# LPD-EPFL-ML/X-MAP

Measured on AMD Instinct MI355X. Metric: item_sim_pairs_per_s, higher is better.
Workload: dtype f64

## Files before the change

### include/xmap_hip.h

```cpp
#ifndef XMAP_HIP_H
#define XMAP_HIP_H
#include <stdint.h>

#ifdef __cplusplus
extern "C" {
#endif

#define XMAP_OK 0
#define XMAP_ERR_HIP -1
#define XMAP_ERR_ARG -2
#define XMAP_ERR_OVERFLOW -3
#define XMAP_ERR_CAPACITY -4

#define XMAP_COSINE 0
#define XMAP_ADJUST_COSINE 1
#define XMAP_COSINE_EXACT 2

#define XMAP_TOPC 10

typedef struct xmap_ratings {
    int64_t n_users;
    int32_t n_items;
    int64_t nnz;
    const int64_t *user_ptr;
    const int32_t *user_item;
    const float *user_rating;
    const int64_t *user_time;
    const int64_t *item_ptr;
    const int32_t *item_user;
    const float *item_rating;
    const int32_t *prefix_cls;
    const int32_t *suffix_cls;
    const uint32_t *contains_mask;
    const uint8_t *flags;
} xmap_ratings;

const char *xmap_last_error(void);
int xmap_version(void);

int xmap_trim(void);
int xmap_debug_arena(void *stream, int64_t *live, int64_t *reserved);
int xmap_debug_arena_call(void *stream, int64_t bytes, int fail);

int xmap_exclusive_scan_i64(void *stream, const int64_t *in, int64_t *out, int64_t n, int64_t *h_total);
int xmap_exclusive_scan_i32_to_i64(void *stream, const int32_t *in, int64_t *out, int64_t n, int64_t *h_total);


int xmap_build_csc(void *stream, int64_t n_users, int32_t n_items, int64_t nnz, const int64_t *user_ptr,
                   const int32_t *user_item, const float *user_rating, int32_t *cnt ,
                   int64_t *item_ptr , int32_t *item_user , float *item_rating );

int xmap_user_stats(void *stream, const xmap_ratings *R, double *u_avg, double *u_norm2);

int xmap_item_stats(void *stream, const xmap_ratings *R, const double *u_avg, double *info ,
                    double *norms ,
                    int32_t *ua_item , int32_t *ia_user ,
                    int32_t item_lo, int32_t item_hi );

#ifdef XMAP_CROSSCHECK
int xmap_sim_plan(void *stream, const xmap_ratings *R, int32_t slot_target, int32_t *Q, int64_t *W, int64_t *unit_ptr,
                  int64_t *h_n_units, int64_t *h_contrib);
int xmap_sim_units(void *stream, int32_t n_items, const int32_t *Q, const int64_t *unit_ptr,
                   int32_t *unit_item , int32_t *unit_q );

int xmap_sim_count(void *stream, const xmap_ratings *R, int method, int cap, const double *u_avg,
                   const double *info, const int32_t *ua_item, const int32_t *ia_user, const int32_t *Q,
                   const int32_t *unit_item, const int32_t *unit_q, int64_t unit_lo, int64_t unit_hi,
                   int32_t *unit_cnt , int64_t *d_counters , int64_t *h_counters );
int xmap_sim_fill(void *stream, const xmap_ratings *R, int method, int cap, const double *u_avg,
                  const double *info, const int32_t *ua_item, const int32_t *ia_user, const int32_t *Q,
                  const int32_t *unit_item, const int32_t *unit_q, int64_t unit_lo, int64_t unit_hi,
                  const int64_t *unit_off , int32_t *col, double *sim, int32_t *mutu, int32_t *nij);

int xmap_sim_row_ptr(void *stream, int32_t n_items, const int64_t *unit_ptr, const int64_t *unit_off ,
                     int64_t *row_ptr );
#endif

#define XMAP_PAIRS_HEAVY 1
#define XMAP_PAIRS_LIGHT 2
#define XMAP_PAIRS_HEAVY_MERGE 4
#define XMAP_PAIRS_RESET 8
#define XMAP_PAIRS_MIRCOUNT 16
#define XMAP_PAIRS_RAW 32
#define XMAP_PAIRS_SHARD_SUMS 64
#define XMAP_PAIRS_NO_MARKS 128
#define XMAP_PAIRS_DEAL(m, r) ((((m) & 0xff) << 16) | (((r) & 0xff) << 8))
#define XMAP_PAIRS_DEAL_MOD(phases) (((phases) >> 16) & 0xff)
#define XMAP_PAIRS_DEAL_REM(phases) (((phases) >> 8) & 0xff)
int xmap_sim2_layout(void *stream, const xmap_ratings *R, const double *info, int32_t ch_min, int32_t *hist ,
                     int64_t *pre , int32_t *ctl , int32_t *hid , int32_t *hlist ,
                     uint64_t *ub_key , void *ub ,
                     void *rc ,
                     uint64_t *Wp ,
                     int32_t dups , int32_t *h_ctl );
int xmap_sim2_plan(void *stream, const xmap_ratings *R, int32_t slot_target, const void *rc, const int64_t *pre,
                   const int32_t *hid, const int32_t *ctl, int32_t *Q, int32_t *C, uint8_t *small ,
                   uint64_t *Wp , int32_t *Qcat , int64_t *uq_ptr ,
                   int64_t *uc_ptr , int32_t dups, int64_t *h_counts );
int xmap_sim2_units(void *stream, int32_t n_items, const int64_t *item_ptr, const int32_t *Qcat, const int64_t *uq_ptr,
                    int32_t *uq_item, int32_t *uq_q , const int32_t *C, const int64_t *uc_ptr, int32_t *uc_item,
                    int32_t *uc_c);
int xmap_sim2_pairs(void *stream, const xmap_ratings *R, int method, int cap, const double *u_avg, const double *norms,
                    const void *rc, const void *ub, const int32_t *Q,
                    const uint8_t *small, const int32_t *uq_item, const int32_t *uq_q, const int64_t *cls_ptr ,
                    int64_t unit_lo, int64_t unit_hi, const int32_t *hid,
                    const int32_t *hlist, const int32_t *ctl, const int32_t *C, const int64_t *uc_ptr,
                    const int32_t *uc_item, const int32_t *uc_c, int32_t n_heavy_units, int32_t n_heavy, int phases,
                    double *hp_hi, double *hp_lo, int32_t *hp_cnt, int32_t *hp_mut, int64_t coo_cap, int32_t *coo_i,
                    int32_t *coo_j, double *coo_sim, int32_t *coo_mutu, int32_t *coo_nij,
                    double *coo_ls , int32_t *rowcnt,
                    int64_t *d_shards ,
                    int64_t *d_counters ,
                    int32_t *mircnt );
int xmap_sim2_scatter(void *stream, int32_t n_items, int64_t n_coo, const int32_t *coo_i, const int32_t *coo_j,
                      const double *coo_sim, const int32_t *coo_mutu, const int32_t *coo_nij, const double *coo_ls ,
                      const int64_t *row_ptr, int32_t *fill , const int32_t *hid, const int32_t *hlist,
                      int32_t *col, double *sim, int32_t *mutu, int32_t *nij, double *ls );
#define XMAP_LAYOUT_RECORDS 1
#define XMAP_LAYOUT_STATS 2
#define XMAP_LAYOUT_UB_FLAGS 4
#define XMAP_LAYOUT_RC_FLAGS 8
#define XMAP_LAYOUT_ALL 15
int xmap_sim3_layout(void *stream, const xmap_ratings *R, int64_t *item_ptr ,
                     const double *rating64 , int32_t ch_min, int32_t phases, int32_t stats_lo, int32_t stats_hi,
                     int32_t *cnt ,
                     double *u_avg , double *u_norm , int32_t *hist ,
                     int64_t *pre , int32_t *ctl , int32_t *hid , int32_t *hlist ,
                     uint64_t *ub_key , void *ub , void *srec ,
                     void *bufA , void *bufB , void *rc ,
                     uint64_t *Wp , double *info , double *norms , int32_t *h_ctl );
int xmap_sim3_plan(void *stream, const xmap_ratings *R, int32_t slot_target, const int64_t *pre, const int32_t *hid,
                   const int32_t *ctl, int32_t *Q, int32_t *C, uint8_t *small, uint64_t *Wp, int32_t *Qcat ,
                   int64_t *uq_ptr , int64_t *uc_ptr , int32_t dups, int32_t *uq_item, int32_t *uq_q ,
                   int32_t *uc_item, int32_t *uc_c, int64_t cap_light, int64_t cap_heavy, int64_t *h_out );
int xmap_sim3_mircount(void *stream, int32_t n_items, int64_t coo_cap, const int32_t *coo_i, const int32_t *coo_j,
                       const int64_t *d_shards , int64_t n_pairs, int32_t skip_self, void *scratch, int32_t *mir );
int xmap_sim3_mirror(void *stream, int32_t n_items, int64_t coo_cap, const int32_t *coo_i, const int32_t *coo_j,
                     const double *coo_sim, const int32_t *coo_mutu, const int32_t *coo_nij,
                     const int64_t *d_shards ,
                     int64_t n_pairs, const int32_t *own , const int32_t *mir , int32_t *tot ,
                     int64_t *row_ptr , int64_t *mptr , int32_t *fill ,
                     void *bufA , void *bufB , int32_t *col,
                     double *sim, int32_t *mutu, int32_t *nij, const double *coo_aux , double *aux ,
                     int32_t row_lo, int32_t row_hi );

int xmap_sim2_pack_pairs(void *stream, int64_t n_coo, const int32_t *coo_i, const int32_t *coo_j, const double *coo_sim,
                         const int32_t *coo_mutu, const int32_t *coo_nij, int64_t *rec , int64_t *h_count);
int xmap_sim2_unpack_pairs(void *stream, int64_t n, const int64_t *rec , int32_t *coo_i, int32_t *coo_j, double *coo_sim,
                           int32_t *coo_mutu, int32_t *coo_nij);
int xmap_item_partials(void *stream, const xmap_ratings *R, const double *u_avg, double *partial );
int xmap_item_merge(void *stream, int32_t n_items, int32_t n_parts, const double *parts , double *info ,
                    double *norms );
int xmap_sim2_pack_partials(void *stream, int64_t n_coo, const int32_t *coo_i, const int32_t *coo_j, const double *coo_hi,
                            const double *coo_lo, const int32_t *coo_mutu, const int32_t *coo_nij, int64_t *rec ,
                            int64_t *h_count);
int xmap_sim2_sort_partials(void *stream, int64_t n, const int64_t *rec , int64_t *rec_sorted , int32_t n_items,
                            int32_t n_owners );
int xmap_sim2_merge_partials(void *stream, int method, int cap, int32_t n_items, int64_t n, const int64_t *rec_sorted,
                             const double *norms , int32_t *coo_i, int32_t *coo_j, double *coo_sim, int32_t *coo_mutu,
                             int32_t *coo_nij, int32_t *rowcnt , int64_t *h_counts );



typedef struct xmap_sim {
    int32_t n_items;
    const int64_t *row_ptr;
    const int32_t *col;
    const double *sim;
    const int32_t *mutu;
    const int32_t *nij;
    const double *info;
    const double *frac;
} xmap_sim;

int xmap_bridge_flags(void *stream, const xmap_sim *S, const int32_t *prefix_cls, uint8_t *bb);

int xmap_knn_classify(void *stream, const xmap_sim *S, int top_k, const uint8_t *bb, const int32_t *suffix_cls,
                      const uint32_t *contains_mask, uint8_t *cls, int32_t *kcnt ,
                      int32_t *kcol , double *kval ,
                      int32_t row_lo, int32_t row_hi );

int xmap_knn_thresholds(void *stream, int32_t n_items, int top_k, const int32_t *kcnt, const int32_t *kcol, const double *kval,
                        void *thr );
int xmap_reverse_count(void *stream, const xmap_sim *S, int mode, int top_k, const uint8_t *bb, const uint8_t *cls,
                       const int32_t *kcnt, const int32_t *kcol, const double *kval, const int32_t *suffix_cls,
                       const uint32_t *contains_mask, const uint8_t *flags, const int64_t *attach_ptr,
                       const void *thr ,
// ... 344 lines not shown
```

### x-map_amd/csrc/api.hip

```cpp
#include <math.h>
#include <stdlib.h>
#include <vector>

#include "common.h"

namespace xmap {

struct Pool {
    std::vector<void *> ptrs;
    void release() {
        for (void *p : ptrs) (void)hipFree(p);
        ptrs.clear();
    }
};
struct ScratchPool : Pool { ~ScratchPool() { release(); } };

}

using namespace xmap;

struct xmap_ctx {
    int device = 0;
    hipStream_t st = nullptr;
    Pool p_ratings, p_sim, p_ext, p_gen, p_rows;
// ... 168 lines not shown
    XM_HIP(hipMemsetAsync(c->top_end, 0xff, sizeof(int32_t) * (size_t)I * XMAP_TOPC, c->st));
    XM_HIP(hipMemsetAsync(c->top_val, 0, sizeof(double) * (size_t)I * XMAP_TOPC, c->st));
    int64_t *d_cnt;
    XM_ALLOCZ(c->p_ext, d_cnt, 8);
    int64_t h_cnt[8] = {0, 0, 0, 0, 0, 0, 0, 0};
    int rc;
    if (c->T.n_nb > 0) rc = xmap_extend_cols(c->st, &c->T, &c->Un, &Rw, &O, c->fast_div, d_cnt, h_cnt);
    else rc = xmap_extend_paths(c->st, &c->T, &c->Un, &Rw, &O, d_cnt, h_cnt);
    if (rc && rc != XMAP_ERR_CAPACITY) {
        c->p_rows.release();
        c->acc = nullptr;
    }
    c->n_out = h_cnt[0]; c->n_paths = h_cnt[1];
    return rc;
}

struct TriPass {
    const xmap_ratings *R;
    const double *rating64;
    int ch_min, dups, method, cap;
    bool heavy;
    bool aux, skip_self;
    int64_t half_contrib;
    Pool *stats_pool, *csr_pool, *mutu_pool;
    int64_t *row_ptr;
};
struct TriResult {
    double *u_avg, *u_norm , *info, *norms , *sim, *aux;
    int32_t *col, *mutu, *nij;
    int64_t n, n_unordered, kept;
};

static int tri_pass(hipStream_t st, const TriPass &J, Pool &tmp, TriResult &O) {
#define T_ALLOC(ptr, n) XM_TRY(dalloc(tmp, &(ptr), (size_t)(n), st))
#define T_ALLOCZ(ptr, n) XM_TRY(dalloc(tmp, &(ptr), (size_t)(n), st, true))
    const xmap_ratings &R = *J.R;
    const int I = R.n_items;
    const int64_t U = R.n_users, nnz = R.nnz;
    const bool wide = J.rating64 != nullptr;
    const size_t n1 = (size_t)(nnz ? nnz : 1), i1 = (size_t)(I ? I : 1);
    const size_t rw = wide ? 3 : 2;
    int32_t *cnt, *hist, *ctl, *hid, *hlist;
    int64_t *pre;
    uint64_t *ub_key, *ub, *rcrec, *Wp, *srec, *buf_a, *buf_b;
    O.u_norm = nullptr; O.aux = nullptr;
    XM_TRY(dalloc(*J.stats_pool, &O.u_avg, (size_t)U, st, wide));
    if (!wide) XM_TRY(dalloc(*J.stats_pool, &O.u_norm, (size_t)U, st));
    XM_TRY(dalloc(*J.stats_pool, &O.info, i1 * 4, st, true));
    T_ALLOCZ(O.norms, 2 * i1);
    T_ALLOC(cnt, i1);
    T_ALLOC(hist, U + 2); T_ALLOC(pre, U + 3); T_ALLOC(ctl, 4); T_ALLOC(hid, i1); T_ALLOCZ(hlist, 1024);
    T_ALLOC(ub_key, n1); T_ALLOC(ub, (wide ? 2 : 1) * n1); T_ALLOC(rcrec, 2 * n1); T_ALLOC(Wp, i1);
    T_ALLOC(srec, rw * n1); T_ALLOC(buf_a, rw * n1); T_ALLOC(buf_b, rw * n1);
    XM_TRY(xmap_sim3_layout(st, &R, (int64_t *)R.item_ptr, J.rating64, J.ch_min, XMAP_LAYOUT_RECORDS | XMAP_LAYOUT_STATS | XMAP_LAYOUT_UB_FLAGS,
                            0, I, cnt, O.u_avg, O.u_norm, hist, pre, ctl, hid, hlist, ub_key, ub, srec, buf_a, buf_b, rcrec, Wp, O.info,
                            O.norms, nullptr));
    int32_t *Q, *Cc, *Qcat, *uq_item = nullptr, *uq_q = nullptr, *uc_item = nullptr, *uc_c = nullptr;
    uint8_t *small;
    int64_t *uq_ptr, *uc_ptr;
    T_ALLOCZ(Q, i1); T_ALLOCZ(Cc, i1); T_ALLOCZ(small, i1); T_ALLOC(Qcat, 5 * i1); T_ALLOCZ(uq_ptr, (size_t)5 * I + 1);
    T_ALLOCZ(uc_ptr, I + 1);
    int slot_target = 768;
    double coo_slack = 1.0;
    int64_t hc[10];
    auto plan = [&](int target) -> int {
        const int64_t cap_light = J.half_contrib / target + I + 1, cap_heavy = nnz / J.ch_min + 1025;
        T_ALLOC(uq_item, cap_light); T_ALLOC(uq_q, 4 * cap_light); T_ALLOC(uc_item, cap_heavy); T_ALLOC(uc_c, cap_heavy);
        return xmap_sim3_plan(st, &R, target, pre, hid, ctl, Q, Cc, small, Wp, Qcat, uq_ptr, uc_ptr, J.dups, uq_item, uq_q, uc_item, uc_c,
                              cap_light, cap_heavy, hc);
    };
    XM_TRY(plan(slot_target));
    const int phases = XMAP_PAIRS_RESET | XMAP_PAIRS_LIGHT | XMAP_PAIRS_MIRCOUNT | XMAP_PAIRS_SHARD_SUMS | XMAP_PAIRS_NO_MARKS |
                       (J.heavy ? XMAP_PAIRS_HEAVY | XMAP_PAIRS_HEAVY_MERGE : 0);
    int32_t *coo_i = nullptr, *coo_j = nullptr, *coo_mutu = nullptr, *coo_nij = nullptr, *own = nullptr, *mir = nullptr;
    double *coo_sim = nullptr, *coo_aux = nullptr;
    int64_t *d_shards = nullptr;
    int64_t cap_coo = 0;
    for (;;) {
        const int64_t n_light = hc[0], n_hu = J.heavy ? hc[1] : 0, n_heavy = J.heavy ? hc[9] : 0;
        cap_coo = ((int64_t)((double)(J.half_contrib > 0 ? J.half_contrib : 1) * coo_slack) / 4096 + 1100) * 4096;
        double *hp_hi, *hp_lo;
        int32_t *hp_cnt, *hp_mut;
        int64_t *d_cnt;
        T_ALLOC(coo_i, cap_coo); T_ALLOC(coo_j, cap_coo); T_ALLOC(coo_sim, cap_coo); T_ALLOC(coo_mutu, cap_coo); T_ALLOC(coo_nij, cap_coo);
        if (J.aux) T_ALLOC(coo_aux, cap_coo);
        T_ALLOC(own, i1); T_ALLOC(mir, i1);
        const size_t hp = (size_t)(n_hu ? n_hu : 1) * 1024;
        T_ALLOC(hp_hi, hp); T_ALLOC(hp_lo, hp); T_ALLOC(hp_cnt, hp); T_ALLOC(hp_mut, hp);
        T_ALLOCZ(d_cnt, 6); T_ALLOC(d_shards, 2 * 4096);
        XM_TRY(xmap_sim2_pairs(st, &R, J.method, J.cap, O.u_avg, O.norms, rcrec, ub, Q, small, uq_item, uq_q, hc + 2, 0, n_light, hid, hlist,
                               ctl, Cc, uc_ptr, uc_item, uc_c, (int32_t)n_hu, (int32_t)n_heavy, phases, hp_hi, hp_lo, hp_cnt, hp_mut, cap_coo, coo_i,
                               coo_j, coo_sim, coo_mutu, coo_nij, coo_aux, own, d_shards, d_cnt, mir));
        int64_t h_cnt[6];
        XM_TRY(d2h(h_cnt, d_cnt, 6, st));
        XM_HIP(hipStreamSynchronize(st));
        if (h_cnt[2]) {
            if (slot_target <= 32) { set_error("pair-table overflow"); return XMAP_ERR_OVERFLOW; }
            slot_target /= 2;
            XM_TRY(plan(slot_target));
            continue;
        }
        if (h_cnt[3]) {
            if (coo_slack > 64) { set_error("half-COO overflow"); return XMAP_ERR_CAPACITY; }
            coo_slack *= 2;
            continue;
        }
        O.n = h_cnt[4]; O.n_unordered = h_cnt[5];
        break;
    }
    const int64_t n = O.n;
    const size_t nn = (size_t)(n ? n : 1);
    O.kept = 2 * n;
    int64_t *mptr;
    int32_t *fill, *tot;
    uint64_t *mir_a, *mir_b;
    T_ALLOCZ(mptr, I + 1);
    XM_TRY(dalloc(*J.csr_pool, &O.col, (size_t)O.kept, st)); XM_TRY(dalloc(*J.csr_pool, &O.sim, (size_t)O.kept, st));
    XM_TRY(dalloc(*J.mutu_pool, &O.mutu, (size_t)O.kept, st)); XM_TRY(dalloc(*J.csr_pool, &O.nij, (size_t)O.kept, st));
    if (J.aux) XM_TRY(dalloc(*J.csr_pool, &O.aux, (size_t)O.kept, st));
    T_ALLOC(fill, i1); T_ALLOC(tot, i1); T_ALLOC(mir_a, (J.aux ? 4 : 3) * nn); T_ALLOC(mir_b, (J.aux ? 4 : 3) * nn);
    XM_TRY(xmap_sim3_mircount(st, I, cap_coo, coo_i, coo_j, d_shards, n, J.skip_self ? 1 : 0, mir_a, mir));
    return xmap_sim3_mirror(st, I, cap_coo, coo_i, coo_j, coo_sim, coo_mutu, coo_nij, d_shards, n, own, mir, tot, J.row_ptr, mptr, fill, mir_a,
                            mir_b, O.col, O.sim, O.mutu, O.nij, coo_aux, O.aux, 0, I);
#undef T_ALLOC
#undef T_ALLOCZ
}

}

extern "C" {

int xmap_ctx_create(int device, xmap_ctx **out) {
    XM_ARG(out);
    *out = nullptr;
    XM_HIP(hipSetDevice(device));
    xmap_ctx *c = new xmap_ctx();
    c->device = device;
    memset(&c->R, 0, sizeof(c->R)); memset(&c->S, 0, sizeof(c->S)); memset(&c->T, 0, sizeof(c->T)); memset(&c->Un, 0, sizeof(c->Un));
    hipError_t e = hipStreamCreate(&c->st);
    if (e != hipSuccess) { delete c; set_error("hipStreamCreate -> %s", hipGetErrorString(e)); return XMAP_ERR_HIP; }
    *out = c;
    return XMAP_OK;
}

void xmap_ctx_destroy(xmap_ctx *c) {
    if (!c) return;
    (void)hipSetDevice(c->device);
    (void)hipStreamSynchronize(c->st);
    drop_tail(c);
    drop_fold(c);
    drop_union(c);
    c->p_gen.release(); c->p_ext.release(); c->p_sim.release(); c->p_rows.release(); c->p_ratings.release();
    if (c->st) (void)hipStreamDestroy(c->st);
    delete c;
}

static bool plain_sums_exact(int64_t U, int64_t nnz, const float *rating) {
    const char *force = getenv("XMAP_EXACT_COSINE");
    if (force && force[0] == '1') return false;
    double M = 0.0;
    int e = 0;
    for (int64_t k = 0; k < nnz; k++) {
        const double r = fabs((double)rating[k]);
        if (!(r <= 1e300)) return false;
        if (r > M) M = r;
        while (e <= 26 && ldexp(r, e) != floor(ldexp(r, e))) e++;
        if (e > 26) return false;
    }
    if (M == 0.0) return true;
    const double Mi = ldexp(M, e);
    if (Mi > 134217728.0) return false;
    const uint64_t m2 = (uint64_t)Mi * (uint64_t)Mi;
    return (uint64_t)U <= (1ull << 53) / m2;
}
// ... 1208 lines not shown
```

### x-map_amd/csrc/common.h

```cpp
#pragma once
#if defined(__HIP_DEVICE_COMPILE__) && !defined(__gfx950__)
#error "libxmap_hip is written for gfx950 (MI355X): build with --offload-arch=gfx950"
#endif
#include <hip/hip_runtime.h>
#include <stdint.h>
#include <stdio.h>
#include <string.h>

#include "../../include/xmap_hip.h"

namespace xmap {

void set_error(const char *fmt, ...);

#define XM_HIP(call)                                                                         \
    do {                                                                                     \
        hipError_t e_ = (call);                                                              \
        if (e_ != hipSuccess) {                                                              \
            xmap::set_error("%s:%d %s -> %s", __FILE__, __LINE__, #call, hipGetErrorString(e_)); \
            return XMAP_ERR_HIP;                                                             \
        }                                                                                    \
    } while (0)

#define XM_LAUNCH_CHECK() XM_HIP(hipGetLastError())

#define XM_ARG(cond)                                                        \
    do {                                                                    \
        if (!(cond)) {                                                      \
            xmap::set_error("%s:%d bad argument: %s", __FILE__, __LINE__, #cond); \
            return XMAP_ERR_ARG;                                            \
        }                                                                   \
    } while (0)

hipError_t xm_malloc_async(void **p, size_t bytes, hipStream_t st);
hipError_t xm_free_async(void *p, hipStream_t st);
struct XmScope {
    int dev; hipStream_t st; size_t live0; bool ok;
    explicit XmScope(hipStream_t st);
    ~XmScope();
    XmScope(const XmScope &) = delete;
    XmScope &operator=(const XmScope &) = delete;
};
#define XM_SCOPE(stream) xmap::XmScope xm_scope_((hipStream_t)(stream))
int radix_sort_pairs(hipStream_t st, unsigned long long *keys, int *vals, unsigned long long *keys_tmp, int *vals_tmp, long long n,
                     int bits);

constexpr int WAVE = 64;

__device__ __forceinline__ int lane_id() { return threadIdx.x & 63; }

__device__ __forceinline__ int rl32(int v, int l) { return __builtin_amdgcn_readlane(v, l); }
__device__ __forceinline__ float rlf(float v, int l) { return __int_as_float(rl32(__float_as_int(v), l)); }
__device__ __forceinline__ long long rl64(long long v, int l) {
    int lo = rl32((int)(v & 0xffffffffll), l), hi = rl32((int)(v >> 32), l);
    return ((long long)hi << 32) | (unsigned int)lo;
}
__device__ __forceinline__ double rld(double v, int l) {
    return __longlong_as_double(rl64(__double_as_longlong(v), l));
}
__device__ __forceinline__ int uniform(int v) { return __builtin_amdgcn_readfirstlane(v); }

__device__ __forceinline__ unsigned long long lanemask_lt() {
    return (1ull << lane_id()) - 1ull;
}

__device__ __forceinline__ double wave_sum(double v) {
#pragma unroll
    for (int m = 32; m >= 1; m >>= 1) v += __shfl_xor(v, m, 64);
    return v;
}
__device__ __forceinline__ long long wave_sum_ll(long long v) {
#pragma unroll
    for (int m = 32; m >= 1; m >>= 1) v += __shfl_xor(v, m, 64);
    return v;
}

__device__ __forceinline__ void dd_add(double &hi, double &lo, double x) {
    double s = hi + x;
    double bb = s - hi;
    double e = (hi - (s - bb)) + (x - bb);
    e += lo;
    double h2 = s + e;
    lo = e - (h2 - s);
    hi = h2;
}

template <int G>
__device__ __forceinline__ void dd_reduce(double &hi, double &lo) {
#pragma unroll
    for (int m = G / 2; m >= 1; m >>= 1) {
        double oh = __shfl_down(hi, m, G), ol = __shfl_down(lo, m, G);
        dd_add(hi, lo, oh);
        dd_add(hi, lo, ol);
    }
}

// ... 7 lines not shown
```

### x-map_amd/csrc/tri.h

```cpp
#pragma once
#include "common.h"
#include "tilesort.h"

namespace xmap {

constexpr int T_SLOTS = 1024;
constexpr int HMAX = 1024;
constexpr int SMALL_BOUND = 96;
constexpr int MID_BOUND = 384;

constexpr int N_CLASSES = 5;
constexpr int WIDE_MIN = 2048;
__host__ __device__ __forceinline__ int class_rank(int cls) {
    return cls == 4 ? 0 : (cls == 0 ? 1 : (cls == 2 ? 2 : (cls == 3 ? 3 : 4)));
}

__device__ __forceinline__ double weighted(double cs, int n, int cap) {
    const int mn = n < cap ? n : cap;
    return 1.0 * cs * (double)mn / (double)cap;
}
__device__ __forceinline__ unsigned long long ls_key(double d) {
    return (d != d) ? 0x7ff8000000000000ull : (unsigned long long)__double_as_longlong(d);
}

struct RaterRec { int e0; int pos_ge; float rating; int user; };
struct UbWide { int item_ge; int pad; double rating; };
struct RaterRecWide { int e0; int pos_ge; double rating; };

constexpr int COO_SHARDS = 4096;

int mirror_counts(hipStream_t st, int n_items, long long range_cap, int n_ranges, const unsigned long long *cur, const int *coo_i,
                  const int *coo_j, bool skip_self, int *part, int *counts);
void ts_geometry(int K, long long M, int ch, ts::Geo &G);
int ts_prepare(hipStream_t st, ts::Geo &G, const long long *ptr);
extern template __global__ void ts::k_ts_bin<3, true, ts::RecLoader<3>>(ts::Geo, ts::RecLoader<3>, long long, unsigned long long *__restrict__);

}
```

### x-map_amd/csrc/tri_layout.hip

```cpp
#include "tri.h"
#include "item_stats.h"

namespace xmap {

__device__ __forceinline__ unsigned long long wkey(int n, int item) {
    return ((unsigned long long)(unsigned)n << 32) | (unsigned)item;
}

constexpr int HIST_LDS = 2048;
constexpr int HIST_PER = 16;
__global__ __launch_bounds__(256) void k_hist(int I, const long long *iptr, int HB, int *hist) {
    __shared__ int loc[HIST_LDS];
    for (int t = threadIdx.x; t < HIST_LDS; t += 256) loc[t] = 0;
    __syncthreads();
    const long long base = (long long)blockIdx.x * 256 * HIST_PER;
    for (int q = 0; q < HIST_PER; q++) {
        const long long i = base + (long long)q * 256 + threadIdx.x;
        if (i < I) {
            long long n = iptr[i + 1] - iptr[i];
            int bin = n < HB - 1 ? (int)n : HB - 1;
            if (bin < HIST_LDS) atomicAdd(&loc[bin], 1); else atomicAdd(&hist[bin], 1);
        }
    }
    __syncthreads();
// ... 132 lines not shown
        i = lo;
        const int u = iuser[p];
        const long long a = uptr[u], b = uptr[u + 1];
        RaterRec r;
        r.e0 = (int)a; r.pos_ge = 0; r.rating = 0.f; r.user = u;
        for (long long e = a; e < b; e++) {
            int2 v = ub[e];
            if ((v.x & 0x7fffffff) == i) {
                if (taken && e + 1 < b && (ub[e + 1].x & 0x7fffffff) == i) {
                    e += atomicAdd(&taken[e], 1);
                    v = ub[e];
                }
                const int pos = (b - a >= 2) ? (int)(e - a) : 0;
                r.pos_ge = (int)((unsigned)pos | ((unsigned)v.x & 0x80000000u));
                r.rating = __int_as_float(v.y);
                pos_sum = pos;
                break;
            }
        }
        rc[p] = r;
    }
    const int lane = lane_id();
    const int i_prev = __shfl_up(i, 1, 64);
    const unsigned long long heads = __ballot(lane == 0 || i != i_prev);
    long long incl = pos_sum;
#pragma unroll
    for (int d = 1; d < 64; d <<= 1) { const long long t = __shfl_up(incl, d, 64); if (lane >= d) incl += t; }
    const bool seg_end = (lane == 63) || ((heads >> (lane + 1)) & 1ull);
    const int h = 63 - __clzll((long long)(heads & ((lane == 63) ? ~0ull : ((2ull << lane) - 1ull))));
    const long long before = __shfl(incl, h > 0 ? h - 1 : 0, 64);
    if (seg_end && i >= 0) {
        const long long seg = incl - (h > 0 ? before : 0);
        if (seg) atomicAdd(&Wp[i], (unsigned long long)seg);
    }
}
__device__ __forceinline__ void plan_item(int i, long long w, int I, const long long *iptr, const long long *pre, int HB,
                                          const int *hid, const int *CH, int target, int dups, int *Q, int *C,
                                          uint8_t *small, unsigned long long *Wp, int *Qcat) {
    const long long n = iptr[i + 1] - iptr[i];
    long long ge = I - pre[n < HB - 1 ? n : HB - 1];
    const long long others = ge - 1 + (dups ? 1 : 0);
    long long bound = w < others ? w : others;
    int q = 0, c = 0;
    if (w > 0) {
        if (hid[i] >= 0) c = (int)((n + *CH - 1) / *CH);
        else q = (int)((bound + target - 1) / target);
    }
    Q[i] = q;
    C[i] = c;
    const int cls = (q >= 1 && n >= WIDE_MIN) ? 4
                    : ((q != 1) ? 0 : (bound <= SMALL_BOUND ? 1 : (bound <= 2 * SMALL_BOUND ? 3 : (bound <= MID_BOUND ? 2 : 0))));
    small[i] = (uint8_t)cls;
    Wp[i] = (unsigned long long)w;
    Qcat[(size_t)class_rank(cls) * I + i] = q;
}

__global__ __launch_bounds__(256) void k_plan2(int I, const long long *iptr, const RaterRec *rc, const long long *pre,
                                               int HB, const int *hid, const int *CH, int target, int dups, int *Q, int *C,
                                               uint8_t *small, unsigned long long *Wp, int *Qcat) {
    const int i = blockIdx.x * blockDim.x + threadIdx.x;
    if (i >= I) return;
    plan_item(i, (long long)Wp[i], I, iptr, pre, HB, hid, CH, target, dups, Q, C, small, Wp, Qcat);
}

__global__ __launch_bounds__(256) void k_fill_units2(int I, const long long *iptr, const int *Qcat, const long long *uq_ptr,
                                                     int *uq_item, int *uq_q, const int *C, const long long *uc_ptr, int *uc_item,
                                                     int *uc_c, long long cap_light, long long cap_heavy) {
    const long long x = (long long)blockIdx.x * blockDim.x + threadIdx.x;
    if (x >= (long long)N_CLASSES * I) return;
    const int i = (int)(x % I);
    long long b = uq_ptr[x];
    const int nq = Qcat[x];
    if (nq > 0) {
        const int p0 = (int)iptr[i], p1 = (int)iptr[i + 1];
        for (int k = 0; k < nq && b + k < cap_light; k++) {
            uq_item[b + k] = i;
            ((int4 *)uq_q)[b + k] = make_int4(k, p0, p1, nq);
        }
    }
    if (x >= I) return;
    b = uc_ptr[i];
    for (int k = 0; k < C[i] && b + k < cap_heavy; k++) { uc_item[b + k] = i; uc_c[b + k] = k; }
}

constexpr int CNT_SLOTS = 4096;
constexpr int CNT_CHUNK = 8192;
__device__ __forceinline__ int cnt_slot(int it) { return (int)(mix32((uint32_t)it) & (CNT_SLOTS - 1)); }

__global__ __launch_bounds__(256) void k_count3(long long nnz, const int *uitem, int *cnt) {
    __shared__ int tag[CNT_SLOTS], loc[CNT_SLOTS];
    for (int t = threadIdx.x; t < CNT_SLOTS; t += 256) { tag[t] = -1; loc[t] = 0; }
    __syncthreads();
    const long long e0 = (long long)blockIdx.x * CNT_CHUNK;
    for (int q = threadIdx.x; q < CNT_CHUNK; q += 256) {
        const long long e = e0 + q;
        if (e >= nnz) break;
        const int it = uitem[e];
        const int sl = cnt_slot(it);
        const int old = atomicCAS(&tag[sl], -1, it);
        if (old == -1 || old == it) atomicAdd(&loc[sl], 1); else atomicAdd(&cnt[it], 1);
    }
    __syncthreads();
    for (int t = threadIdx.x; t < CNT_SLOTS; t += 256)
        if (loc[t]) atomicAdd(&cnt[tag[t]], loc[t]);
}


template <bool WIDE>
__device__ __forceinline__ void sort_entry3(const int *uitem, const float *ur32, const double *ur64, const int *cnt,
                                            long long e, unsigned long long &key, int &px, long long &py) {
    const int it = uitem[e];
    key = wkey(cnt[it], it);
    px = it;
    py = WIDE ? __double_as_longlong(ur64[e]) : (long long)(unsigned)__float_as_int(ur32[e]);
}

template <bool WIDE>
__device__ __forceinline__ void bitonic_desc3(int width, int pos, unsigned long long &key, int &px, long long &py) {
#pragma unroll
    for (int k2 = 2; k2 <= 64; k2 <<= 1) {
        if (k2 <= width)
// ... 269 lines not shown
        dd_add(s, slo, o[0]);
        dd_add(s, slo, o[1]);
        dd_add(q, qlo, o[2]);
        dd_add(q, qlo, o[3]);
        dd_add(a2, a2lo, o[4]);
        dd_add(a2, a2lo, o[5]);
        n += o[6];
    }
    const int i = d.x;
    info[(size_t)i * 4 + 0] = (n > 0.0) ? 1.0 * s / n : 0.0;
    info[(size_t)i * 4 + 1] = sqrt(q);
    info[(size_t)i * 4 + 2] = sqrt(a2);
    info[(size_t)i * 4 + 3] = 1.0 * n;
    norms[i] = sqrt(q);
    norms[(size_t)I + i] = sqrt(a2);
}

template <typename Src>
__global__ __launch_bounds__(256) void k_item_big_flags(const long long *iptr, const Src src, BigList B, const double *info) {
    const unsigned c = blockIdx.x * 4 + uniform((int)(threadIdx.x >> 6));
    if (c >= B.counters[0]) return;
    const int2 d = B.chunks[c];
    const double avg = info[(size_t)d.x * 4];
    const long long p0 = iptr[d.x] + (long long)d.y * STAT_CHK;
    const long long p1 = min(iptr[d.x + 1], p0 + STAT_CHK);
    for (long long p = p0 + lane_id(); p < p1; p += 64) {
        double r; int u;
        src.load(p, r, u);
        src.set_flag(p, r >= avg);
    }
}

__global__ __launch_bounds__(256) void k_rc_flags(long long nnz, RaterRec *rc, const int2 *ub, const double *info) {
    const long long p = (long long)blockIdx.x * blockDim.x + threadIdx.x;
    if (p >= nnz) return;
    const RaterRec r = rc[p];
    const int it = ub[(long long)r.e0 + (r.pos_ge & 0x7fffffff)].x & 0x7fffffff;
    if ((double)r.rating >= info[(size_t)it * 4]) rc[p].pos_ge = (int)((unsigned)r.pos_ge | 0x80000000u);
}

__global__ __launch_bounds__(256) void k_ub_flags(long long nnz, int2 *ub, const double *info) {
    const long long e = (long long)blockIdx.x * blockDim.x + threadIdx.x;
    if (e >= nnz) return;
    const int2 v = ub[e];
    if ((double)__int_as_float(v.y) >= info[(size_t)v.x * 4]) ub[e].x = (int)((unsigned)v.x | 0x80000000u);
}

}

using namespace xmap;

namespace {

int heavy_set(void *stream, int I, int64_t n_users, const int64_t *item_ptr, int32_t ch_min, int32_t *hist, int64_t *pre, int32_t *ctl,
              int32_t *hid, int32_t *hlist) {
    hipStream_t st = (hipStream_t)stream;
    const int HB = (int)n_users + 2;
    XM_HIP(hipMemsetAsync(hist, 0, sizeof(int32_t) * (size_t)HB, st));
    XM_HIP(hipMemsetAsync(ctl, 0x7f, sizeof(int32_t), st));
    XM_HIP(hipMemsetAsync(ctl + 1, 0, 3 * sizeof(int32_t), st));
    if (I > 0) {
        k_hist<<<dim3((unsigned)((I + 256 * HIST_PER - 1) / (256 * HIST_PER))), dim3(256), 0, st>>>(I, (const long long *)item_ptr, HB, hist);
        XM_LAUNCH_CHECK();
    }
    int rcode = xmap_exclusive_scan_i32_to_i64(stream, hist, pre, HB, nullptr);
    if (rcode) return rcode;
    if (HB - 1 > ch_min) {
        k_threshold<<<dim3((unsigned)((HB + 255) / 256)), dim3(256), 0, st>>>(I, HB, (const long long *)pre, ch_min, ctl);
        XM_LAUNCH_CHECK();
    }
    if (I > 0) {
        k_mark_heavy<<<dim3((unsigned)((I + 255) / 256)), dim3(256), 0, st>>>(I, (const long long *)item_ptr, ctl, hid, hlist, ctl + 1);
        XM_LAUNCH_CHECK();
    }
    return XMAP_OK;
}

int read_heavy_ctl(hipStream_t st, const int32_t *ctl, int32_t *h_ctl) {
    XM_HIP(hipMemcpyAsync(h_ctl, ctl, 2 * sizeof(int32_t), hipMemcpyDeviceToHost, st));
    XM_HIP(hipStreamSynchronize(st));
    if (h_ctl[1] > HMAX) {
        set_error("heavy set larger than %d", HMAX);
        return XMAP_ERR_OVERFLOW;
    }
    return XMAP_OK;
}

int plan_rows(void *stream, const xmap_ratings *R, int32_t slot_target, const void *rc, const int64_t *pre, const int32_t *hid,
              const int32_t *ctl, int32_t *Q, int32_t *C, uint8_t *small, uint64_t *Wp, int32_t *Qcat, int64_t *uq_ptr, int64_t *uc_ptr,
              int32_t dups, int64_t *h_light, int64_t *h_heavy) {
    XM_ARG(slot_target > 0 && slot_target <= T_SLOTS);
    hipStream_t st = (hipStream_t)stream;
    const int I = R->n_items;
    XM_HIP(hipMemsetAsync(Qcat, 0, sizeof(int32_t) * (size_t)N_CLASSES * (size_t)(I > 0 ? I : 1), st));
    if (I > 0) {
        k_plan2<<<dim3((unsigned)((I + 255) / 256)), dim3(256), 0, st>>>(
            I, (const long long *)R->item_ptr, (const RaterRec *)rc, (const long long *)pre, (int)R->n_users + 2, hid, ctl, slot_target, dups,
            Q, C, small, (unsigned long long *)Wp, Qcat);
        XM_LAUNCH_CHECK();
    }
    int rcode = xmap_exclusive_scan_i32_to_i64(stream, Qcat, uq_ptr, (int64_t)N_CLASSES * I, h_light);
    if (rcode) return rcode;
    return xmap_exclusive_scan_i32_to_i64(stream, C, uc_ptr, I, h_heavy);
}

template <int RW>
int sort_rater_records(hipStream_t st, const ts::Geo &G, long long nnz, const void *srec, void *bufA, void *bufB, const int64_t *user_ptr,
                       void *rc, uint64_t *Wp) {
    constexpr bool WIDE = RW == 3;
    const dim3 gridA((unsigned)((nnz + G.ch - 1) / G.ch)), gridB((unsigned)G.clist_cap), gridL((unsigned)G.slist_cap);
    ts::RecLoader<RW> LA{(const unsigned long long *)srec}, LB{(const unsigned long long *)bufA};
    ts::k_ts_bin<RW, false, ts::RecLoader<RW>><<<gridA, dim3(ts::BT), 0, st>>>(G, LA, nnz, (unsigned long long *)bufA);
    XM_LAUNCH_CHECK();
    ts::k_ts_bin<RW, true, ts::RecLoader<RW>><<<gridB, dim3(ts::BT), 0, st>>>(G, LB, nnz, (unsigned long long *)bufB);
    XM_LAUNCH_CHECK();
    k_rc_tiles<WIDE><<<dim3((unsigned)G.T), dim3(ts::CT), 0, st>>>(G, (const unsigned long long *)bufB, (const long long *)user_ptr,
                                                                  (ulonglong2 *)rc, (unsigned long long *)Wp);
    XM_LAUNCH_CHECK();
    k_rc_large<WIDE><<<gridL, dim3(ts::LT), 0, st>>>(G, (const unsigned long long *)bufB, (const long long *)user_ptr, (ulonglong2 *)rc,
                                                     (unsigned long long *)Wp);
    XM_LAUNCH_CHECK();
    return XMAP_OK;
}

template <typename Src>
int item_stats3(hipStream_t st, int I, int lo, int hi, const int64_t *item_ptr, const Src &src, double *info, double *norms,
                const BigList &B) {
    const long long *iptr = (const long long *)item_ptr;
    const dim3 grid((unsigned)((hi - lo + 15) / 16)), gridC((unsigned)((B.chunk_cap + 3) / 4)), gridI((unsigned)((B.item_cap + 63) / 64));
    k_item_stats3<Src><<<grid, dim3(256), 0, st>>>(I, lo, hi, iptr, src, info, norms, B);
    XM_LAUNCH_CHECK();
    k_item_chunks<Src><<<gridC, dim3(256), 0, st>>>(iptr, src, B);
    XM_LAUNCH_CHECK();
    k_item_big<<<gridI, dim3(64), 0, st>>>(I, B, info, norms);
    XM_LAUNCH_CHECK();
    if constexpr (Src::has_flags) {
        k_item_big_flags<Src><<<gridC, dim3(256), 0, st>>>(iptr, src, B, info);
        XM_LAUNCH_CHECK();
    }
    return XMAP_OK;
}

}

extern "C" {

int xmap_sim2_layout(void *stream, const xmap_ratings *R, const double *info, int32_t ch_min, int32_t *hist ,
                     int64_t *pre , int32_t *ctl , int32_t *hid, int32_t *hlist ,
                     uint64_t *ub_key , void *ub , void *rc ,
                     uint64_t *Wp , int32_t dups, int32_t *h_ctl ) {
    XM_ARG(R && info && hist && pre && ctl && hid && hlist && ub_key && ub && rc && Wp && ch_min >= 64);
    XM_ARG(R->nnz < 0x7fffffffLL && R->n_users < 0x7ffffff0LL);
    hipStream_t st = (hipStream_t)stream;
    const int I = R->n_items;
    int rcode = heavy_set(stream, I, R->n_users, R->item_ptr, ch_min, hist, pre, ctl, hid, hlist);
    if (rcode) return rcode;
    if (R->n_users > 0) {
        k_sort_profiles<<<dim3((unsigned)((R->n_users + 15) / 16)), dim3(256), 0, st>>>(
            R->n_users, (const long long *)R->user_ptr, R->user_item, R->user_rating, (const long long *)R->item_ptr, info,
            (unsigned long long *)ub_key, (int2 *)ub);
        XM_LAUNCH_CHECK();
    }
    XM_HIP(hipMemsetAsync(Wp, 0, sizeof(uint64_t) * (size_t)(I > 0 ? I : 1), st));
    if (R->nnz > 0) {
        if (dups) XM_HIP(hipMemsetAsync(ub_key, 0, sizeof(int32_t) * (size_t)R->nnz, st));
        k_rater_records<<<dim3((unsigned)((R->nnz + 255) / 256)), dim3(256), 0, st>>>(
            I, R->nnz, (const long long *)R->item_ptr, R->item_user, (const long long *)R->user_ptr, (const int2 *)ub,
            (RaterRec *)rc, dups ? (int *)ub_key : nullptr, (unsigned long long *)Wp);
        XM_LAUNCH_CHECK();
    }
    return h_ctl ? read_heavy_ctl(st, ctl, h_ctl) : XMAP_OK;
}

int xmap_sim2_plan(void *stream, const xmap_ratings *R, int32_t slot_target, const void *rc, const int64_t *pre,
                   const int32_t *hid, const int32_t *ctl, int32_t *Q, int32_t *C, uint8_t *small, uint64_t *Wp ,
                   int32_t *Qcat , int64_t *uq_ptr , int64_t *uc_ptr, int32_t dups,
                   int64_t *h_counts ) {
    XM_ARG(R && rc && Wp && pre && hid && ctl && Q && C && small && Qcat && uq_ptr && uc_ptr && h_counts);
    hipStream_t st = (hipStream_t)stream;
    const int I = R->n_items;
    int rcode = plan_rows(stream, R, slot_target, rc, pre, hid, ctl, Q, C, small, Wp, Qcat, uq_ptr, uc_ptr, dups, &h_counts[0], &h_counts[1]);
    if (rcode) return rcode;
    if (I > 0)
        XM_HIP(hipMemcpy2DAsync(&h_counts[2], sizeof(int64_t), uq_ptr, sizeof(int64_t) * (size_t)I, sizeof(int64_t),
                                N_CLASSES, hipMemcpyDeviceToHost, st));
    else
        for (int c = 0; c < N_CLASSES; c++) h_counts[2 + c] = 0;
    XM_HIP(hipStreamSynchronize(st));
    h_counts[2 + N_CLASSES] = h_counts[0];
    return XMAP_OK;
}

int xmap_sim2_units(void *stream, int32_t n_items, const int64_t *item_ptr, const int32_t *Qcat, const int64_t *uq_ptr,
                    int32_t *uq_item, int32_t *uq_q, const int32_t *C, const int64_t *uc_ptr, int32_t *uc_item, int32_t *uc_c) {
    XM_ARG(item_ptr && Qcat && uq_ptr && uq_item && uq_q && C && uc_ptr && uc_item && uc_c);
    if (n_items == 0) return XMAP_OK;
    k_fill_units2<<<dim3((unsigned)(((long long)N_CLASSES * n_items + 255) / 256)), dim3(256), 0, (hipStream_t)stream>>>(
        n_items, (const long long *)item_ptr, Qcat, (const long long *)uq_ptr, uq_item, uq_q, C, (const long long *)uc_ptr, uc_item, uc_c, 0x7fffffffffffffffLL,
        0x7fffffffffffffffLL);
    XM_LAUNCH_CHECK();
    return XMAP_OK;
}

int xmap_sim3_plan(void *stream, const xmap_ratings *R, int32_t slot_target, const int64_t *pre, const int32_t *hid,
                   const int32_t *ctl, int32_t *Q, int32_t *C, uint8_t *small, uint64_t *Wp, int32_t *Qcat, int64_t *uq_ptr,
                   int64_t *uc_ptr, int32_t dups, int32_t *uq_item, int32_t *uq_q, int32_t *uc_item, int32_t *uc_c,
                   int64_t cap_light, int64_t cap_heavy, int64_t *h_out) {
    XM_SCOPE(stream);
    XM_ARG(R && Wp && pre && hid && ctl && Q && C && small && Qcat && uq_ptr && uc_ptr && h_out);
    XM_ARG(uq_item && uq_q && uc_item && uc_c && cap_light >= 0 && cap_heavy >= 0);
    hipStream_t st = (hipStream_t)stream;
    const int I = R->n_items;
    for (int c = 0; c < 10; c++) h_out[c] = 0;
    int rcode = plan_rows(stream, R, slot_target, nullptr, pre, hid, ctl, Q, C, small, Wp, Qcat, uq_ptr, uc_ptr, dups, nullptr, nullptr);
    if (rcode) return rcode;
    if (I > 0) {
        k_fill_units2<<<dim3((unsigned)(((long long)N_CLASSES * I + 255) / 256)), dim3(256), 0, st>>>(
            I, (const long long *)R->item_ptr, Qcat, (const long long *)uq_ptr, uq_item, uq_q, C, (const long long *)uc_ptr, uc_item, uc_c,
            cap_light, cap_heavy);
        XM_LAUNCH_CHECK();
        XM_HIP(hipMemcpy2DAsync(&h_out[2], sizeof(int64_t), uq_ptr, sizeof(int64_t) * (size_t)I, sizeof(int64_t), N_CLASSES + 1,
                                hipMemcpyDeviceToHost, st));
        XM_HIP(hipMemcpyAsync(&h_out[1], uc_ptr + I, sizeof(int64_t), hipMemcpyDeviceToHost, st));
    }
    int32_t h_ctl[2] = {0, 0};
    rcode = read_heavy_ctl(st, ctl, h_ctl);
    h_out[0] = h_out[2 + N_CLASSES];
    h_out[8] = h_ctl[0]; h_out[9] = h_ctl[1];
    if (rcode) return rcode;
    if (h_out[0] > cap_light || h_out[1] > cap_heavy) {
        set_error("unit arrays too small: %lld light / %lld heavy units, room for %lld / %lld", (long long)h_out[0], (long long)h_out[1],
                  (long long)cap_light, (long long)cap_heavy);
        return XMAP_ERR_CAPACITY;
    }
    return XMAP_OK;
}

int xmap_sim3_layout(void *stream, const xmap_ratings *R, int64_t *item_ptr, const double *rating64, int32_t ch_min, int32_t phases,
                     int32_t stats_lo, int32_t stats_hi, int32_t *cnt, double *u_avg, double *u_norm, int32_t *hist, int64_t *pre, int32_t *ctl, int32_t *hid, int32_t *hlist,
                     uint64_t *ub_key, void *ub, void *srec, void *bufA, void *bufB, void *rc, uint64_t *Wp, double *info,
                     double *norms, int32_t *h_ctl) {
    XM_SCOPE(stream);
    XM_ARG(R && item_ptr && (const int64_t *)item_ptr == R->item_ptr && cnt && u_avg && hist && pre && ctl && hid && hlist);
    XM_ARG(ub_key && ub && srec && bufA && bufB && rc && Wp && info && norms && ch_min >= 64);
    XM_ARG(R->nnz < 0x7fffffffLL && R->n_users < 0x7ffffff0LL && R->n_items >= 0);
    XM_ARG(rating64 || u_norm);
    XM_ARG(stats_lo >= 0 && stats_lo <= stats_hi && stats_hi <= R->n_items && (phases & ~XMAP_LAYOUT_ALL) == 0);
    hipStream_t st = (hipStream_t)stream;
    const int I = R->n_items;
    const long long nnz = R->nnz;
    const bool wide = rating64 != nullptr;
    const size_t In = (size_t)(I > 0 ? I : 1);
    int rcode = XMAP_OK;
    if (phases & XMAP_LAYOUT_RECORDS) {
        XM_HIP(hipMemsetAsync(cnt, 0, sizeof(int32_t) * In, st));
        const char *cb_env = getenv("XMAP_COUNT_PART_MIN");
        const long long cb_min = cb_env ? atoll(cb_env) : 2000000ll;
        if (nnz >= cb_min && I > 0) {
            rcode = mirror_counts(st, I, nnz, 1, nullptr, nullptr, R->user_item, false, (int *)bufA, cnt);
            if (rcode) return rcode;
        } else if (nnz > 0) {
            k_count3<<<dim3((unsigned)((nnz + CNT_CHUNK - 1) / CNT_CHUNK)), dim3(256), 0, st>>>(nnz, R->user_item, cnt);
            XM_LAUNCH_CHECK();
        }
        rcode = xmap_exclusive_scan_i32_to_i64(stream, cnt, item_ptr, I, nullptr);
        if (rcode) return rcode;
        if (!wide) {
            rcode = xmap_user_stats(stream, R, u_avg, u_norm);
            if (rcode) return rcode;
        }
        rcode = heavy_set(stream, I, R->n_users, item_ptr, ch_min, hist, pre, ctl, hid, hlist);
        if (rcode) return rcode;
        if (R->n_users > 0 && nnz > 0) {
            const dim3 grid((unsigned)((R->n_users + 15) / 16));
            (wide ? k_sort_profiles3<true> : k_sort_profiles3<false>)<<<grid, dim3(256), 0, st>>>(
                R->n_users, (const long long *)R->user_ptr, R->user_item, wide ? nullptr : R->user_rating, rating64, cnt,
                (unsigned long long *)ub_key, ub, (unsigned long long *)srec);
            XM_LAUNCH_CHECK();
        }
        XM_HIP(hipMemsetAsync(Wp, 0, sizeof(uint64_t) * In, st));
        if (nnz > 0 && I > 0) {
            ts::Geo G;
            ts_geometry(I, nnz, wide ? ts::Chunk<3>::CH : ts::Chunk<2>::CH, G);
            rcode = ts_prepare(st, G, (const long long *)item_ptr);
            if (rcode) return rcode;
            rcode = wide ? sort_rater_records<3>(st, G, nnz, srec, bufA, bufB, R->user_ptr, rc, Wp)
                         : sort_rater_records<2>(st, G, nnz, srec, bufA, bufB, R->user_ptr, rc, Wp);
            if (rcode) return rcode;
        }
    }
    if ((phases & XMAP_LAYOUT_STATS) && stats_hi > stats_lo) {
        BigList B;
        B.chunk_cap = nnz / STAT_CHK + nnz / STAT_BIG + 2;
        B.item_cap = nnz / STAT_BIG + 2;
        XM_HIP(xm_malloc_async((void **)&B.counters, 2 * sizeof(unsigned), st));
        XM_HIP(xm_malloc_async((void **)&B.chunks, sizeof(int2) * (size_t)B.chunk_cap, st));
        XM_HIP(xm_malloc_async((void **)&B.items, sizeof(int4) * (size_t)B.item_cap, st));
        XM_HIP(xm_malloc_async((void **)&B.part, sizeof(double) * ITEM_PART * (size_t)B.chunk_cap, st));
        XM_HIP(hipMemsetAsync(B.counters, 0, 2 * sizeof(unsigned), st));
        rcode = wide ? item_stats3(st, I, stats_lo, stats_hi, item_ptr, RcWideSrc{(const RaterRecWide *)rc}, info, norms, B)
                     : item_stats3(st, I, stats_lo, stats_hi, item_ptr, RcSrc{(RaterRec *)rc, u_avg}, info, norms, B);
        if (rcode) return rcode;
    }
    if (!wide && nnz > 0 && I > 0) {
        if (phases & XMAP_LAYOUT_RC_FLAGS) {
            k_rc_flags<<<dim3((unsigned)((nnz + 255) / 256)), dim3(256), 0, st>>>(nnz, (RaterRec *)rc, (const int2 *)ub, info);
            XM_LAUNCH_CHECK();
        }
        if (phases & XMAP_LAYOUT_UB_FLAGS) {
            k_ub_flags<<<dim3((unsigned)((nnz + 255) / 256)), dim3(256), 0, st>>>(nnz, (int2 *)ub, info);
            XM_LAUNCH_CHECK();
        }
    }
    return h_ctl ? read_heavy_ctl(st, ctl, h_ctl) : XMAP_OK;
}
}
```

### x-map_amd/csrc/tri_mirror.hip

```cpp
#include "tri.h"

namespace xmap {

constexpr int SC_U = 4;
__global__ __launch_bounds__(256) void k_scatter(long long n, const int *coo_i, const int *coo_j, const double *coo_sim,
                                                 const int *coo_mutu, const int *coo_nij, const double *coo_aux,
                                                 const long long *row_ptr, int *fill, int *col, double *sim, int *mutu,
                                                 int *nij, double *aux) {
    const int lane = lane_id();
    const long long r0 = ((long long)blockIdx.x * (blockDim.x >> 6) + uniform((int)(threadIdx.x >> 6))) * (64 * SC_U) + lane;
    int i[SC_U], j[SC_U], m[SC_U], nn[SC_U];
    double s[SC_U], x[SC_U];
    bool valid[SC_U];
#pragma unroll
    for (int u = 0; u < SC_U; u++) {
        const long long r = r0 + 64 * u;
        i[u] = (r < n) ? coo_i[r] : -1;
    }
#pragma unroll
    for (int u = 0; u < SC_U; u++) {
        const long long r = r0 + 64 * u;
        valid[u] = i[u] >= 0;
        j[u] = 0; m[u] = 0; nn[u] = 0; s[u] = 0.0; x[u] = 0.0;
        if (valid[u]) {
// ... 133 lines not shown
    int it[CB_SPB][EPT];
    unsigned rk[CB_SPB][EPT];
#pragma unroll
    for (int sg = 0; sg < CB_SPB; sg++) {
        const long long g = (long long)blockIdx.x * CB_SPB + sg;
        const long long c = g / n_ranges;
        const int r = (int)(g - c * n_ranges);
        const long long n = (c < cpr) ? ((cur && (long long)cur[r] < range_cap) ? (long long)cur[r] : range_cap) : 0;
        const long long b = (long long)r * range_cap;
#pragma unroll
        for (int q = 0; q < EPT; q++) {
            const long long e = c * CB_CHUNK + q * CB_T + tid;
            it[sg][q] = -1;
            if (e < n) {
                const int j = coo_j[b + e];
                if (!SELF || j != coo_i[b + e]) it[sg][q] = j;
            }
        }
    }
#pragma unroll
    for (int sg = 0; sg < CB_SPB; sg++)
#pragma unroll
        for (int q = 0; q < EPT; q++) rk[sg][q] = it[sg][q] >= 0 ? atomicAdd(&h[it[sg][q] >> sh], 1u) : 0u;
    __syncthreads();
    {
        const unsigned c = h[tid];
        const int lane = tid & 63, w = tid >> 6;
        unsigned inc = c;
#pragma unroll
        for (int d = 1; d < 64; d <<= 1) { const unsigned o = __shfl_up(inc, d, 64); if (lane >= d) inc += o; }
        if (lane == 63) wsum[w] = inc;
        __syncthreads();
        unsigned bs = 0;
        for (int x = 0; x < w; x++) bs += wsum[x];
        off[tid] = bs + inc - c;
        if (tid == CB_T - 1) off[CB_MAX] = bs + inc;
        if (c) base[tid] = bptr[tid] + (long long)atomicAdd(&bcur[tid], c);
    }
    __syncthreads();
#pragma unroll
    for (int sg = 0; sg < CB_SPB; sg++)
#pragma unroll
        for (int q = 0; q < EPT; q++)
            if (it[sg][q] >= 0) stage[off[it[sg][q] >> sh] + rk[sg][q]] = it[sg][q];
    __syncthreads();
    const int total = (int)off[CB_MAX];
    for (int x = tid; x < total; x += CB_T) {
        const int v = stage[x];
        const int bk = v >> sh;
        out[base[bk] + (x - (int)off[bk])] = v;
    }
}

__global__ __launch_bounds__(256) void k_row_totals(int I, const int *own, const int *mir, int *tot) {
    const int i = blockIdx.x * blockDim.x + threadIdx.x;
    if (i < I) tot[i] = own[i] + mir[i];
}

template <bool AUX, bool SHARE>
struct CooLoaderT {
    static constexpr int RW = AUX ? 4 : 3;
    const int *__restrict__ coo_i; const int *__restrict__ coo_j; const double *__restrict__ coo_sim;
    const int *__restrict__ coo_mutu; const int *__restrict__ coo_nij; const double *__restrict__ coo_aux;
    const longlong2 *chunks; const unsigned *n_chunks;
    const long long *row_ptr; int *fill; int *col; double *sim; int *mutu; int *nij; double *aux;
    int row_lo, row_hi;
    __device__ __forceinline__ bool chunk(long long, long long &i0, long long &i1) const {
        if (blockIdx.x >= *n_chunks) return false;
        const longlong2 c = chunks[blockIdx.x];
        i0 = c.x; i1 = c.x + c.y;
        return true;
    }
    __device__ __forceinline__ void load(long long idx, unsigned long long (&w)[RW]) const {
        w[0] = (unsigned long long)(unsigned)coo_j[idx] | ((unsigned long long)(unsigned)coo_i[idx] << 32);
        w[1] = (unsigned long long)__double_as_longlong(coo_sim[idx]);
        w[2] = (unsigned long long)(unsigned)coo_mutu[idx] | ((unsigned long long)(unsigned)coo_nij[idx] << 32);
        if (AUX) w[RW - 1] = (unsigned long long)__double_as_longlong(coo_aux[idx]);
    }
    __device__ __forceinline__ bool keep(const unsigned long long (&w)[RW]) const {
        const int j = (int)(unsigned)w[0];
        return (!AUX || j != (int)(w[0] >> 32)) && (!SHARE || (j >= row_lo && j < row_hi));
    }
    __device__ __forceinline__ void extra(long long, const unsigned long long (&w)[ts::Chunk<RW>::EPT][RW],
                                          const bool (&on)[ts::Chunk<RW>::EPT]) const {
        constexpr int E = ts::Chunk<RW>::EPT;
        const int lane = lane_id();
        int lead[E], base[E];
        long long rp[E];
#pragma unroll
        for (int r = 0; r < E; r++) {
            const int iw = (int)(w[r][0] >> 32);
            const bool mine = on[r] && (!SHARE || (iw >= row_lo && iw < row_hi));
            const int iu = mine ? iw : -1 - lane;
            const int prev = __shfl_up(iu, 1, 64);
            const bool leader = (lane == 0) || (prev != iu);
            const unsigned long long lm = __ballot(leader);
            const unsigned long long below = lm & ((lane == 63) ? ~0ull : ((2ull << lane) - 1ull));
            lead[r] = 63 - __clzll((long long)below);
            const unsigned long long above = (lane == 63) ? 0ull : (lm >> (lane + 1));
            const int next = above ? lane + 1 + (__ffsll((long long)above) - 1) : 64;
            base[r] = 0; rp[r] = -1;
            if (leader && mine) base[r] = atomicAdd(&fill[iu], next - lane);
            if (mine) rp[r] = row_ptr[iu];
        }
#pragma unroll
        for (int r = 0; r < E; r++) {
            const int bs = __shfl(base[r], lead[r], 64);
            if (rp[r] >= 0) {
                const long long a = rp[r] + bs + (lane - lead[r]);
                col[a] = (int)(unsigned)w[r][0]; sim[a] = __longlong_as_double((long long)w[r][1]);
// ... 111 lines not shown
    const int t = (int)(measure(G, k, p) >> G.ts_log);
    const bool large = cnt >= (1ll << G.ts_log);
    const int tp = k > 0 ? (int)(measure(G, k - 1, G.ptr[k - 1]) >> G.ts_log) : -1;
    for (int x = tp + 1; x <= t; x++) { G.tile_key0[x] = k; G.tile_pos0[x] = p; }
    if (k == G.K - 1)
        for (int x = t + 1; x <= G.T; x++) { G.tile_key0[x] = G.K; G.tile_pos0[x] = G.ptr[G.K]; }
    if (large) {
        G.tile_large[t] = k;
        const int nsl = (int)((cnt + SL - 1) / SL);
        const unsigned base = atomicAdd(&G.counters[1], (unsigned)nsl);
        for (int x = 0; x < nsl; x++)
            if ((long long)base + x < G.slist_cap) G.slist[base + x] = make_int2(k, x);
    }
}

__global__ __launch_bounds__(256) void k_ts_chunks(Geo G) {
    const int a = blockIdx.x * blockDim.x + threadIdx.x;
    if (a >= G.NA) return;
    const int t0 = a << NB_LOG, t1 = min(G.T, (a + 1) << NB_LOG);
    const long long size = G.tile_pos0[t1] - G.tile_pos0[t0];
    const int nch = (int)((size + G.ch - 1) / G.ch);
    if (nch == 0) return;
    const unsigned base = atomicAdd(&G.counters[0], (unsigned)nch);
    for (int x = 0; x < nch; x++)
        if ((long long)base + x < G.clist_cap) G.clist[base + x] = make_int2(a, x);
}

}

template __global__ void ts::k_ts_bin<3, true, ts::RecLoader<3>>(ts::Geo, ts::RecLoader<3>, long long, unsigned long long *__restrict__);

void ts_geometry(int K, long long M, int ch, ts::Geo &G) {
    G.K = K; G.M = M; G.ch = ch;
    G.ts_log = 11;
    for (;;) {
        const long long TS = 1ll << G.ts_log;
        long long kw = M / (4 * (long long)(K > 0 ? K : 1));
        const long long kw_min = TS / (ts::NK_MAX - 2) + 1;
        if (kw < kw_min) kw = kw_min;
        if (kw < 4) kw = 4;
        const long long tiles = ((M + (long long)K * kw) >> G.ts_log) + 1;
        if (tiles <= (long long)ts::NA_MAX * ts::NB || G.ts_log >= 30) {
            G.KW = (int)kw;
            G.NA = (int)((tiles + ts::NB - 1) / ts::NB);
            if (G.NA < 1) G.NA = 1;
            if (G.NA > ts::NA_MAX) G.NA = ts::NA_MAX;
            G.T = G.NA * ts::NB;
            return;
        }
        G.ts_log++;
    }
}

int ts_prepare(hipStream_t st, ts::Geo &G, const long long *ptr) {
    G.ptr = ptr;
    G.clist_cap = G.M / G.ch + G.NA + 1;
    G.slist_cap = G.M / ts::SL + (G.M >> G.ts_log) + 2;
    XM_HIP(xm_malloc_async((void **)&G.tile_key0, sizeof(int) * ((size_t)G.T + 1), st));
    XM_HIP(xm_malloc_async((void **)&G.tile_pos0, sizeof(long long) * ((size_t)G.T + 1), st));
    XM_HIP(xm_malloc_async((void **)&G.tile_large, sizeof(int) * (size_t)G.T, st));
    unsigned long long *z = nullptr;
    const size_t nz = (size_t)G.NA + 2 * (size_t)G.T + 1;
    XM_HIP(xm_malloc_async((void **)&z, sizeof(unsigned long long) * nz, st));
    G.curA = z; G.curB = z + G.NA; G.counters = (unsigned *)(z + G.NA + 2 * (size_t)G.T);
    XM_HIP(xm_malloc_async((void **)&G.clist, sizeof(int2) * (size_t)G.clist_cap, st));
    XM_HIP(xm_malloc_async((void **)&G.slist, sizeof(int2) * (size_t)G.slist_cap, st));
    XM_HIP(hipMemsetAsync(z, 0, sizeof(unsigned long long) * nz, st));
    XM_HIP(hipMemsetAsync(G.tile_large, 0xff, sizeof(int) * (size_t)G.T, st));
    ts::k_ts_plan<<<dim3((unsigned)((G.K + 255) / 256)), dim3(256), 0, st>>>(G);
    XM_LAUNCH_CHECK();
    ts::k_ts_chunks<<<dim3((unsigned)((G.NA + 255) / 256)), dim3(256), 0, st>>>(G);
    XM_LAUNCH_CHECK();
    return XMAP_OK;
}

namespace {
template <bool AUX, bool SHARE>
int mirror_levels(hipStream_t st, const ts::Geo &G, int64_t coo_cap, const int32_t *coo_i, const int32_t *coo_j, const double *coo_sim,
                  const int32_t *coo_mutu, const int32_t *coo_nij, const double *coo_aux, const longlong2 *chunks, const unsigned *n_chunks,
                  long long chunk_cap, int64_t n_pairs, const int32_t *own, const int64_t *row_ptr, int32_t *fill, void *bufA, void *bufB,
                  int32_t *col, double *sim, int32_t *mutu, int32_t *nij, double *aux, int row_lo, int row_hi) {
    constexpr int RW = AUX ? 4 : 3;
    CooLoaderT<AUX, SHARE> LA{coo_i, coo_j, coo_sim, coo_mutu, coo_nij, coo_aux, chunks, n_chunks, (const long long *)row_ptr, fill,
                              col, sim, mutu, nij, aux, row_lo, row_hi};
    ts::RecLoader<RW> LB{(const unsigned long long *)bufA};
    ts::k_ts_bin<RW, false, CooLoaderT<AUX, SHARE>><<<dim3((unsigned)chunk_cap), dim3(ts::BT), 0, st>>>(G, LA, coo_cap, (unsigned long long *)bufA);
    XM_LAUNCH_CHECK();
    ts::k_ts_bin<RW, true, ts::RecLoader<RW>><<<dim3((unsigned)G.clist_cap), dim3(ts::BT), 0, st>>>(G, LB, n_pairs, (unsigned long long *)bufB);
    XM_LAUNCH_CHECK();
    k_mir_tiles<AUX><<<dim3((unsigned)G.T), dim3(ts::CT), 0, st>>>(G, (const unsigned long long *)bufB, (const long long *)row_ptr, own, col,
                                                                   sim, mutu, nij, aux);
    XM_LAUNCH_CHECK();
    k_mir_large<AUX><<<dim3((unsigned)G.slist_cap), dim3(ts::LT), 0, st>>>(G, (const unsigned long long *)bufB, (const long long *)row_ptr, own,
                                                                            col, sim, mutu, nij, aux);
    XM_LAUNCH_CHECK();
    return XMAP_OK;
}
}

int mirror_counts(hipStream_t st, int n_items, long long range_cap, int n_ranges, const unsigned long long *cur, const int *coo_i,
                  const int *coo_j, bool skip_self, int *part, int *counts) {
    if (n_items <= 0 || range_cap <= 0 || n_ranges <= 0) return XMAP_OK;
    int sh = 0;
    while (((long long)(n_items - 1) >> sh) >= CB_MAX) sh++;
    unsigned *bcnt = nullptr, *bcur = nullptr;
    long long *bptr = nullptr;
    XM_HIP(xm_malloc_async((void **)&bcnt, sizeof(unsigned) * CB_MAX, st));
    XM_HIP(xm_malloc_async((void **)&bcur, sizeof(unsigned) * CB_MAX, st));
    XM_HIP(xm_malloc_async((void **)&bptr, sizeof(long long) * (CB_MAX + 1), st));
    XM_HIP(hipMemsetAsync(bcnt, 0, sizeof(unsigned) * CB_MAX, st));
    const long long segs = (long long)n_ranges * ((range_cap + CB_CHUNK - 1) / CB_CHUNK);
    const dim3 g((unsigned)((segs + CB_SPB - 1) / CB_SPB));
    (skip_self ? k_cbs_hist<true> : k_cbs_hist<false>)<<<g, dim3(CB_T), 0, st>>>(range_cap, n_ranges, cur, coo_i, coo_j, sh, bcnt);
    XM_LAUNCH_CHECK();
    k_cb_scan<<<dim3(1), dim3(CB_MAX), 0, st>>>(bcnt, bptr, bcur);
    XM_LAUNCH_CHECK();
    (skip_self ? k_cbs_scatter<true> : k_cbs_scatter<false>)<<<g, dim3(CB_T), 0, st>>>(range_cap, n_ranges, cur, coo_i, coo_j, sh, bptr, bcur,
                                                                                        part);
    XM_LAUNCH_CHECK();
    const long long cap = range_cap * n_ranges;
    k_cb_count<<<dim3((unsigned)((cap + (long long)CB_CHUNK * CB_SPB - 1) / ((long long)CB_CHUNK * CB_SPB))), dim3(CB_T), 0, st>>>(
        -1, part, sh, bptr, n_items, counts);
    XM_LAUNCH_CHECK();
    return XMAP_OK;
}

}

using namespace xmap;

extern "C" {

int xmap_sim2_scatter(void *stream, int32_t n_items, int64_t n_coo, const int32_t *coo_i, const int32_t *coo_j,
                      const double *coo_sim, const int32_t *coo_mutu, const int32_t *coo_nij, const double *coo_ls ,
                      const int64_t *row_ptr, int32_t *fill , const int32_t *hid, const int32_t *hlist,
                      int32_t *col, double *sim, int32_t *mutu, int32_t *nij, double *ls ) {
    XM_ARG(coo_i && coo_j && coo_sim && coo_mutu && coo_nij && row_ptr && fill && hid && hlist && col && sim && mutu && nij);
    XM_ARG((coo_ls != nullptr) == (ls != nullptr));
    hipStream_t st = (hipStream_t)stream;
    XM_HIP(hipMemsetAsync(fill, 0, sizeof(int32_t) * (size_t)(n_items > 0 ? n_items : 1), st));
    if (n_coo > 0) {
        k_scatter<<<dim3((unsigned)((n_coo + 256 * SC_U - 1) / (256 * SC_U))), dim3(256), 0, st>>>(
            n_coo, coo_i, coo_j, coo_sim, coo_mutu, coo_nij, coo_ls, (const long long *)row_ptr, fill, col, sim, mutu, nij, ls);
        XM_LAUNCH_CHECK();
    }
    return XMAP_OK;
}

int xmap_sim3_mircount(void *stream, int32_t n_items, int64_t coo_cap, const int32_t *coo_i, const int32_t *coo_j,
                       const int64_t *d_shards, int64_t n_pairs, int32_t skip_self, void *scratch, int32_t *mir) {
    XM_SCOPE(stream);
    XM_ARG(coo_i && coo_j && scratch && mir && n_items >= 0 && coo_cap >= 0 && n_pairs >= 0);
    XM_ARG(d_shards ? (coo_cap >= COO_SHARDS) : (n_pairs <= coo_cap));
    hipStream_t st = (hipStream_t)stream;
    if (n_items == 0) return XMAP_OK;
    XM_HIP(hipMemsetAsync(mir, 0, sizeof(int32_t) * (size_t)n_items, st));
    if (n_pairs == 0 || coo_cap == 0) return XMAP_OK;
    return mirror_counts(st, n_items, d_shards ? coo_cap / COO_SHARDS : n_pairs, d_shards ? COO_SHARDS : 1,
                         (const unsigned long long *)d_shards, coo_i, coo_j, skip_self != 0, (int *)scratch, mir);
}

int xmap_sim3_mirror(void *stream, int32_t n_items, int64_t coo_cap, const int32_t *coo_i, const int32_t *coo_j,
                     const double *coo_sim, const int32_t *coo_mutu, const int32_t *coo_nij, const int64_t *d_shards, int64_t n_pairs,
                     const int32_t *own, const int32_t *mir, int32_t *tot, int64_t *row_ptr, int64_t *mptr, int32_t *fill,
                     void *bufA, void *bufB, int32_t *col, double *sim, int32_t *mutu, int32_t *nij, const double *coo_aux, double *aux,
                     int32_t row_lo, int32_t row_hi) {
    XM_SCOPE(stream);
    XM_ARG(row_lo >= 0 && row_lo <= row_hi && row_hi <= n_items);
    XM_ARG(coo_i && coo_j && coo_sim && coo_mutu && coo_nij && own && mir && tot && row_ptr && mptr && fill && bufA && bufB);
    XM_ARG(col && sim && mutu && nij && n_items >= 0 && coo_cap >= 0 && n_pairs >= 0 && n_pairs < 0x7fffffffLL);
    XM_ARG(d_shards ? (coo_cap >= COO_SHARDS) : (n_pairs <= coo_cap));
    XM_ARG((coo_aux != nullptr) == (aux != nullptr));
    hipStream_t st = (hipStream_t)stream;
    const int I = n_items;
    if (I > 0) {
        k_row_totals<<<dim3((unsigned)((I + 255) / 256)), dim3(256), 0, st>>>(I, own, mir, tot);
        XM_LAUNCH_CHECK();
    }
    int rcode = xmap_exclusive_scan_i32_to_i64(stream, tot, row_ptr, I, nullptr);
    if (rcode) return rcode;
    rcode = xmap_exclusive_scan_i32_to_i64(stream, mir, mptr, I, nullptr);
    if (rcode) return rcode;
    if (n_pairs == 0 || I == 0 || coo_cap == 0) return XMAP_OK;
    XM_HIP(hipMemsetAsync(fill, 0, sizeof(int32_t) * (size_t)I, st));
    ts::Geo G;
    ts_geometry(I, n_pairs, coo_aux ? ts::Chunk<4>::CH : ts::Chunk<3>::CH, G);
    rcode = ts_prepare(st, G, (const long long *)mptr);
    if (rcode) return rcode;
    static_assert(ts::Chunk<3>::CH <= ts::Chunk<4>::CH && ts::Chunk<4>::CH % ts::Chunk<3>::CH == 0, "chunk lists by the narrow record width");
    const int n_shards = d_shards ? COO_SHARDS : 1;
    const long long shard_cap = d_shards ? coo_cap / COO_SHARDS : coo_cap;
    const long long chunk_cap = n_pairs / ts::Chunk<3>::CH + n_shards + 1;
    longlong2 *chunks = nullptr;
    unsigned *n_chunks = nullptr;
    XM_HIP(xm_malloc_async((void **)&chunks, sizeof(longlong2) * (size_t)chunk_cap, st));
    XM_HIP(xm_malloc_async((void **)&n_chunks, sizeof(unsigned), st));
    XM_HIP(hipMemsetAsync(n_chunks, 0, sizeof(unsigned), st));
    k_coo_chunks<<<dim3((unsigned)((n_shards + 255) / 256)), dim3(256), 0, st>>>(n_shards, shard_cap, (const unsigned long long *)d_shards,
                                                                                 n_pairs, chunks, n_chunks, chunk_cap);
    XM_LAUNCH_CHECK();
    const bool share = row_lo > 0 || row_hi < I;
    auto levels = coo_aux ? (share ? mirror_levels<true, true> : mirror_levels<true, false>)
                          : (share ? mirror_levels<false, true> : mirror_levels<false, false>);
    return levels(st, G, coo_cap, coo_i, coo_j, coo_sim, coo_mutu, coo_nij, coo_aux, chunks, n_chunks, chunk_cap, n_pairs, own, row_ptr, fill,
                  bufA, bufB, col, sim, mutu, nij, aux, row_lo, row_hi);
}
}
```

### x-map_amd/csrc/tri_pairs.hip

```cpp
#include <type_traits>

#include "tri.h"

namespace xmap {

constexpr uint32_t T_EMPTY = 0xFFFFFFFFu;

struct TriArgs {
    const long long *iptr;
    const RaterRec *rc;
    const int2 *ub;
    const double *u_avg; const double *nrm;
    int cap;
    const int *Q; const uint8_t *small; const int *uq_item; const int *uq_q; long long unit_lo, unit_hi;
    const int *hid; const int *hlist; const int *CH; const int *uc_item; const int *uc_c;
    const long long *uc_ptr; const int *C;
    double *hp_hi; double *hp_lo; int *hp_cnt; int *hp_mut;
    long long shard_cap;
    unsigned long long *shard_cur;
    unsigned long long *shard_occ;
    int *coo_i; int *coo_j; double *coo_sim; int *coo_mutu; int *coo_nij;
    double *coo_aux;
    int *rowcnt;
    int *mircnt;
// ... 509 lines not shown

namespace {

template <int METHOD, bool LS>
int launch_tri(int c, dim3 grid, hipStream_t st, const TriArgs &A) {
#define XM_TRI(LOG_SLOTS, NW) k_pair_tri<METHOD, LOG_SLOTS, NW, LS><<<grid, dim3(64 * NW), 0, st>>>(A)
    switch (c) {
    case 0: XM_TRI(10, 16); break;
    case 1: XM_TRI(10, 4); break;
    case 2: XM_TRI(9, 2); break;
    case 3: XM_TRI(8, 1); break;
    default: XM_TRI(7, 1); break;
    }
#undef XM_TRI
    XM_LAUNCH_CHECK();
    return XMAP_OK;
}

int launch_heavy(int method, hipStream_t st, const TriArgs &A, int n_units, int n_heavy) {
    const bool cos = method == XMAP_COSINE;
    if (n_units > 0) {
        (cos ? k_pair_heavy<XMAP_COSINE> : k_pair_heavy<XMAP_ADJUST_COSINE>)<<<dim3((unsigned)n_units), dim3(64 * HEAVY_WAVES), 0, st>>>(A);
        XM_LAUNCH_CHECK();
    }
    if (n_heavy > 0) {
        (cos ? k_heavy_merge<XMAP_COSINE> : k_heavy_merge<XMAP_ADJUST_COSINE>)<<<dim3((unsigned)n_heavy), dim3(256), 0, st>>>(A, n_heavy);
        XM_LAUNCH_CHECK();
    }
    return XMAP_OK;
}

}

extern "C" {

int xmap_sim2_pairs(void *stream, const xmap_ratings *R, int method, int cap, const double *u_avg, const double *norms, const void *rc,
                    const void *ub, const int32_t *Q, const uint8_t *small, const int32_t *uq_item, const int32_t *uq_q,
                    const int64_t *cls_ptr , int64_t unit_lo, int64_t unit_hi, const int32_t *hid, const int32_t *hlist,
                    const int32_t *ctl, const int32_t *C, const int64_t *uc_ptr, const int32_t *uc_item, const int32_t *uc_c,
                    int32_t n_heavy_units, int32_t n_heavy, int phases, double *hp_hi, double *hp_lo, int32_t *hp_cnt, int32_t *hp_mut,
                    int64_t coo_cap, int32_t *coo_i, int32_t *coo_j, double *coo_sim, int32_t *coo_mutu, int32_t *coo_nij,
                    double *coo_ls , int32_t *rowcnt, int64_t *d_shards , int64_t *d_counters ,
                    int32_t *mircnt ) {
    XM_SCOPE(stream);
    XM_ARG(R && u_avg && norms && rc && ub);
    XM_ARG(Q && small && uq_item && uq_q && cls_ptr && hid && hlist && ctl && C && uc_ptr && uc_item && uc_c);
    XM_ARG(coo_i && coo_j && coo_sim && coo_mutu && coo_nij && rowcnt && d_shards && d_counters);
    XM_ARG(coo_cap >= COO_SHARDS);
    XM_ARG(method == XMAP_COSINE || method == XMAP_ADJUST_COSINE || method == XMAP_COSINE_EXACT);
    XM_ARG(n_heavy_units == 0 || !(phases & (XMAP_PAIRS_HEAVY | XMAP_PAIRS_HEAVY_MERGE)) || (hp_hi && hp_lo && hp_cnt && hp_mut));
    hipStream_t st = (hipStream_t)stream;
    const bool exact_cos = method == XMAP_COSINE_EXACT;
    const double *nrm = norms + (method == XMAP_ADJUST_COSINE ? (size_t)R->n_items : 0);
    if (exact_cos) {
        double *zero_avg = nullptr;
        const size_t ub = sizeof(double) * (size_t)(R->n_users > 0 ? R->n_users : 1);
        XM_HIP(xm_malloc_async((void **)&zero_avg, ub, st));
        XM_HIP(hipMemsetAsync(zero_avg, 0, ub, st));
        u_avg = zero_avg;
        method = XMAP_ADJUST_COSINE;
    }
    const bool raw = (phases & XMAP_PAIRS_RAW) != 0;
    XM_ARG(!coo_ls || ((raw || method == XMAP_ADJUST_COSINE) && n_heavy_units == 0));
    XM_ARG(!raw || (coo_ls && n_heavy_units == 0 && n_heavy == 0));
    const size_t In = (size_t)(R->n_items > 0 ? R->n_items : 1);
    if (phases & XMAP_PAIRS_RESET) {
        XM_HIP(hipMemsetAsync(d_counters, 0, 4 * sizeof(int64_t), st));
        XM_HIP(hipMemsetAsync(d_shards, 0, 2 * COO_SHARDS * sizeof(int64_t), st));
        if (!(phases & XMAP_PAIRS_NO_MARKS)) XM_HIP(hipMemsetAsync(coo_i, 0xff, sizeof(int32_t) * (size_t)coo_cap, st));
        XM_HIP(hipMemsetAsync(rowcnt, 0, sizeof(int32_t) * In, st));
        if (mircnt) XM_HIP(hipMemsetAsync(mircnt, 0, sizeof(int32_t) * In, st));
    }
    TriArgs A;
    memset(&A, 0, sizeof(A));
    A.iptr = (const long long *)R->item_ptr; A.rc = (const RaterRec *)rc; A.ub = (const int2 *)ub;
    A.u_avg = u_avg; A.nrm = nrm; A.cap = cap;
    A.Q = Q; A.small = small; A.uq_item = uq_item; A.uq_q = uq_q; A.unit_lo = unit_lo; A.unit_hi = unit_hi;
    A.hid = hid; A.hlist = hlist; A.CH = ctl; A.uc_item = uc_item; A.uc_c = uc_c;
    A.uc_ptr = (const long long *)uc_ptr; A.C = C;
    A.hp_hi = hp_hi; A.hp_lo = hp_lo; A.hp_cnt = hp_cnt; A.hp_mut = hp_mut;
    A.shard_cap = coo_cap / COO_SHARDS; A.shard_cur = (unsigned long long *)d_shards;
    A.shard_occ = (unsigned long long *)d_shards + COO_SHARDS;
    A.coo_i = coo_i; A.coo_j = coo_j; A.coo_sim = coo_sim; A.coo_mutu = coo_mutu; A.coo_nij = coo_nij; A.coo_aux = coo_ls; A.raw = raw ? 1 : 0;
    A.heavy_mod = XMAP_PAIRS_DEAL_MOD(phases); A.heavy_rem = XMAP_PAIRS_DEAL_REM(phases);
    if (A.heavy_mod < 1) A.heavy_mod = 1;
    A.rowcnt = rowcnt; A.mircnt = mircnt; A.counters = (unsigned long long *)d_counters;
    const int all_rows = XMAP_PAIRS_HEAVY | XMAP_PAIRS_LIGHT | XMAP_PAIRS_HEAVY_MERGE;
    const bool light = (phases & XMAP_PAIRS_LIGHT) && unit_hi > unit_lo;
    const bool heavy_aside = (phases & all_rows) == all_rows && n_heavy_units > 0 && unit_hi > unit_lo;
    hipStream_t hs = st;
    SideStreams *side = nullptr;
    if (light || heavy_aside) {
        side = side_streams();
        if (!side) return XMAP_ERR_HIP;
        XM_HIP(hipEventRecord(side->fork, st));
    }
    if (heavy_aside) {
        hs = side->s[N_CLASSES];
        XM_HIP(hipStreamWaitEvent(hs, side->fork, 0));
    }
    int rcode = launch_heavy(method, hs, A, (phases & XMAP_PAIRS_HEAVY) ? n_heavy_units : 0, heavy_aside ? n_heavy : 0);
    if (rcode) return rcode;
    if (heavy_aside) {
        XM_HIP(hipEventRecord(side->done[N_CLASSES], hs));
        XM_HIP(hipStreamWaitEvent(st, side->done[N_CLASSES], 0));
    }
    if (light) {
        for (int c = 0; c < N_CLASSES; c++) {
            const long long lo = unit_lo > cls_ptr[c] ? unit_lo : cls_ptr[c];
            const long long hi = unit_hi < cls_ptr[c + 1] ? unit_hi : cls_ptr[c + 1];
            if (hi <= lo) continue;
            A.unit_lo = lo; A.unit_hi = hi;
            const dim3 grid((unsigned)(hi - lo));
            hipStream_t cs = side->s[c];
            XM_HIP(hipStreamWaitEvent(cs, side->fork, 0));
            if (coo_ls && !raw) rcode = launch_tri<XMAP_ADJUST_COSINE, true>(c, grid, cs, A);
            else if (method == XMAP_COSINE) rcode = launch_tri<XMAP_COSINE, false>(c, grid, cs, A);
            else rcode = launch_tri<XMAP_ADJUST_COSINE, false>(c, grid, cs, A);
            if (rcode) return rcode;
            XM_HIP(hipEventRecord(side->done[c], cs));
            XM_HIP(hipStreamWaitEvent(st, side->done[c], 0));
        }
        A.unit_lo = unit_lo; A.unit_hi = unit_hi;
    }
    if ((phases & XMAP_PAIRS_HEAVY_MERGE) && !heavy_aside && n_heavy_units > 0) {
        rcode = launch_heavy(method, st, A, 0, n_heavy);
        if (rcode) return rcode;
    }
    if (phases & XMAP_PAIRS_SHARD_SUMS) {
        XM_HIP(hipMemsetAsync(d_counters + 4, 0, 2 * sizeof(int64_t), st));
        k_shard_sums<<<dim3(1), dim3(256), 0, st>>>((const unsigned long long *)d_shards, (unsigned long long *)d_counters);
        XM_LAUNCH_CHECK();
    }
    if ((phases & XMAP_PAIRS_MIRCOUNT) && !raw && !mircnt && R->n_items > 0) {
        int *part = nullptr;
        XM_HIP(xm_malloc_async((void **)&part, sizeof(int) * (size_t)coo_cap, st));
        return mirror_counts(st, R->n_items, coo_cap / COO_SHARDS, COO_SHARDS, (const unsigned long long *)d_shards, coo_i, coo_j,
                             coo_ls != nullptr, part, rowcnt);
    }
    return XMAP_OK;
}
}
```

### x-map_amd/csrc/util.hip

```cpp
#include <stdarg.h>
#include <stdlib.h>
#include <vector>

#include "common.h"

namespace xmap {
static thread_local char g_err[512] = "";
void set_error(const char *fmt, ...) {
    va_list ap;
    va_start(ap, fmt);
    vsnprintf(g_err, sizeof(g_err), fmt, ap);
    va_end(ap);
}

namespace {
struct Chunk { char *base; size_t size, used; };
struct Arena { int dev; hipStream_t st; std::vector<Chunk> chunks; size_t live; };
thread_local std::vector<Arena> g_arenas;
constexpr size_t ARENA_KEEP = (size_t)256 << 20;
Arena *arena_find(int dev, hipStream_t st) {
    for (Arena &a : g_arenas) if (a.dev == dev && a.st == st) return &a;
    return nullptr;
}
Arena *arena_of(hipStream_t st) {
// ... 10 lines not shown
    if (hipStreamSynchronize(a->st) != hipSuccess) return;
    std::vector<Chunk> keep;
    size_t kept = 0;
    std::vector<Chunk> all = a->chunks;
    for (size_t i = 0; i < all.size(); i++)
        for (size_t j = i + 1; j < all.size(); j++)
            if (all[j].size < all[i].size) { Chunk t = all[i]; all[i] = all[j]; all[j] = t; }
    for (Chunk &c : all) {
        if (kept + c.size <= ARENA_KEEP) { keep.push_back(c); kept += c.size; }
        else (void)hipFree(c.base);
    }
    a->chunks.swap(keep);
}
}

XmScope::XmScope(hipStream_t s) : dev(0), st(s), live0(0), ok(false) {
    if (hipGetDevice(&dev) != hipSuccess) return;
    ok = true;
    if (Arena *a = arena_find(dev, st)) live0 = a->live;
}
XmScope::~XmScope() {
    if (!ok) return;
    Arena *a = arena_find(dev, st);
    if (!a || a->live <= live0) return;
    a->live = live0;
    if (a->live == 0) arena_reset(a);
}

hipError_t xm_malloc_async(void **p, size_t bytes, hipStream_t st) {
    Arena *a = arena_of(st);
    if (!a) return hipErrorInvalidDevice;
    bytes = (bytes + 255) & ~(size_t)255;
    if (bytes == 0) bytes = 256;
    for (Chunk &c : a->chunks)
        if (c.size - c.used >= bytes) { *p = c.base + c.used; c.used += bytes; a->live++; return hipSuccess; }
    Chunk c;
    c.size = bytes > ((size_t)32 << 20) ? bytes : ((size_t)32 << 20);
    c.used = bytes;
    hipError_t e = hipMalloc((void **)&c.base, c.size);
    if (e != hipSuccess) return e;
    a->chunks.push_back(c);
    *p = c.base;
    a->live++;
    return hipSuccess;
}
hipError_t xm_free_async(void *p, hipStream_t st) {
    (void)p;
    Arena *a = arena_of(st);
    if (!a || a->live == 0) return hipErrorInvalidValue;
    if (--a->live == 0) arena_reset(a);
    return hipSuccess;
}

constexpr int SCAN_THREADS = 256;
constexpr int SCAN_ITEMS = 8;
constexpr int SCAN_TILE = SCAN_THREADS * SCAN_ITEMS;

__device__ __forceinline__ long long block_exclusive_scan(long long v, long long *total, long long *smem) {
    int lane = threadIdx.x & 63, w = threadIdx.x >> 6;
    long long inc = v;
#pragma unroll
    for (int d = 1; d < 64; d <<= 1) {
        long long o = __shfl_up(inc, d, 64);
        if (lane >= d) inc += o;
    }
    if (lane == 63) smem[w] = inc;
    __syncthreads();
    long long base = 0, tot = 0;
    for (int k = 0; k < SCAN_THREADS / 64; k++) {
        long long s = smem[k];
        if (k < w) base += s;
        tot += s;
    }
    __syncthreads();
    *total = tot;
    return base + inc - v;
}

template <typename TIn>
__global__ __launch_bounds__(SCAN_THREADS) void k_tile_sums(const TIn *in, long long n, long long *tile_sum) {
    __shared__ long long smem[4];
    long long base = (long long)blockIdx.x * SCAN_TILE + (long long)threadIdx.x * SCAN_ITEMS;
    long long s = 0;
#pragma unroll
    for (int k = 0; k < SCAN_ITEMS; k++)
        if (base + k < n) s += (long long)in[base + k];
    long long tot;
    block_exclusive_scan(s, &tot, smem);
    if (threadIdx.x == 0) tile_sum[blockIdx.x] = tot;
}

__global__ __launch_bounds__(SCAN_THREADS) void k_scan_tile_sums(long long *tile_sum, long long n_tiles, long long *grand) {
    __shared__ long long smem[4];
    long long carry = 0;
    for (long long b = 0; b < n_tiles; b += SCAN_THREADS) {
        long long i = b + threadIdx.x;
        long long v = i < n_tiles ? tile_sum[i] : 0;
        long long tot;
        long long ex = block_exclusive_scan(v, &tot, smem);
        if (i < n_tiles) tile_sum[i] = carry + ex;
        carry += tot;
    }
    if (threadIdx.x == 0) *grand = carry;
}

template <typename TIn>
__global__ __launch_bounds__(SCAN_THREADS) void k_tile_scan(const TIn *in, long long n, const long long *tile_off,
                                                            long long *out) {
    __shared__ long long smem[4];
    long long base = (long long)blockIdx.x * SCAN_TILE + (long long)threadIdx.x * SCAN_ITEMS;
    long long v[SCAN_ITEMS];
    long long s = 0;
#pragma unroll
    for (int k = 0; k < SCAN_ITEMS; k++) {
        v[k] = (base + k < n) ? (long long)in[base + k] : 0;
        s += v[k];
    }
    long long tot;
    long long ex = block_exclusive_scan(s, &tot, smem) + tile_off[blockIdx.x];
#pragma unroll
    for (int k = 0; k < SCAN_ITEMS; k++) {
        if (base + k < n) out[base + k] = ex;
        ex += v[k];
    }
}

template <typename TIn>
static int exclusive_scan(hipStream_t st, const TIn *in, int64_t *out, int64_t n, int64_t *h_total) {
    XM_ARG(n >= 0);
    XM_SCOPE(st);
    int64_t n_tiles = (n + SCAN_TILE - 1) / SCAN_TILE;
    long long *tile = nullptr;
    XM_HIP(xm_malloc_async((void **)&tile, sizeof(long long) * (size_t)(n_tiles + 1), st));
    if (n_tiles > 0) {
        k_tile_sums<TIn><<<dim3((unsigned)n_tiles), dim3(SCAN_THREADS), 0, st>>>(in, n, tile);
        XM_LAUNCH_CHECK();
    }
    k_scan_tile_sums<<<dim3(1), dim3(SCAN_THREADS), 0, st>>>(tile, n_tiles, (long long *)(out + n));
    XM_LAUNCH_CHECK();
    if (n_tiles > 0) {
        k_tile_scan<TIn><<<dim3((unsigned)n_tiles), dim3(SCAN_THREADS), 0, st>>>(in, n, tile, (long long *)out);
        XM_LAUNCH_CHECK();
    }
    XM_HIP(xm_free_async(tile, st));
    if (h_total) {
        XM_HIP(hipMemcpyAsync(h_total, out + n, sizeof(int64_t), hipMemcpyDeviceToHost, st));
        XM_HIP(hipStreamSynchronize(st));
    }
    return XMAP_OK;
}
}

extern "C" {
const char *xmap_last_error(void) { return xmap::g_err; }
int xmap_version(void) { return 113; }

int xmap_trim(void) {
    XM_HIP(hipDeviceSynchronize());
    int dev = 0;
    XM_HIP(hipGetDevice(&dev));
    for (xmap::Arena &a : xmap::g_arenas) {
        if (a.dev != dev || a.live != 0) continue;
        for (xmap::Chunk &c : a.chunks) (void)hipFree(c.base);
        a.chunks.clear();
    }
    return XMAP_OK;
}

int xmap_debug_arena(void *stream, int64_t *live, int64_t *reserved) {
    XM_ARG(live && reserved);
    int dev = 0;
    XM_HIP(hipGetDevice(&dev));
    *live = 0; *reserved = 0;
    if (xmap::Arena *a = xmap::arena_find(dev, (hipStream_t)stream)) {
        *live = (int64_t)a->live;
        for (xmap::Chunk &c : a->chunks) *reserved += (int64_t)c.size;
    }
    return XMAP_OK;
}
int xmap_debug_arena_call(void *stream, int64_t bytes, int fail) {
    using namespace xmap;
    XM_SCOPE(stream);
    hipStream_t st = (hipStream_t)stream;
    void *a = nullptr, *b = nullptr;
    XM_HIP(xm_malloc_async(&a, (size_t)bytes, st));
    XM_HIP(xm_malloc_async(&b, 1024, st));
    XM_ARG(!fail);
    XM_HIP(xm_free_async(b, st));
    XM_HIP(xm_free_async(a, st));
    return XMAP_OK;
}

int xmap_exclusive_scan_i64(void *stream, const int64_t *in, int64_t *out, int64_t n, int64_t *h_total) {
    return xmap::exclusive_scan<long long>((hipStream_t)stream, (const long long *)in, out, n, h_total);
}
int xmap_exclusive_scan_i32_to_i64(void *stream, const int32_t *in, int64_t *out, int64_t n, int64_t *h_total) {
    return xmap::exclusive_scan<int>((hipStream_t)stream, in, out, n, h_total);
}
}
```

### x-map_amd/xmap/engine/device.py

```python
import ctypes as C
import os

import numpy as np
import torch

from . import hipabi as abi
from .exactness import plain_sums_exact

lib = abi.lib
vp, i32, i64, check = abi.vp, abi.i32, abi.i64, abi.check


def _stream(dev):
    return C.c_void_p(torch.cuda.current_stream(dev).cuda_stream)


SLOT_TARGET = 768
CH_MIN = 2048


class DeviceRatings(object):

    def __init__(self, user_ptr, item, rating, time, n_items, attrs, device="cuda:0", rating64=False):
        self.device = torch.device(device)
        user_ptr = np.ascontiguousarray(user_ptr, np.int64)
        item = np.ascontiguousarray(item, np.int32)
        if user_ptr.ndim != 1 or len(user_ptr) < 1:
            raise ValueError("user_ptr must hold n_users + 1 entries")
        prefix_cls, suffix_cls = [np.ascontiguousarray(a, np.int32) for a in attrs[:2]]
        if len(prefix_cls) != int(n_items) or len(suffix_cls) != int(n_items) or len(item) < max(int(user_ptr[-1]), 0):
            raise ValueError("prefix_cls / suffix_cls must hold n_items entries, item user_ptr[-1]")
        if abi.lib.xmap_check_ratings(len(user_ptr) - 1, int(n_items), user_ptr.ctypes.data, item.ctypes.data, prefix_cls.ctypes.data,
                                      suffix_cls.ctypes.data, 1 if rating64 else 0):
            raise ValueError((abi.lib.xmap_last_error() or b"").decode())
        r64 = np.ascontiguousarray(rating, np.float64) if rating64 else None
        rating = np.ascontiguousarray(rating, np.float32)
        time = np.ascontiguousarray(time, np.int64)
        self.n_users = len(user_ptr) - 1
        self.n_items = int(n_items)
        self.nnz = int(user_ptr[-1])
        self.plain_exact = plain_sums_exact(rating[:self.nnz], self.n_users)
        d = np.diff(user_ptr)
        self.half_contrib = int((d * (d - 1) // 2).sum())
        contains_mask, flags = attrs[2:]
        d = self.device
        t = torch.from_numpy
        self.user_ptr = t(user_ptr).to(d)
        self.user_item = t(item).to(d)
        self.user_rating = t(rating).to(d)
        self.user_rating64 = t(r64).to(d) if r64 is not None else None
        self.user_time = t(time).to(d)
        self.item_ptr = torch.zeros(self.n_items + 1, dtype=torch.int64, device=d)
        self.item_user = torch.zeros(max(self.nnz, 1), dtype=torch.int32, device=d)
        self.item_rating = torch.zeros(max(self.nnz, 1), dtype=torch.float32, device=d)
        self.csc_ready = False
        self.prefix_cls = t(prefix_cls).to(d)
        self.suffix_cls = t(suffix_cls).to(d)
        self.contains_mask = t(np.ascontiguousarray(contains_mask, np.uint32).view(np.int32)).to(d)
        self.flags = t(np.ascontiguousarray(flags, np.uint8)).to(d)
        self.c = abi.Ratings(self.n_users, self.n_items, self.nnz,
                             self.user_ptr.data_ptr(), self.user_item.data_ptr(), self.user_rating.data_ptr(),
                             self.user_time.data_ptr(), self.item_ptr.data_ptr(), self.item_user.data_ptr(),
                             self.item_rating.data_ptr(), self.prefix_cls.data_ptr(), self.suffix_cls.data_ptr(),
                             self.contains_mask.data_ptr(), self.flags.data_ptr())

    def bytes_resident(self):
        return sum(x.numel() * x.element_size() for x in (
            self.user_ptr, self.user_item, self.user_rating, self.user_time, self.item_ptr,
            self.item_user, self.item_rating))


# ... 15 lines not shown

class _Timed(object):

    def __init__(self, eng, name):
        self.eng, self.name = eng, name

    def __enter__(self):
        if self.eng.timers is not None:
            self.a = torch.cuda.Event(enable_timing=True)
            self.b = torch.cuda.Event(enable_timing=True)
            self.a.record(torch.cuda.current_stream(self.eng.dev))
        return self

    def __exit__(self, *exc):
        if self.eng.timers is not None:
            self.b.record(torch.cuda.current_stream(self.eng.dev))
            self.eng.timers.setdefault(self.name, []).append((self.a, self.b))
        return False


class Engine(object):
    def __init__(self, ratings):
        self.R = ratings
        self.dev = ratings.device
        self.timers = None
        self._scratch = {}

    def _zero_scratch(self, name, numel, dtype):
        t = self._scratch.get(name)
        if t is None or t.numel() < numel or t.dtype != dtype:
            t = torch.zeros(numel, dtype=dtype, device=self.dev)
            self._scratch[name] = t
        return t

    def hbm_available(self, *own):
        free, _ = torch.cuda.mem_get_info(self.dev)
        cached = torch.cuda.memory_reserved(self.dev) - torch.cuda.memory_allocated(self.dev)
        held = sum(t.numel() * t.element_size() for n, t in self._scratch.items() if n in own)
        return int(free + max(cached, 0) + held)

    def _drop_scratch(self, *names):
        for n in names:
            self._scratch.pop(n, None)

    def timed(self, name):
        return _Timed(self, name)

    def timer_ms(self):
        torch.cuda.synchronize(self.dev)
        return {k: [a.elapsed_time(b) for a, b in v] for k, v in (self.timers or {}).items()}

    def _empty(self, shape, dtype):
        return torch.empty(shape, dtype=dtype, device=self.dev)

    def _out(self, shape, dtype, written):
        return self._empty(shape, dtype) if written else self._zeros(shape, dtype)

    def _zeros(self, shape, dtype):
        return torch.zeros(shape, dtype=dtype, device=self.dev)

    def pair_method(self, method):
        m = abi.METHODS[method] if isinstance(method, str) else int(method)
        return abi.COSINE_EXACT if (m == abi.COSINE and not self.R.plain_exact) else m

    def build_csc(self):
        R = self.R
        st = _stream(self.dev)
        cnt = self._empty(max(R.n_items, 1), torch.int32)
        with self.timed("build_csc"):
            check(lib.xmap_build_csc(st, i64(R.n_users), i32(R.n_items), i64(R.nnz), vp(R.user_ptr), vp(R.user_item),
                                     vp(R.user_rating), vp(cnt), vp(R.item_ptr), vp(R.item_user), vp(R.item_rating)))
        R.csc_ready = True

    def stats(self, packed=False, item_range=None):
        R = self.R
        st = _stream(self.dev)
        self.build_csc()
        u_avg = self._empty(max(R.n_users, 1), torch.float64)
        u_norm = self._empty(max(R.n_users, 1), torch.float64)
        check(lib.xmap_user_stats(st, C.byref(R.c), vp(u_avg), vp(u_norm)))
        info = self._out((max(R.n_items, 1), 4), torch.float64, R.n_items > 0)
        self.norms = self._out(2 * max(R.n_items, 1), torch.float64, R.n_items > 0)
        ua_item = self._empty(max(R.nnz, 1), torch.int32) if packed else None
        ia_user = self._empty(max(R.nnz, 1), torch.int32) if packed else None
        lo, hi = (0, R.n_items) if item_range is None else (int(item_range[0]), int(item_range[1]))
        if packed:
            abi.xcheck(abi.xlib().xmap_item_stats(st, C.byref(R.c), vp(u_avg), vp(info), vp(self.norms), vp(ua_item), vp(ia_user), i32(lo), i32(hi)))
        else:
            check(lib.xmap_item_stats(st, C.byref(R.c), vp(u_avg), vp(info), vp(self.norms), vp(ua_item), vp(ia_user), i32(lo), i32(hi)))
        return u_avg, u_norm, info, ua_item, ia_user

    def stats_partial(self):
        R = self.R
        st = _stream(self.dev)
        self.build_csc()
        u_avg = self._empty(max(R.n_users, 1), torch.float64)
        u_norm = self._empty(max(R.n_users, 1), torch.float64)
        check(lib.xmap_user_stats(st, C.byref(R.c), vp(u_avg), vp(u_norm)))
        partial = self._out((max(R.n_items, 1), 7), torch.float64, R.n_items > 0)
        check(lib.xmap_item_partials(st, C.byref(R.c), vp(u_avg), vp(partial)))
        return u_avg, u_norm, partial

    def stats_merge(self, parts):
        I = self.R.n_items
        parts = parts.contiguous()
        info = self._out((max(I, 1), 4), torch.float64, I > 0)
# ... 150 lines not shown
                                       i32(1 if dups else 0), h_ctl))
        L.CH, L.n_heavy = int(h_ctl[0]), int(h_ctl[1])
        L.slot_target = slot_target
        self._tri_plan(L, slot_target)
        both = torch.stack([L.Wp[:I].sum(), L.Wp[L.hlist[:L.n_heavy].long()].sum()]).tolist() if I else [0, 0]
        L.half_contrib, L.heavy_half = int(both[0]), int(both[1])
        return L

    def _layout_buffers(self, dups, wide=False):
        I, U, nnz = self.R.n_items, self.R.n_users, self.R.nnz
        n1, i1 = max(nnz, 1), max(I, 1)
        L = SimResult()
        L.hist = self._empty(U + 2, torch.int32)
        L.pre = self._empty(U + 3, torch.int64)
        L.ctl = self._empty(4, torch.int32)
        L.hid = self._empty(i1, torch.int32)
        L.hlist = self._zeros(1024, torch.int32)
        L.ub_key = self._empty(n1, torch.int64)
        L.ub = self._empty(n1 * (2 if wide else 1), torch.int64)
        L.rc = self._empty(n1 * 2, torch.int64)
        L.Wp = self._empty(i1, torch.int64)
        L.dups = bool(dups)
        return L

    def _plan_buffers(self, L):
        I = self.R.n_items
        L.Q = self._out(max(I, 1), torch.int32, I > 0)
        L.C = self._out(max(I, 1), torch.int32, I > 0)
        L.small = self._out(max(I, 1), torch.uint8, I > 0)
        L.Qcat = self._empty(5 * max(I, 1), torch.int32)
        L.uq_ptr = self._out(5 * I + 1, torch.int64, I > 0)
        L.uc_ptr = self._out(I + 1, torch.int64, I > 0)

    def _tri_plan(self, L, slot_target):
        R = self.R
        st = _stream(self.dev)
        I = R.n_items
        self._plan_buffers(L)
        h = (C.c_int64 * 8)()
        with self.timed("tri_plan"):
            check(lib.xmap_sim2_plan(st, C.byref(R.c), i32(slot_target), vp(L.rc), vp(L.pre), vp(L.hid),
                                     vp(L.ctl), vp(L.Q), vp(L.C), vp(L.small), vp(L.Wp), vp(L.Qcat), vp(L.uq_ptr),
                                     vp(L.uc_ptr), i32(1 if getattr(L, "dups", False) else 0), h))
            L.n_light, L.n_heavy_units = int(h[0]), int(h[1])
            L.cls_ptr = (C.c_int64 * 6)(*[int(h[2 + c]) for c in range(6)])
            L.uq_item = self._empty(max(L.n_light, 1), torch.int32)
            L.uq_q = self._empty(4 * max(L.n_light, 1), torch.int32)
            L.uc_item = self._empty(max(L.n_heavy_units, 1), torch.int32)
            L.uc_c = self._empty(max(L.n_heavy_units, 1), torch.int32)
            check(lib.xmap_sim2_units(st, i32(I), vp(R.item_ptr), vp(L.Qcat), vp(L.uq_ptr), vp(L.uq_item), vp(L.uq_q),
                                      vp(L.C), vp(L.uc_ptr), vp(L.uc_item), vp(L.uc_c)))
        L.slot_target = slot_target

    def _tri_plan3(self, L, slot_target):
        R = self.R
        st = _stream(self.dev)
        I = R.n_items
        self._plan_buffers(L)
        cap_light = L.half_contrib // max(int(slot_target), 1) + I + 1
        cap_heavy = R.nnz // max(int(L.ch_min), 1) + 1025
        L.uq_item = self._empty(cap_light, torch.int32)
        L.uq_q = self._empty(4 * cap_light, torch.int32)
        L.uc_item = self._empty(cap_heavy, torch.int32)
        L.uc_c = self._empty(cap_heavy, torch.int32)
        h = (C.c_int64 * 10)()
        with self.timed("tri_plan"):
            check(lib.xmap_sim3_plan(st, C.byref(R.c), i32(slot_target), vp(L.pre), vp(L.hid), vp(L.ctl), vp(L.Q), vp(L.C),
                                     vp(L.small), vp(L.Wp), vp(L.Qcat), vp(L.uq_ptr), vp(L.uc_ptr),
                                     i32(1 if getattr(L, "dups", False) else 0), vp(L.uq_item), vp(L.uq_q), vp(L.uc_item),
                                     vp(L.uc_c), i64(cap_light), i64(cap_heavy), h))
        L.n_light, L.n_heavy_units = int(h[0]), int(h[1])
        L.cls_ptr = (C.c_int64 * 6)(*[int(h[2 + c]) for c in range(6)])
        L.CH, L.n_heavy = int(h[8]), int(h[9])
        L.slot_target = slot_target
        L.replan = self._tri_plan3

    def heavy_half(self, L):
        if getattr(L, "_heavy_half", None) is None:
            L._heavy_half = int(L.Wp[L.hlist[:L.n_heavy].long()].sum().item()) if L.n_heavy else 0
        return L._heavy_half

    def tri_pairs(self, method, cap, stats, L, unit_range=None, do_heavy=True, retry=True, rec=False, raw=False, split=False,
                  heavy_deal=None, marks=True, count_mir=False):
        R = self.R
        st = _stream(self.dev)
        m = self.pair_method(method)
        u_avg, u_norm, info, _, _ = stats
        I = R.n_items
        coo_slack = 1.0
        while True:
            lo, hi = (0, L.n_light) if unit_range is None else (int(unit_range[0]), int(unit_range[1]))
            cap_coo = (max(int(L.half_contrib * coo_slack), 1) // 4096 + 1100) * 4096
            coo_i = self._empty(cap_coo, torch.int32)
            coo_j = self._empty(cap_coo, torch.int32)
            coo_sim = self._empty(cap_coo, torch.float64)
            coo_mutu = self._empty(cap_coo, torch.int32)
            coo_nij = self._empty(cap_coo, torch.int32)
            coo_ls = self._empty(cap_coo, torch.float64) if (rec or raw) else None
            rowcnt = self._empty(max(I, 1), torch.int32)
            mircnt = self._empty(max(I, 1), torch.int32) if split else None
            nh = L.n_heavy_units if do_heavy else 0
            hp_hi = self._empty(max(nh, 1) * 1024, torch.float64)
            hp_lo = self._empty(max(nh, 1) * 1024, torch.float64)
            hp_cnt = self._empty(max(nh, 1) * 1024, torch.int32)
            hp_mut = self._empty(max(nh, 1) * 1024, torch.int32)
            d_cnt = self._zeros(6, torch.int64)
            d_shards = self._empty(2 * 4096, torch.int64)

            deal = 0 if heavy_deal is None else abi.pairs_deal(heavy_deal[1], heavy_deal[0])
            heavy, merge = (abi.PAIRS_HEAVY, abi.PAIRS_HEAVY_MERGE) if do_heavy else (0, 0)
            light = abi.PAIRS_LIGHT | (abi.PAIRS_RAW if raw else 0)

            def run(phases):
                phases |= deal | (0 if marks else abi.PAIRS_NO_MARKS)
                check(lib.xmap_sim2_pairs(
                    st, C.byref(R.c), m, int(cap), vp(u_avg), vp(self.norms), vp(L.rc), vp(L.ub), vp(L.Q), vp(L.small),
                    vp(L.uq_item),
                    vp(L.uq_q), L.cls_ptr, i64(lo), i64(hi), vp(L.hid), vp(L.hlist), vp(L.ctl), vp(L.C), vp(L.uc_ptr),
                    vp(L.uc_item), vp(L.uc_c), i32(nh), i32(L.n_heavy), phases,
                    vp(hp_hi), vp(hp_lo), vp(hp_cnt), vp(hp_mut), i64(cap_coo), vp(coo_i), vp(coo_j), vp(coo_sim),
                    vp(coo_mutu), vp(coo_nij), vp(coo_ls), vp(rowcnt), vp(d_shards), vp(d_cnt), vp(mircnt)))
            if os.environ.get("XMAP_SPLIT_PHASES") == "1":
                with self.timed("pair_heavy"):
                    run(abi.PAIRS_RESET | heavy)
                with self.timed("pair_tri"):
                    run(light)
                with self.timed("heavy_merge"):
                    run(merge | abi.PAIRS_MIRCOUNT)
            else:
                with self.timed("pair_tri"):
                    run(abi.PAIRS_RESET | heavy | light | merge | abi.PAIRS_MIRCOUNT | abi.PAIRS_SHARD_SUMS)
            if count_mir and split and not raw:
                with self.timed("mir_count"):
                    scratch = self._empty(cap_coo, torch.int32)
                    check(lib.xmap_sim3_mircount(st, i32(I), i64(cap_coo), vp(coo_i), vp(coo_j), vp(d_shards), i64(cap_coo),
                                                 i32(1 if rec else 0), vp(scratch), vp(mircnt)))
            h = d_cnt.tolist()
            if h[2]:
                if L.slot_target <= 32:
                    raise abi.XmapError(abi.ERR_OVERFLOW, "pair-table overflow")
                if not retry:
                    return (None, rowcnt, 0, 0) + ((None, None) if split else ()) + (1,)
                getattr(L, "replan", self._tri_plan)(L, L.slot_target // 2)
                continue
            if h[3]:
                if coo_slack > 64:
                    raise abi.XmapError(abi.ERR_CAPACITY, "half-COO overflow")
                coo_slack *= 2
                continue
            break
        if os.environ.get("XMAP_SPLIT_PHASES") == "1":
            h[4:6] = d_shards.view(2, 4096).sum(dim=1).tolist()
        n, n_unordered = int(h[4]), int(h[5])
        coo = (coo_i, coo_j, coo_sim, coo_mutu, coo_nij) + ((coo_ls,) if (rec or raw) else ())
        out = (coo, rowcnt, n, n_unordered)
        if split:
            return out + (mircnt, d_shards) + (() if retry else (0,))
        return out if retry else out + (0,)

    def tri_scatter(self, coo, rowcnt, info, n=None, L=None):
        R = self.R
        st = _stream(self.dev)
        I = R.n_items
        coo_i, coo_j, coo_sim, coo_mutu, coo_nij = [x.contiguous() for x in coo[:5]]
        coo_ls = coo[5].contiguous() if len(coo) > 5 else None
        n_scan = int(coo_i.numel())
        if n is None:
            n = n_scan
        row_ptr = self._out(I + 1, torch.int64, I > 0)
        tot = C.c_int64(0)
        check(lib.xmap_exclusive_scan_i32_to_i64(st, vp(rowcnt), vp(row_ptr), i64(I), C.byref(tot) if coo_ls is not None else None))
        kept = 2 * n if coo_ls is None else int(tot.value)
        ls = self._empty(max(kept, 1), torch.float64) if coo_ls is not None else None
        col = self._empty(max(kept, 1), torch.int32)
        sim = self._empty(max(kept, 1), torch.float64)
        mutu = self._empty(max(kept, 1), torch.int32)
        nij = self._empty(max(kept, 1), torch.int32)
        fill = self._empty(max(I, 1), torch.int32)
        with self.timed("scatter"):
          if n:
            check(lib.xmap_sim2_scatter(st, i32(I), i64(n_scan), vp(coo_i), vp(coo_j), vp(coo_sim), vp(coo_mutu),
                                        vp(coo_nij), vp(coo_ls), vp(row_ptr), vp(fill), vp(L.hid), vp(L.hlist), vp(col),
                                        vp(sim), vp(mutu), vp(nij), vp(ls)))
        S = self.sim_from_device(row_ptr, col[:kept], sim[:kept], mutu[:kept], nij[:kept], info)
        S.ls = ls[:kept] if ls is not None else None
        return S

    def rec_sim(self, cap, slot_target=SLOT_TARGET):
        R = self.R
        with self.timed("rec_stats"):
            stats, L = self.layout3(slot_target, ch_min=max(64, R.n_users + 2), wide=True)
        S, n_unordered = self._pairs_to_csr("adjust_cosine", cap, stats, L, rec=True)
        S.cap, S.n_unordered, S.layout = int(cap), n_unordered, L
        S.norm = self.norms[R.n_items:2 * R.n_items]
        return S

    def rec_select(self, S, keep):
        st = _stream(self.dev)
        I = self.R.n_items
        cnt = self._zeros(max(I, 1), torch.int32)
        col = self._empty((max(I, 1), keep), torch.int32)
        sim = self._empty((max(I, 1), keep), torch.float64)
        ls = self._empty((max(I, 1), keep), torch.float64)
        with self.timed("rec_select"):
            check(lib.xmap_rec_select(st, i32(I), vp(S.row_ptr), vp(S.col), vp(S.sim), vp(S.ls), i32(keep), vp(cnt),
                                      vp(col), vp(sim), vp(ls)))
        return cnt[:I], col[:I], sim[:I], ls[:I]

    def layout3(self, slot_target=SLOT_TARGET, ch_min=CH_MIN, wide=False, item_range=None):
        R = self.R
        st = _stream(self.dev)
        I, U, nnz = R.n_items, R.n_users, R.nnz
        n1, i1 = max(nnz, 1), max(I, 1)
        rw = 3 if wide else 2
        L = self._layout_buffers(wide, wide)
        cnt = self._empty(i1, torch.int32)
        u_avg = self._zeros(max(U, 1), torch.float64) if wide else self._empty(max(U, 1), torch.float64)
        u_norm = None if wide else self._empty(max(U, 1), torch.float64)
        srec = self._empty(n1 * rw, torch.int64)
        buf_a = self._empty(n1 * rw, torch.int64)
        buf_b = self._empty(n1 * rw, torch.int64)
        L.wide = bool(wide)
        info = self._out((i1, 4), torch.float64, I > 0)
        self.norms = self._out(2 * i1, torch.float64, I > 0)
        r64 = None
        if wide:
            r64 = R.user_rating64 if R.user_rating64 is not None else R.user_rating.double()
        def call(phases, lo, hi):
            check(lib.xmap_sim3_layout(st, C.byref(R.c), vp(R.item_ptr), vp(r64), i32(ch_min), i32(phases), i32(lo), i32(hi), vp(cnt),
                                       vp(u_avg), vp(u_norm), vp(L.hist), vp(L.pre), vp(L.ctl), vp(L.hid), vp(L.hlist),
                                       vp(L.ub_key), vp(L.ub), vp(srec), vp(buf_a), vp(buf_b), vp(L.rc), vp(L.Wp), vp(info),
                                       vp(self.norms), None))
        R.csc_ready = False
        L.ch_min = int(ch_min)
        L.half_contrib = R.half_contrib
        if item_range is None:
            with self.timed("layout3"):
                call(abi.LAYOUT_RECORDS | abi.LAYOUT_STATS | abi.LAYOUT_UB_FLAGS, 0, I)
            self._tri_plan3(L, slot_target)
        else:
            with self.timed("layout3"):
                call(abi.LAYOUT_RECORDS | abi.LAYOUT_STATS, int(item_range[0]), int(item_range[1]))

            def finish():
                with self.timed("layout3_flags"):
                    call(abi.LAYOUT_UB_FLAGS | abi.LAYOUT_RC_FLAGS, 0, I)
                self._tri_plan3(L, slot_target)
            L.finish = finish
        return (u_avg, u_norm, info, None, None), L

    def mir_counts(self, coo, n, mir, shards=None, skip_self=False):
        I = self.R.n_items
        scratch = self._empty(max(int(n), 1), torch.int32)
        check(lib.xmap_sim3_mircount(_stream(self.dev), i32(I), i64(int(coo[0].numel())), vp(coo[0].contiguous()), vp(coo[1].contiguous()),
                                     vp(shards), i64(n), i32(1 if skip_self else 0), vp(scratch), vp(mir)))
        return mir

    def tri_mirror(self, coo, own, mir, info, n, shards=None, rows=None, counted=False):
        R = self.R
        st = _stream(self.dev)
        I = R.n_items
        coo_i, coo_j, coo_sim, coo_mutu, coo_nij = [x.contiguous() for x in coo[:5]]
        coo_ls = coo[5].contiguous() if len(coo) > 5 else None
        cap = int(coo_i.numel())
        kept = 2 * int(n)
        lo, hi = (0, I) if rows is None else (int(rows[0]), int(rows[1]))
        if rows is not None and I > 0:
            own = own.clone()
            own[:lo].zero_(); own[hi:].zero_()
            if counted:
                mir = mir.clone()
                mir[:lo].zero_(); mir[hi:].zero_()
                kept = int((own[lo:hi].long().sum() + mir[lo:hi].long().sum()).item())
        rw = 4 if coo_ls is not None else 3
        row_ptr = self._out(I + 1, torch.int64, I > 0)
        mptr = self._empty(I + 1, torch.int64)
        tot = self._empty(max(I, 1), torch.int32)
        fill = self._empty(max(I, 1), torch.int32)
        buf_a = self._empty(max(int(n), 1) * rw, torch.int64)
        buf_b = self._empty(max(int(n), 1) * rw, torch.int64)
        col = self._empty(max(kept, 1), torch.int32)
        sim = self._empty(max(kept, 1), torch.float64)
        mutu = self._empty(max(kept, 1), torch.int32)
        nij = self._empty(max(kept, 1), torch.int32)
        ls = self._empty(max(kept, 1), torch.float64) if coo_ls is not None else None
        with self.timed("scatter"):
            if not counted:
                check(lib.xmap_sim3_mircount(st, i32(I), i64(cap), vp(coo_i), vp(coo_j), vp(shards), i64(n), i32(1 if coo_ls is not None else 0),
                                             vp(buf_a), vp(mir)))
                if rows is not None and I > 0:
                    mir[:lo].zero_(); mir[hi:].zero_()
                    kept = int((own[lo:hi].long().sum() + mir[lo:hi].long().sum()).item())
            check(lib.xmap_sim3_mirror(st, i32(I), i64(cap), vp(coo_i), vp(coo_j), vp(coo_sim), vp(coo_mutu), vp(coo_nij), vp(shards), i64(n),
                                       vp(own), vp(mir), vp(tot), vp(row_ptr), vp(mptr), vp(fill), vp(buf_a), vp(buf_b), vp(col),
                                       vp(sim), vp(mutu), vp(nij), vp(coo_ls), vp(ls), i32(lo), i32(hi)))
        if coo_ls is not None:
            kept = int(row_ptr[I].item()) if I > 0 else 0
        S = self.sim_from_device(row_ptr, col[:kept], sim[:kept], mutu[:kept], nij[:kept], info)
        S.ls = ls[:kept] if ls is not None else None
        return S

    def _pairs_to_csr(self, method, cap, stats, L, rec=False):
        if os.environ.get("XMAP_A_V2") == "1":
            coo, rowcnt, n, n_unordered = self.tri_pairs(method, cap, stats, L, do_heavy=not rec, rec=rec)
            return self.tri_scatter(coo, rowcnt, stats[2], n, L), n_unordered
        coo, own, n, n_unordered, mir, shards = self.tri_pairs(method, cap, stats, L, do_heavy=not rec, rec=rec, split=True,
                                                               marks=False, count_mir=True)
        return self.tri_mirror(coo, own, mir, stats[2], n, shards, counted=True), n_unordered

    def item_sim_tri(self, method, cap, slot_target=SLOT_TARGET, ch_min=CH_MIN):
        if os.environ.get("XMAP_A_V2") == "1":
            with self.timed("stats"):
                stats = self.stats()
            L = self.tri_layout(stats, slot_target, ch_min)
        else:
            stats, L = self.layout3(slot_target, ch_min)
        S, n_unordered = self._pairs_to_csr(method, cap, stats, L)
        S.method = abi.METHODS[method] if isinstance(method, str) else int(method)
        S.cap = int(cap)
        S.u_avg, S.u_norm = stats[0], stats[1]
        S.n_eval, S.n_contrib = 2 * n_unordered, 2 * L.half_contrib
        S.n_units, S.layout, S.slot_target = L.n_light + L.n_heavy_units, L, L.slot_target
        return S

    def sim_from_device(self, row_ptr, col, sim, mutu, nij, info):
        S = SimResult()
        S.n_items = self.R.n_items
        n = int(col.numel())
        if n == 0:
            col = self._zeros(1, torch.int32); sim = self._zeros(1, torch.float64)
            mutu = self._zeros(1, torch.int32); nij = self._zeros(1, torch.int32)
        S.row_ptr, S.info = row_ptr.contiguous(), info
        col, sim, mutu, nij = col.contiguous(), sim.contiguous(), mutu.contiguous(), nij.contiguous()
        S.col, S.sim, S.mutu, S.nij = col[:n], sim[:n], mutu[:n], nij[:n]
        S.n_kept = n
        S.c = abi.Sim(S.n_items, S.row_ptr.data_ptr(), col.data_ptr(), sim.data_ptr(), mutu.data_ptr(),
                      nij.data_ptr(), info.data_ptr())
        S._keep = (col, sim, mutu, nij)
        return S

    def sim_from_host(self, row_ptr, col, sim, mutu, nij, info, frac=None):
        d = self.dev
        n = int(row_ptr[-1])

        def up(a, dt):
            return torch.from_numpy(np.ascontiguousarray(a if n else np.zeros(1), dt)).to(d)
        row_ptr_d = torch.from_numpy(np.ascontiguousarray(row_ptr, np.int64)).to(d)
        info_d = torch.from_numpy(np.ascontiguousarray(info, np.float64)).to(d)
        S = self.sim_from_device(row_ptr_d, up(col, np.int32)[:n], up(sim, np.float64)[:n], up(mutu, np.int32)[:n],
                                 up(nij if nij is not None else np.zeros(max(n, 1)), np.int32)[:n], info_d)
        if frac is not None:
            S.frac = up(frac, np.float64)
            S.c.frac = S.frac.data_ptr()
        return S

    def knn(self, S, top_k, bb=None, rows=None):
        R = self.R
        st = _stream(self.dev)
        I, k = R.n_items, int(top_k)
        E = ExtResult()
        E.k = k
        if bb is not None:
            E.bb = bb.to(torch.uint8).contiguous()
        else:
            E.bb = self._zeros(max(I, 1), torch.uint8)
            check(lib.xmap_bridge_flags(st, C.byref(S.c), vp(R.prefix_cls), vp(E.bb)))
        alloc = self._empty if I > 0 else self._zeros
        E.cls = alloc(max(I, 1), torch.uint8)
        E.kcnt = alloc((max(I, 1), 2), torch.int32)
# ... 1018 lines not shown
```

### x-map_amd/xmap/engine/hipabi.py

```python
import ctypes as C
import os

HERE = os.path.dirname(os.path.abspath(__file__))
LIB_PATH = os.environ.get("XMAP_HIP_LIB") or os.path.normpath(os.path.join(HERE, "..", "..", "libxmap_hip.so"))
XLIB_PATH = os.environ.get("XMAP_HIP_XLIB") or os.path.normpath(os.path.join(HERE, "..", "..", "libxmap_hip_xcheck.so"))

COSINE, ADJUST_COSINE = 0, 1
METHODS = {"cosine": COSINE, "adjust_cosine": ADJUST_COSINE}
COSINE_EXACT = 2
TOPC = 10
MID_ROWS_SPAN = 36864
ERR_HIP, ERR_ARG, ERR_OVERFLOW, ERR_CAPACITY = -1, -2, -3, -4
TOPN_KEEP_HELD = 1
AUDIENCE_KEEP_HOLDERS = 1
SRC_RESIDENT, SRC_FOLDIN, SRC_ITEM_FOLDIN = 0, 1, 2
GROUP_MEAN, GROUP_MIN, GROUP_MAX = 0, 1, 2
GROUP_MAX_MEMBERS = 64
GROUP_HOW = {"mean": GROUP_MEAN, "min": GROUP_MIN, "max": GROUP_MAX}
UNION_DISTINCT = 1
UNION_MAX_PARTS = 16
EXPLAIN_MAX_EV, EXPLAIN_MAX_SRC = 16, 8
PAIRS_HEAVY, PAIRS_LIGHT, PAIRS_HEAVY_MERGE, PAIRS_RESET = 1, 2, 4, 8
PAIRS_MIRCOUNT, PAIRS_RAW, PAIRS_SHARD_SUMS, PAIRS_NO_MARKS = 16, 32, 64, 128
LAYOUT_RECORDS, LAYOUT_STATS, LAYOUT_UB_FLAGS, LAYOUT_RC_FLAGS, LAYOUT_ALL = 1, 2, 4, 8, 15
# ... 10 lines not shown


class Ratings(C.Structure):
    _fields_ = [("n_users", C.c_int64), ("n_items", C.c_int32), ("nnz", C.c_int64),
                ("user_ptr", C.c_void_p), ("user_item", C.c_void_p), ("user_rating", C.c_void_p),
                ("user_time", C.c_void_p), ("item_ptr", C.c_void_p), ("item_user", C.c_void_p),
                ("item_rating", C.c_void_p), ("prefix_cls", C.c_void_p), ("suffix_cls", C.c_void_p),
                ("contains_mask", C.c_void_p), ("flags", C.c_void_p)]


class Sim(C.Structure):
    _fields_ = [("n_items", C.c_int32), ("row_ptr", C.c_void_p), ("col", C.c_void_p), ("sim", C.c_void_p),
                ("mutu", C.c_void_p), ("nij", C.c_void_p), ("info", C.c_void_p), ("frac", C.c_void_p)]


class ExtTables(C.Structure):
    _fields_ = [("n_items", C.c_int32), ("top_k", C.c_int32),
                ("cls", C.c_void_p), ("kcnt", C.c_void_p), ("kcol", C.c_void_p), ("kval", C.c_void_p), ("flags", C.c_void_p),
                ("att_ptr", C.c_void_p), ("att_idx", C.c_void_p), ("att_val", C.c_void_p),
                ("src_ptr", C.c_void_p), ("src_idx", C.c_void_p), ("src_val", C.c_void_p), ("src_flag", C.c_void_p),
                ("rnn_ptr", C.c_void_p), ("rnn_idx", C.c_void_p), ("rnn_val", C.c_void_p),
                ("n_nb", C.c_int32), ("nb_id", C.c_void_p), ("nb_list", C.c_void_p), ("midX", C.c_void_p), ("dir", C.c_void_p),
                ("dir_ptr", C.c_void_p),
                ("n_ends", C.c_int32), ("urank", C.c_void_p), ("uitem", C.c_void_p)]


class UnionPart(C.Structure):
    _fields_ = [("n_users", C.c_int64), ("n_items", C.c_int32), ("n_rows", C.c_int64), ("n_target_rows", C.c_int64),
                ("user", C.c_void_p), ("item", C.c_void_p), ("rating", C.c_void_p), ("time", C.c_void_p),
                ("off_t", C.c_void_p), ("off_m", C.c_void_p), ("user_map", C.c_void_p), ("item_map", C.c_void_p)]


class PathUnits(C.Structure):
    _fields_ = [("n_units", C.c_int32), ("unit_start", C.c_void_p), ("unit_c", C.c_void_p), ("unit_G", C.c_void_p),
                ("unit_row", C.c_void_p), ("unit_nt", C.c_void_p), ("n_heavy", C.c_int32), ("heavy_unit0", C.c_void_p)]


class PathRows(C.Structure):
    _fields_ = [("n_slots", C.c_int32), ("acc", C.c_void_p), ("touched", C.c_void_p), ("hacc", C.c_void_p),
                ("htouched", C.c_void_p)]


class PathOut(C.Structure):
    _fields_ = [("n_cand", C.c_void_p), ("top_end", C.c_void_p), ("top_val", C.c_void_p), ("xs_cap", C.c_int64),
                ("xs_off", C.c_void_p), ("xs_end", C.c_void_p), ("xs_val", C.c_void_p)]


class RecFilter(C.Structure):
    _fields_ = [("allow", C.c_void_p), ("ex_ptr", C.c_void_p), ("ex_id", C.c_void_p), ("min_score", C.c_double)]


EXPORTS = [
    "xmap_last_error", "xmap_version", "xmap_trim", "xmap_debug_arena", "xmap_debug_arena_call", "xmap_exclusive_scan_i64", "xmap_exclusive_scan_i32_to_i64",
    "xmap_build_csc", "xmap_user_stats", "xmap_item_stats", 
    "xmap_sim2_layout", "xmap_sim2_plan", "xmap_sim2_units",
    "xmap_sim2_pairs", "xmap_sim2_scatter", "xmap_sim3_layout", "xmap_sim3_plan", "xmap_sim3_mircount", "xmap_sim3_mirror", "xmap_item_partials", "xmap_item_merge", "xmap_sim2_pack_partials",
    "xmap_sim2_sort_partials", "xmap_sim2_merge_partials", "xmap_sim2_pack_pairs", "xmap_sim2_unpack_pairs", "xmap_bridge_flags", "xmap_knn_classify", "xmap_knn_thresholds", "xmap_reverse_count", "xmap_reverse_count_att_rnn",
    "xmap_reverse_fill", "xmap_topc_from_lists", "xmap_path_weights", "xmap_extend_paths", 
    "xmap_mid_rows_count", "xmap_mid_rows_place", "xmap_edge_ranges", "xmap_end_universe", "xmap_extend_cols", "xmap_extend_cols_slots", "xmap_nb_index", "xmap_path_plan", "xmap_end_order", "xmap_dense_normalize", "xmap_dense_layout", "xmap_dense_topk", "xmap_rec_select", "xmap_predict", "xmap_rec_profiles", "xmap_predict_rows", "xmap_mae", "xmap_topn_rows", "xmap_audience_rows", "xmap_explain_rows", "xmap_explain_sources", "xmap_eval_users", "xmap_topn_eval", "xmap_select_map", "xmap_alterego_count", "xmap_alterego_fill", "xmap_foldin_count", "xmap_foldin_fill", "xmap_union_count", "xmap_union_fill",
    "xmap_feed_text", "xmap_feed_texts", "xmap_feed_merge", "xmap_feed_sizes", "xmap_feed_arrays", "xmap_feed_ids", "xmap_feed_free",
    "xmap_ctx_upload_feed", "xmap_feed_format", "xmap_ctx_create", "xmap_ctx_destroy", "xmap_check_ratings", "xmap_ctx_upload_ratings", "xmap_ctx_item_sim", "xmap_ctx_sim_download", "xmap_ctx_extend",
    "xmap_ctx_ext_download", "xmap_ctx_ext_lists", "xmap_ctx_candidates", "xmap_ctx_generate", "xmap_ctx_gen_download",
    "xmap_ctx_rec_sim", "xmap_ctx_rec_profiles_download", "xmap_ctx_rec_download", "xmap_ctx_rec_select", "xmap_ctx_rec_set_neighbors",
    "xmap_ctx_rec_neighbors_download", "xmap_ctx_predict", "xmap_ctx_recommend", "xmap_ctx_evaluate_topn",
    "xmap_ctx_foldin", "xmap_ctx_foldin_download", "xmap_ctx_foldin_recommend", "xmap_ctx_foldin_predict", "xmap_ctx_union",
    "xmap_ctx_explain", "xmap_ctx_foldin_explain", "xmap_ctx_audience", "xmap_ctx_foldin_audience",
    "xmap_itemfold_count", "xmap_itemfold_fill", "xmap_itemfold_audience_rows", "xmap_ctx_item_foldin", "xmap_ctx_item_foldin_download",
    "xmap_ctx_item_foldin_audience", "xmap_ctx_item_foldin_predict", "xmap_ctx_item_foldin_recommend",
    "xmap_topn_rows_filtered", "xmap_audience_rows_filtered", "xmap_ctx_recommend_filtered", "xmap_ctx_audience_filtered",
    "xmap_div_index", "xmap_diversify_rows", "xmap_ctx_recommend_diverse",
    "xmap_group_topn_rows", "xmap_ctx_recommend_group",
]

if not os.path.exists(LIB_PATH):
    raise ImportError("libxmap_hip.so not built (%s); the MI355X engine has no CPU fallback" % LIB_PATH)
lib = C.CDLL(LIB_PATH)
lib.xmap_last_error.restype = C.c_char_p
for _n in EXPORTS:
    getattr(lib, _n)
XCHECK_EXPORTS = ["xmap_sim_plan", "xmap_sim_units", "xmap_sim_count", "xmap_sim_fill", "xmap_sim_row_ptr", "xmap_extend_paths2",
                  "xmap_mid_tally", "xmap_mid_place"]

HEADER_PATH = os.path.normpath(os.path.join(HERE, "..", "..", "..", "include", "xmap_hip.h"))


def header_prototypes(path=HEADER_PATH):
    import re
    with open(path) as f:
        text = f.read()
    text = re.sub(r"#\s*ifdef\s+XMAP_CROSSCHECK[^\n]*\n", "\n", text)
    text = re.sub(r"/\*.*?\*/", " ", text, flags=re.S)
    text = re.sub(r"//[^\n]*", " ", text)
    out = {}
    for m in re.finditer(r"\b(?:int|void|const\s+char\s*\*)\s*(xmap_\w+)\s*\(([^;{]*?)\)\s*;", text, flags=re.S):
        name, args = m.group(1), " ".join(m.group(2).split())
        types = []
        for a in ([] if args in ("", "void") else args.split(",")):
            if "*" in a:
                types.append(C.c_void_p)
            elif "int64_t" in a:
                types.append(C.c_int64)
            elif "double" in a:
                types.append(C.c_double)
            elif "float" in a:
                types.append(C.c_float)
            else:
# ... 84 lines not shown
```

Before: 24.84 billion.

## Overlap host waits with GPU work and batch memsets in item-sim pipeline

Splits plan and pair-counter readbacks into begin/wait halves that use events and pinned host slots. This lets the UB-flags layout pass and the mirror count kernel be queued while the host waits, instead of after a full stream sync. Several memsets are merged into a single multi-fill launch, and the Qcat zeroing memset is replaced by writes inside the planning kernel. Mirror and pair buffers are preallocated and reused across stages. In exchange, mircount now runs over the full COO capacity before overflow is known, which can waste work on retries.

```diff
diff --git a/include/xmap_hip.h b/include/xmap_hip.h
--- a/include/xmap_hip.h
+++ b/include/xmap_hip.h
@@ -44,6 +44,9 @@
 
 int xmap_exclusive_scan_i64(void *stream, const int64_t *in, int64_t *out, int64_t n, int64_t *h_total);
 int xmap_exclusive_scan_i32_to_i64(void *stream, const int32_t *in, int64_t *out, int64_t n, int64_t *h_total);
+int xmap_exclusive_scan2_i32_to_i64(void *stream, const int32_t *in_a, const int32_t *in_b, int32_t a_plus_b, int64_t *out_a,
+                                    int64_t *out_b, int64_t n, int64_t *h_totals);
+int xmap_scan_self_tiles(void);
 
 
 int xmap_build_csc(void *stream, int64_t n_users, int32_t n_items, int64_t nnz, const int64_t *user_ptr,
@@ -133,6 +136,13 @@
                    const int32_t *ctl, int32_t *Q, int32_t *C, uint8_t *small, uint64_t *Wp, int32_t *Qcat ,
                    int64_t *uq_ptr , int64_t *uc_ptr , int32_t dups, int32_t *uq_item, int32_t *uq_q ,
                    int32_t *uc_item, int32_t *uc_c, int64_t cap_light, int64_t cap_heavy, int64_t *h_out );
+int xmap_sim3_plan_begin(void *stream, const xmap_ratings *R, int32_t slot_target, const int64_t *pre, const int32_t *hid,
+                         const int32_t *ctl, int32_t *Q, int32_t *C, uint8_t *small, uint64_t *Wp, int32_t *Qcat ,
+                         int64_t *uq_ptr , int64_t *uc_ptr , int32_t dups, int32_t *uq_item, int32_t *uq_q ,
+                         int32_t *uc_item, int32_t *uc_c, int64_t cap_light, int64_t cap_heavy);
+int xmap_sim3_plan_wait(int64_t cap_light, int64_t cap_heavy, int64_t *h_out );
+int xmap_sim3_counters_begin(void *stream, const int64_t *d_counters );
+int xmap_sim3_counters_wait(int64_t *h_out );
 int xmap_sim3_mircount(void *stream, int32_t n_items, int64_t coo_cap, const int32_t *coo_i, const int32_t *coo_j,
                        const int64_t *d_shards , int64_t n_pairs, int32_t skip_self, void *scratch, int32_t *mir );
 int xmap_sim3_mirror(void *stream, int32_t n_items, int64_t coo_cap, const int32_t *coo_i, const int32_t *coo_j,
diff --git a/x-map_amd/csrc/api.hip b/x-map_amd/csrc/api.hip
--- a/x-map_amd/csrc/api.hip
+++ b/x-map_amd/csrc/api.hip
@@ -244,7 +244,7 @@
     T_ALLOC(hist, U + 2); T_ALLOC(pre, U + 3); T_ALLOC(ctl, 4); T_ALLOC(hid, i1); T_ALLOCZ(hlist, 1024);
     T_ALLOC(ub_key, n1); T_ALLOC(ub, (wide ? 2 : 1) * n1); T_ALLOC(rcrec, 2 * n1); T_ALLOC(Wp, i1);
     T_ALLOC(srec, rw * n1); T_ALLOC(buf_a, rw * n1); T_ALLOC(buf_b, rw * n1);
-    XM_TRY(xmap_sim3_layout(st, &R, (int64_t *)R.item_ptr, J.rating64, J.ch_min, XMAP_LAYOUT_RECORDS | XMAP_LAYOUT_STATS | XMAP_LAYOUT_UB_FLAGS,
+    XM_TRY(xmap_sim3_layout(st, &R, (int64_t *)R.item_ptr, J.rating64, J.ch_min, XMAP_LAYOUT_RECORDS | XMAP_LAYOUT_STATS,
                             0, I, cnt, O.u_avg, O.u_norm, hist, pre, ctl, hid, hlist, ub_key, ub, srec, buf_a, buf_b, rcrec, Wp, O.info,
                             O.norms, nullptr));
     int32_t *Q, *Cc, *Qcat, *uq_item = nullptr, *uq_q = nullptr, *uc_item = nullptr, *uc_c = nullptr;
@@ -255,13 +255,17 @@
     int slot_target = 768;
     double coo_slack = 1.0;
     int64_t hc[10];
-    auto plan = [&](int target) -> int {
+    auto plan = [&](int target, bool ub_flags) -> int {
         const int64_t cap_light = J.half_contrib / target + I + 1, cap_heavy = nnz / J.ch_min + 1025;
         T_ALLOC(uq_item, cap_light); T_ALLOC(uq_q, 4 * cap_light); T_ALLOC(uc_item, cap_heavy); T_ALLOC(uc_c, cap_heavy);
-        return xmap_sim3_plan(st, &R, target, pre, hid, ctl, Q, Cc, small, Wp, Qcat, uq_ptr, uc_ptr, J.dups, uq_item, uq_q, uc_item, uc_c,
-                              cap_light, cap_heavy, hc);
+        XM_TRY(xmap_sim3_plan_begin(st, &R, target, pre, hid, ctl, Q, Cc, small, Wp, Qcat, uq_ptr, uc_ptr, J.dups, uq_item, uq_q, uc_item, uc_c,
+                                    cap_light, cap_heavy));
+        if (ub_flags && !wide)
+            XM_TRY(xmap_sim3_layout(st, &R, (int64_t *)R.item_ptr, J.rating64, J.ch_min, XMAP_LAYOUT_UB_FLAGS, 0, I, cnt, O.u_avg, O.u_norm, hist,
+                                    pre, ctl, hid, hlist, ub_key, ub, srec, buf_a, buf_b, rcrec, Wp, O.info, O.norms, nullptr));
+        return xmap_sim3_plan_wait(cap_light, cap_heavy, hc);
     };
-    XM_TRY(plan(slot_target));
+    XM_TRY(plan(slot_target, true));
     const int phases = XMAP_PAIRS_RESET | XMAP_PAIRS_LIGHT | XMAP_PAIRS_MIRCOUNT | XMAP_PAIRS_SHARD_SUMS | XMAP_PAIRS_NO_MARKS |
                        (J.heavy ? XMAP_PAIRS_HEAVY | XMAP_PAIRS_HEAVY_MERGE : 0);
     int32_t *coo_i = nullptr, *coo_j = nullptr, *coo_mutu = nullptr, *coo_nij = nullptr, *own = nullptr, *mir = nullptr;
@@ -284,12 +288,15 @@
                                ctl, Cc, uc_ptr, uc_item, uc_c, (int32_t)n_hu, (int32_t)n_heavy, phases, hp_hi, hp_lo, hp_cnt, hp_mut, cap_coo, coo_i,
                                coo_j, coo_sim, coo_mutu, coo_nij, coo_aux, own, d_shards, d_cnt, mir));
         int64_t h_cnt[6];
-        XM_TRY(d2h(h_cnt, d_cnt, 6, st));
-        XM_HIP(hipStreamSynchronize(st));
+        int32_t *mir_part;
+        T_ALLOC(mir_part, cap_coo);
+        XM_TRY(xmap_sim3_counters_begin(st, d_cnt));
+        XM_TRY(xmap_sim3_mircount(st, I, cap_coo, coo_i, coo_j, d_shards, cap_coo, J.skip_self ? 1 : 0, mir_part, mir));
+        XM_TRY(xmap_sim3_counters_wait(h_cnt));
         if (h_cnt[2]) {
             if (slot_target <= 32) { set_error("pair-table overflow"); return XMAP_ERR_OVERFLOW; }
             slot_target /= 2;
-            XM_TRY(plan(slot_target));
+            XM_TRY(plan(slot_target, false));
             continue;
         }
         if (h_cnt[3]) {
@@ -311,7 +318,6 @@
     XM_TRY(dalloc(*J.mutu_pool, &O.mutu, (size_t)O.kept, st)); XM_TRY(dalloc(*J.csr_pool, &O.nij, (size_t)O.kept, st));
     if (J.aux) XM_TRY(dalloc(*J.csr_pool, &O.aux, (size_t)O.kept, st));
     T_ALLOC(fill, i1); T_ALLOC(tot, i1); T_ALLOC(mir_a, (J.aux ? 4 : 3) * nn); T_ALLOC(mir_b, (J.aux ? 4 : 3) * nn);
-    XM_TRY(xmap_sim3_mircount(st, I, cap_coo, coo_i, coo_j, d_shards, n, J.skip_self ? 1 : 0, mir_a, mir));
     return xmap_sim3_mirror(st, I, cap_coo, coo_i, coo_j, coo_sim, coo_mutu, coo_nij, d_shards, n, own, mir, tot, J.row_ptr, mptr, fill, mir_a,
                             mir_b, O.col, O.sim, O.mutu, O.nij, coo_aux, O.aux, 0, I);
 #undef T_ALLOC
diff --git a/x-map_amd/csrc/common.h b/x-map_amd/csrc/common.h
--- a/x-map_amd/csrc/common.h
+++ b/x-map_amd/csrc/common.h
@@ -42,6 +42,22 @@
     XmScope &operator=(const XmScope &) = delete;
 };
 #define XM_SCOPE(stream) xmap::XmScope xm_scope_((hipStream_t)(stream))
+constexpr int HW_SLOTS = 2, HW_WORDS = 16;
+constexpr int HW_PLAN = 0, HW_PAIRS = 1;
+struct HostWait { int dev; int64_t *h; hipEvent_t ev[HW_SLOTS]; bool pending[HW_SLOTS]; };
+HostWait *host_wait();
+int host_wait_post(hipStream_t st, int slot, const void *d_src, int words);
+int host_wait_take(int slot, const int64_t **h);
+struct FillList {
+    enum { MAX = 8 };
+    void *p[MAX]; unsigned long long words[MAX]; unsigned val[MAX]; int n;
+    FillList() : n(0) {}
+    void add(void *ptr, size_t bytes, unsigned v = 0u) {
+        if (n >= MAX) { n = MAX + 1; return; }
+        p[n] = ptr; words[n] = bytes / 4; val[n] = v; n++;
+    }
+};
+int fill_multi(hipStream_t st, const FillList &F);
 int radix_sort_pairs(hipStream_t st, unsigned long long *keys, int *vals, unsigned long long *keys_tmp, int *vals_tmp, long long n,
                      int bits);
 
diff --git a/x-map_amd/csrc/tri.h b/x-map_amd/csrc/tri.h
--- a/x-map_amd/csrc/tri.h
+++ b/x-map_amd/csrc/tri.h
@@ -30,9 +30,9 @@
 constexpr int COO_SHARDS = 4096;
 
 int mirror_counts(hipStream_t st, int n_items, long long range_cap, int n_ranges, const unsigned long long *cur, const int *coo_i,
-                  const int *coo_j, bool skip_self, int *part, int *counts);
+                  const int *coo_j, bool skip_self, int *part, int *counts, FillList *fills = nullptr);
 void ts_geometry(int K, long long M, int ch, ts::Geo &G);
-int ts_prepare(hipStream_t st, ts::Geo &G, const long long *ptr);
+int ts_prepare(hipStream_t st, ts::Geo &G, const long long *ptr, FillList *fills = nullptr);
 extern template __global__ void ts::k_ts_bin<3, true, ts::RecLoader<3>>(ts::Geo, ts::RecLoader<3>, long long, unsigned long long *__restrict__);
 
 }
diff --git a/x-map_amd/csrc/tri_layout.hip b/x-map_amd/csrc/tri_layout.hip
--- a/x-map_amd/csrc/tri_layout.hip
+++ b/x-map_amd/csrc/tri_layout.hip
@@ -208,7 +208,9 @@
                     : ((q != 1) ? 0 : (bound <= SMALL_BOUND ? 1 : (bound <= 2 * SMALL_BOUND ? 3 : (bound <= MID_BOUND ? 2 : 0))));
     small[i] = (uint8_t)cls;
     Wp[i] = (unsigned long long)w;
-    Qcat[(size_t)class_rank(cls) * I + i] = q;
+    const int rank = class_rank(cls);
+#pragma unroll
+    for (int r = 0; r < N_CLASSES; r++) Qcat[(size_t)r * I + i] = (r == rank) ? q : 0;
 }
 
 __global__ __launch_bounds__(256) void k_plan2(int I, const long long *iptr, const RaterRec *rc, const long long *pre,
@@ -221,8 +223,15 @@
 
 __global__ __launch_bounds__(256) void k_fill_units2(int I, const long long *iptr, const int *Qcat, const long long *uq_ptr,
                                                      int *uq_item, int *uq_q, const int *C, const long long *uc_ptr, int *uc_item,
-                                                     int *uc_c, long long cap_light, long long cap_heavy) {
+                                                     int *uc_c, long long cap_light, long long cap_heavy, const int *ctl,
+                                                     long long *counts) {
     const long long x = (long long)blockIdx.x * blockDim.x + threadIdx.x;
+    if (counts && x == 0) {
+        for (int c = 0; c <= N_CLASSES; c++) counts[2 + c] = uq_ptr[(long long)c * I];
+        counts[0] = uq_ptr[(long long)N_CLASSES * I];
+        counts[1] = uc_ptr[I];
+        counts[8] = ctl[0]; counts[9] = ctl[1];
+    }
     if (x >= (long long)N_CLASSES * I) return;
     const int i = (int)(x % I);
     long long b = uq_ptr[x];
@@ -598,13 +607,21 @@
 
 namespace {
 
+void heavy_set_fills(FillList &F, int64_t n_users, int32_t *hist, int32_t *ctl) {
+    F.add(hist, sizeof(int32_t) * (size_t)(n_users + 2));
+    F.add(ctl, sizeof(int32_t), 0x7f7f7f7fu);
+    F.add(ctl + 1, 3 * sizeof(int32_t));
+}
 int heavy_set(void *stream, int I, int64_t n_users, const int64_t *item_ptr, int32_t ch_min, int32_t *hist, int64_t *pre, int32_t *ctl,
-              int32_t *hid, int32_t *hlist) {
+              int32_t *hid, int32_t *hlist, bool filled = false) {
     hipStream_t st = (hipStream_t)stream;
     const int HB = (int)n_users + 2;
-    XM_HIP(hipMemsetAsync(hist, 0, sizeof(int32_t) * (size_t)HB, st));
-    XM_HIP(hipMemsetAsync(ctl, 0x7f, sizeof(int32_t), st));
-    XM_HIP(hipMemsetAsync(ctl + 1, 0, 3 * sizeof(int32_t), st));
+    if (!filled) {
+        FillList F;
+        heavy_set_fills(F, n_users, hist, ctl);
+        int rc = fill_multi(st, F);
+        if (rc) return rc;
+    }
     if (I > 0) {
         k_hist<<<dim3((unsigned)((I + 256 * HIST_PER - 1) / (256 * HIST_PER))), dim3(256), 0, st>>>(I, (const long long *)item_ptr, HB, hist);
         XM_LAUNCH_CHECK();
@@ -638,7 +655,6 @@
     XM_ARG(slot_target > 0 && slot_target <= T_SLOTS);
     hipStream_t st = (hipStream_t)stream;
     const int I = R->n_items;
-    XM_HIP(hipMemsetAsync(Qcat, 0, sizeof(int32_t) * (size_t)N_CLASSES * (size_t)(I > 0 ? I : 1), st));
     if (I > 0) {
         k_plan2<<<dim3((unsigned)((I + 255) / 256)), dim3(256), 0, st>>>(
             I, (const long long *)R->item_ptr, (const RaterRec *)rc, (const long long *)pre, (int)R->n_users + 2, hid, ctl, slot_target, dups,
@@ -743,8 +759,47 @@
     if (n_items == 0) return XMAP_OK;
     k_fill_units2<<<dim3((unsigned)(((long long)N_CLASSES * n_items + 255) / 256)), dim3(256), 0, (hipStream_t)stream>>>(
         n_items, (const long long *)item_ptr, Qcat, (const long long *)uq_ptr, uq_item, uq_q, C, (const long long *)uc_ptr, uc_item, uc_c, 0x7fffffffffffffffLL,
-        0x7fffffffffffffffLL);
+        0x7fffffffffffffffLL, nullptr, nullptr);
     XM_LAUNCH_CHECK();
+    return XMAP_OK;
+}
+
+int xmap_sim3_plan_begin(void *stream, const xmap_ratings *R, int32_t slot_target, const int64_t *pre, const int32_t *hid,
+                         const int32_t *ctl, int32_t *Q, int32_t *C, uint8_t *small, uint64_t *Wp, int32_t *Qcat, int64_t *uq_ptr,
+                         int64_t *uc_ptr, int32_t dups, int32_t *uq_item, int32_t *uq_q, int32_t *uc_item, int32_t *uc_c,
+                         int64_t cap_light, int64_t cap_heavy) {
+    XM_SCOPE(stream);
+    XM_ARG(R && Wp && pre && hid && ctl && Q && C && small && Qcat && uq_ptr && uc_ptr);
+    XM_ARG(uq_item && uq_q && uc_item && uc_c && cap_light >= 0 && cap_heavy >= 0);
+    hipStream_t st = (hipStream_t)stream;
+    const int I = R->n_items;
+    int rcode = plan_rows(stream, R, slot_target, nullptr, pre, hid, ctl, Q, C, small, Wp, Qcat, uq_ptr, uc_ptr, dups, nullptr, nullptr);
+    if (rcode) return rcode;
+    long long *counts = nullptr;
+    XM_HIP(xm_malloc_async((void **)&counts, sizeof(long long) * 10, st));
+    const long long threads = (long long)N_CLASSES * I > 0 ? (long long)N_CLASSES * I : 1;
+    k_fill_units2<<<dim3((unsigned)((threads + 255) / 256)), dim3(256), 0, st>>>(
+        I, (const long long *)R->item_ptr, Qcat, (const long long *)uq_ptr, uq_item, uq_q, C, (const long long *)uc_ptr, uc_item, uc_c,
+        cap_light, cap_heavy, ctl, counts);
+    XM_LAUNCH_CHECK();
+    return host_wait_post(st, HW_PLAN, counts, 10);
+}
+
+int xmap_sim3_plan_wait(int64_t cap_light, int64_t cap_heavy, int64_t *h_out) {
+    XM_ARG(h_out);
+    const int64_t *h = nullptr;
+    int rcode = host_wait_take(HW_PLAN, &h);
+    if (rcode) return rcode;
+    for (int c = 0; c < 10; c++) h_out[c] = h[c];
+    if (h_out[9] > HMAX) {
+        set_error("heavy set larger than %d", HMAX);
+        return XMAP_ERR_OVERFLOW;
+    }
+    if (h_out[0] > cap_light || h_out[1] > cap_heavy) {
+        set_error("unit arrays too small: %lld light / %lld heavy units, room for %lld / %lld", (long long)h_out[0], (long long)h_out[1],
+                  (long long)cap_light, (long long)cap_heavy);
+        return XMAP_ERR_CAPACITY;
+    }
     return XMAP_OK;
 }
 
@@ -752,34 +807,12 @@
                    const int32_t *ctl, int32_t *Q, int32_t *C, uint8_t *small, uint64_t *Wp, int32_t *Qcat, int64_t *uq_ptr,
                    int64_t *uc_ptr, int32_t dups, int32_t *uq_item, int32_t *uq_q, int32_t *uc_item, int32_t *uc_c,
                    int64_t cap_light, int64_t cap_heavy, int64_t *h_out) {
-    XM_SCOPE(stream);
-    XM_ARG(R && Wp && pre && hid && ctl && Q && C && small && Qcat && uq_ptr && uc_ptr && h_out);
-    XM_ARG(uq_item && uq_q && uc_item && uc_c && cap_light >= 0 && cap_heavy >= 0);
-    hipStream_t st = (hipStream_t)stream;
-    const int I = R->n_items;
+    XM_ARG(h_out);
     for (int c = 0; c < 10; c++) h_out[c] = 0;
-    int rcode = plan_rows(stream, R, slot_target, nullptr, pre, hid, ctl, Q, C, small, Wp, Qcat, uq_ptr, uc_ptr, dups, nullptr, nullptr);
+    int rcode = xmap_sim3_plan_begin(stream, R, slot_target, pre, hid, ctl, Q, C, small, Wp, Qcat, uq_ptr, uc_ptr, dups, uq_item, uq_q, uc_item,
+                                     uc_c, cap_light, cap_heavy);
     if (rcode) return rcode;
-    if (I > 0) {
-        k_fill_units2<<<dim3((unsigned)(((long long)N_CLASSES * I + 255) / 256)), dim3(256), 0, st>>>(
-            I, (const long long *)R->item_ptr, Qcat, (const long long *)uq_ptr, uq_item, uq_q, C, (const long long *)uc_ptr, uc_item, uc_c,
-            cap_light, cap_heavy);
-        XM_LAUNCH_CHECK();
-        XM_HIP(hipMemcpy2DAsync(&h_out[2], sizeof(int64_t), uq_ptr, sizeof(int64_t) * (size_t)I, sizeof(int64_t), N_CLASSES + 1,
-                                hipMemcpyDeviceToHost, st));
-        XM_HIP(hipMemcpyAsync(&h_out[1], uc_ptr + I, sizeof(int64_t), hipMemcpyDeviceToHost, st));
-    }
-    int32_t h_ctl[2] = {0, 0};
-    rcode = read_heavy_ctl(st, ctl, h_ctl);
-    h_out[0] = h_out[2 + N_CLASSES];
-    h_out[8] = h_ctl[0]; h_out[9] = h_ctl[1];
-    if (rcode) return rcode;
-    if (h_out[0] > cap_light || h_out[1] > cap_heavy) {
-        set_error("unit arrays too small: %lld light / %lld heavy units, room for %lld / %lld", (long long)h_out[0], (long long)h_out[1],
-                  (long long)cap_light, (long long)cap_heavy);
-        return XMAP_ERR_CAPACITY;
-    }
-    return XMAP_OK;
+    return xmap_sim3_plan_wait(cap_light, cap_heavy, h_out);
 }
 
 int xmap_sim3_layout(void *stream, const xmap_ratings *R, int64_t *item_ptr, const double *rating64, int32_t ch_min, int32_t phases,
@@ -798,16 +831,35 @@
     const bool wide = rating64 != nullptr;
     const size_t In = (size_t)(I > 0 ? I : 1);
     int rcode = XMAP_OK;
+    const bool stats = (phases & XMAP_LAYOUT_STATS) && stats_hi > stats_lo;
+    BigList B;
+    bool b_cleared = false;
+    if (stats) {
+        B.chunk_cap = nnz / STAT_CHK + nnz / STAT_BIG + 2;
+        B.item_cap = nnz / STAT_BIG + 2;
+        XM_HIP(xm_malloc_async((void **)&B.counters, 2 * sizeof(unsigned), st));
+        XM_HIP(xm_malloc_async((void **)&B.chunks, sizeof(int2) * (size_t)B.chunk_cap, st));
+        XM_HIP(xm_malloc_async((void **)&B.items, sizeof(int4) * (size_t)B.item_cap, st));
+        XM_HIP(xm_malloc_async((void **)&B.part, sizeof(double) * ITEM_PART * (size_t)B.chunk_cap, st));
+    }
     if (phases & XMAP_LAYOUT_RECORDS) {
-        XM_HIP(hipMemsetAsync(cnt, 0, sizeof(int32_t) * In, st));
+        FillList F;
+        F.add(cnt, sizeof(int32_t) * In);
+        heavy_set_fills(F, R->n_users, hist, ctl);
+        F.add(Wp, sizeof(uint64_t) * In);
+        if (stats) { F.add(B.counters, 2 * sizeof(unsigned)); b_cleared = true; }
         const char *cb_env = getenv("XMAP_COUNT_PART_MIN");
         const long long cb_min = cb_env ? atoll(cb_env) : 2000000ll;
         if (nnz >= cb_min && I > 0) {
-            rcode = mirror_counts(st, I, nnz, 1, nullptr, nullptr, R->user_item, false, (int *)bufA, cnt);
+            rcode = mirror_counts(st, I, nnz, 1, nullptr, nullptr, R->user_item, false, (int *)bufA, cnt, &F);
             if (rcode) return rcode;
-        } else if (nnz > 0) {
-            k_count3<<<dim3((unsigned)((nnz + CNT_CHUNK - 1) / CNT_CHUNK)), dim3(256), 0, st>>>(nnz, R->user_item, cnt);
-            XM_LAUNCH_CHECK();
+        } else {
+            rcode = fill_multi(st, F);
+            if (rcode) return rcode;
+            if (nnz > 0) {
+                k_count3<<<dim3((unsigned)((nnz + CNT_CHUNK - 1) / CNT_CHUNK)), dim3(256), 0, st>>>(nnz, R->user_item, cnt);
+                XM_LAUNCH_CHECK();
+            }
         }
         rcode = xmap_exclusive_scan_i32_to_i64(stream, cnt, item_ptr, I, nullptr);
         if (rcode) return rcode;
@@ -815,7 +867,7 @@
             rcode = xmap_user_stats(stream, R, u_avg, u_norm);
             if (rcode) return rcode;
         }
-        rcode = heavy_set(stream, I, R->n_users, item_ptr, ch_min, hist, pre, ctl, hid, hlist);
+        rcode = heavy_set(stream, I, R->n_users, item_ptr, ch_min, hist, pre, ctl, hid, hlist, true);
         if (rcode) return rcode;
         if (R->n_users > 0 && nnz > 0) {
             const dim3 grid((unsigned)((R->n_users + 15) / 16));
@@ -824,7 +876,6 @@
                 (unsigned long long *)ub_key, ub, (unsigned long long *)srec);
             XM_LAUNCH_CHECK();
         }
-        XM_HIP(hipMemsetAsync(Wp, 0, sizeof(uint64_t) * In, st));
         if (nnz > 0 && I > 0) {
             ts::Geo G;
             ts_geometry(I, nnz, wide ? ts::Chunk<3>::CH : ts::Chunk<2>::CH, G);
@@ -835,15 +886,8 @@
             if (rcode) return rcode;
         }
     }
-    if ((phases & XMAP_LAYOUT_STATS) && stats_hi > stats_lo) {
-        BigList B;
-        B.chunk_cap = nnz / STAT_CHK + nnz / STAT_BIG + 2;
-        B.item_cap = nnz / STAT_BIG + 2;
-        XM_HIP(xm_malloc_async((void **)&B.counters, 2 * sizeof(unsigned), st));
-        XM_HIP(xm_malloc_async((void **)&B.chunks, sizeof(int2) * (size_t)B.chunk_cap, st));
-        XM_HIP(xm_malloc_async((void **)&B.items, sizeof(int4) * (size_t)B.item_cap, st));
-        XM_HIP(xm_malloc_async((void **)&B.part, sizeof(double) * ITEM_PART * (size_t)B.chunk_cap, st));
-        XM_HIP(hipMemsetAsync(B.counters, 0, 2 * sizeof(unsigned), st));
+    if (stats) {
+        if (!b_cleared) XM_HIP(hipMemsetAsync(B.counters, 0, 2 * sizeof(unsigned), st));
         rcode = wide ? item_stats3(st, I, stats_lo, stats_hi, item_ptr, RcWideSrc{(const RaterRecWide *)rc}, info, norms, B)
                      : item_stats3(st, I, stats_lo, stats_hi, item_ptr, RcSrc{(RaterRec *)rc, u_avg}, info, norms, B);
         if (rcode) return rcode;
diff --git a/x-map_amd/csrc/tri_mirror.hip b/x-map_amd/csrc/tri_mirror.hip
--- a/x-map_amd/csrc/tri_mirror.hip
+++ b/x-map_amd/csrc/tri_mirror.hip
@@ -209,10 +209,6 @@
     }
 }
 
-__global__ __launch_bounds__(256) void k_row_totals(int I, const int *own, const int *mir, int *tot) {
-    const int i = blockIdx.x * blockDim.x + threadIdx.x;
-    if (i < I) tot[i] = own[i] + mir[i];
-}
 
 template <bool AUX, bool SHARE>
 struct CooLoaderT {
@@ -430,7 +426,7 @@
     }
 }
 
-int ts_prepare(hipStream_t st, ts::Geo &G, const long long *ptr) {
+int ts_prepare(hipStream_t st, ts::Geo &G, const long long *ptr, FillList *fills) {
     G.ptr = ptr;
     G.clist_cap = G.M / G.ch + G.NA + 1;
     G.slist_cap = G.M / ts::SL + (G.M >> G.ts_log) + 2;
@@ -443,8 +439,12 @@
     G.curA = z; G.curB = z + G.NA; G.counters = (unsigned *)(z + G.NA + 2 * (size_t)G.T);
     XM_HIP(xm_malloc_async((void **)&G.clist, sizeof(int2) * (size_t)G.clist_cap, st));
     XM_HIP(xm_malloc_async((void **)&G.slist, sizeof(int2) * (size_t)G.slist_cap, st));
-    XM_HIP(hipMemsetAsync(z, 0, sizeof(unsigned long long) * nz, st));
-    XM_HIP(hipMemsetAsync(G.tile_large, 0xff, sizeof(int) * (size_t)G.T, st));
+    FillList own;
+    FillList &F = fills ? *fills : own;
+    F.add(z, sizeof(unsigned long long) * nz);
+    F.add(G.tile_large, sizeof(int) * (size_t)G.T, 0xffffffffu);
+    int rcode = fill_multi(st, F);
+    if (rcode) return rcode;
     ts::k_ts_plan<<<dim3((unsigned)((G.K + 255) / 256)), dim3(256), 0, st>>>(G);
     XM_LAUNCH_CHECK();
     ts::k_ts_chunks<<<dim3((unsigned)((G.NA + 255) / 256)), dim3(256), 0, st>>>(G);
@@ -477,8 +477,10 @@
 }
 
 int mirror_counts(hipStream_t st, int n_items, long long range_cap, int n_ranges, const unsigned long long *cur, const int *coo_i,
-                  const int *coo_j, bool skip_self, int *part, int *counts) {
-    if (n_items <= 0 || range_cap <= 0 || n_ranges <= 0) return XMAP_OK;
+                  const int *coo_j, bool skip_self, int *part, int *counts, FillList *fills) {
+    FillList own;
+    FillList &F = fills ? *fills : own;
+    if (n_items <= 0 || range_cap <= 0 || n_ranges <= 0) return fill_multi(st, F);
     int sh = 0;
     while (((long long)(n_items - 1) >> sh) >= CB_MAX) sh++;
     unsigned *bcnt = nullptr, *bcur = nullptr;
@@ -486,7 +488,9 @@
     XM_HIP(xm_malloc_async((void **)&bcnt, sizeof(unsigned) * CB_MAX, st));
     XM_HIP(xm_malloc_async((void **)&bcur, sizeof(unsigned) * CB_MAX, st));
     XM_HIP(xm_malloc_async((void **)&bptr, sizeof(long long) * (CB_MAX + 1), st));
-    XM_HIP(hipMemsetAsync(bcnt, 0, sizeof(unsigned) * CB_MAX, st));
+    F.add(bcnt, sizeof(unsigned) * CB_MAX);
+    int rcode = fill_multi(st, F);
+    if (rcode) return rcode;
     const long long segs = (long long)n_ranges * ((range_cap + CB_CHUNK - 1) / CB_CHUNK);
     const dim3 g((unsigned)((segs + CB_SPB - 1) / CB_SPB));
     (skip_self ? k_cbs_hist<true> : k_cbs_hist<false>)<<<g, dim3(CB_T), 0, st>>>(range_cap, n_ranges, cur, coo_i, coo_j, sh, bcnt);
@@ -532,10 +536,11 @@
     XM_ARG(d_shards ? (coo_cap >= COO_SHARDS) : (n_pairs <= coo_cap));
     hipStream_t st = (hipStream_t)stream;
     if (n_items == 0) return XMAP_OK;
-    XM_HIP(hipMemsetAsync(mir, 0, sizeof(int32_t) * (size_t)n_items, st));
-    if (n_pairs == 0 || coo_cap == 0) return XMAP_OK;
+    FillList F;
+    F.add(mir, sizeof(int32_t) * (size_t)n_items);
+    if (n_pairs == 0 || coo_cap == 0) return fill_multi(st, F);
     return mirror_counts(st, n_items, d_shards ? coo_cap / COO_SHARDS : n_pairs, d_shards ? COO_SHARDS : 1,
-                         (const unsigned long long *)d_shards, coo_i, coo_j, skip_self != 0, (int *)scratch, mir);
+                         (const unsigned long long *)d_shards, coo_i, coo_j, skip_self != 0, (int *)scratch, mir, &F);
 }
 
 int xmap_sim3_mirror(void *stream, int32_t n_items, int64_t coo_cap, const int32_t *coo_i, const int32_t *coo_j,
@@ -551,20 +556,11 @@
     XM_ARG((coo_aux != nullptr) == (aux != nullptr));
     hipStream_t st = (hipStream_t)stream;
     const int I = n_items;
-    if (I > 0) {
-        k_row_totals<<<dim3((unsigned)((I + 255) / 256)), dim3(256), 0, st>>>(I, own, mir, tot);
-        XM_LAUNCH_CHECK();
-    }
-    int rcode = xmap_exclusive_scan_i32_to_i64(stream, tot, row_ptr, I, nullptr);
-    if (rcode) return rcode;
-    rcode = xmap_exclusive_scan_i32_to_i64(stream, mir, mptr, I, nullptr);
+    int rcode = xmap_exclusive_scan2_i32_to_i64(stream, own, mir, 1, row_ptr, mptr, I, nullptr);
     if (rcode) return rcode;
     if (n_pairs == 0 || I == 0 || coo_cap == 0) return XMAP_OK;
-    XM_HIP(hipMemsetAsync(fill, 0, sizeof(int32_t) * (size_t)I, st));
     ts::Geo G;
     ts_geometry(I, n_pairs, coo_aux ? ts::Chunk<4>::CH : ts::Chunk<3>::CH, G);
-    rcode = ts_prepare(st, G, (const long long *)mptr);
-    if (rcode) return rcode;
     static_assert(ts::Chunk<3>::CH <= ts::Chunk<4>::CH && ts::Chunk<4>::CH % ts::Chunk<3>::CH == 0, "chunk lists by the narrow record width");
     const int n_shards = d_shards ? COO_SHARDS : 1;
     const long long shard_cap = d_shards ? coo_cap / COO_SHARDS : coo_cap;
@@ -573,7 +569,11 @@
     unsigned *n_chunks = nullptr;
     XM_HIP(xm_malloc_async((void **)&chunks, sizeof(longlong2) * (size_t)chunk_cap, st));
     XM_HIP(xm_malloc_async((void **)&n_chunks, sizeof(unsigned), st));
-    XM_HIP(hipMemsetAsync(n_chunks, 0, sizeof(unsigned), st));
+    FillList F;
+    F.add(fill, sizeof(int32_t) * (size_t)I);
+    F.add(n_chunks, sizeof(unsigned));
+    rcode = ts_prepare(st, G, (const long long *)mptr, &F);
+    if (rcode) return rcode;
     k_coo_chunks<<<dim3((unsigned)((n_shards + 255) / 256)), dim3(256), 0, st>>>(n_shards, shard_cap, (const unsigned long long *)d_shards,
                                                                                  n_pairs, chunks, n_chunks, chunk_cap);
     XM_LAUNCH_CHECK();
diff --git a/x-map_amd/csrc/tri_pairs.hip b/x-map_amd/csrc/tri_pairs.hip
--- a/x-map_amd/csrc/tri_pairs.hip
+++ b/x-map_amd/csrc/tri_pairs.hip
@@ -585,11 +585,12 @@
     hipStream_t st = (hipStream_t)stream;
     const bool exact_cos = method == XMAP_COSINE_EXACT;
     const double *nrm = norms + (method == XMAP_ADJUST_COSINE ? (size_t)R->n_items : 0);
+    FillList F;
     if (exact_cos) {
         double *zero_avg = nullptr;
         const size_t ub = sizeof(double) * (size_t)(R->n_users > 0 ? R->n_users : 1);
         XM_HIP(xm_malloc_async((void **)&zero_avg, ub, st));
-        XM_HIP(hipMemsetAsync(zero_avg, 0, ub, st));
+        F.add(zero_avg, ub);
         u_avg = zero_avg;
         method = XMAP_ADJUST_COSINE;
     }
@@ -597,12 +598,17 @@
     XM_ARG(!coo_ls || ((raw || method == XMAP_ADJUST_COSINE) && n_heavy_units == 0));
     XM_ARG(!raw || (coo_ls && n_heavy_units == 0 && n_heavy == 0));
     const size_t In = (size_t)(R->n_items > 0 ? R->n_items : 1);
+    const bool sums_cleared = (phases & XMAP_PAIRS_RESET) && (phases & XMAP_PAIRS_SHARD_SUMS);
     if (phases & XMAP_PAIRS_RESET) {
-        XM_HIP(hipMemsetAsync(d_counters, 0, 4 * sizeof(int64_t), st));
-        XM_HIP(hipMemsetAsync(d_shards, 0, 2 * COO_SHARDS * sizeof(int64_t), st));
+        F.add(d_counters, (sums_cleared ? 6 : 4) * sizeof(int64_t));
+        F.add(d_shards, 2 * COO_SHARDS * sizeof(int64_t));
         if (!(phases & XMAP_PAIRS_NO_MARKS)) XM_HIP(hipMemsetAsync(coo_i, 0xff, sizeof(int32_t) * (size_t)coo_cap, st));
-        XM_HIP(hipMemsetAsync(rowcnt, 0, sizeof(int32_t) * In, st));
-        if (mircnt) XM_HIP(hipMemsetAsync(mircnt, 0, sizeof(int32_t) * In, st));
+        F.add(rowcnt, sizeof(int32_t) * In);
+        if (mircnt) F.add(mircnt, sizeof(int32_t) * In);
+    }
+    {
+        int rc_fill = fill_multi(st, F);
+        if (rc_fill) return rc_fill;
     }
     TriArgs A;
     memset(&A, 0, sizeof(A));
@@ -661,7 +667,7 @@
         if (rcode) return rcode;
     }
     if (phases & XMAP_PAIRS_SHARD_SUMS) {
-        XM_HIP(hipMemsetAsync(d_counters + 4, 0, 2 * sizeof(int64_t), st));
+        if (!sums_cleared) XM_HIP(hipMemsetAsync(d_counters + 4, 0, 2 * sizeof(int64_t), st));
         k_shard_sums<<<dim3(1), dim3(256), 0, st>>>((const unsigned long long *)d_shards, (unsigned long long *)d_counters);
         XM_LAUNCH_CHECK();
     }
@@ -673,4 +679,17 @@
     }
     return XMAP_OK;
 }
-}
+
+int xmap_sim3_counters_begin(void *stream, const int64_t *d_counters) {
+    XM_ARG(d_counters);
+    return host_wait_post((hipStream_t)stream, HW_PAIRS, d_counters, 6);
+}
+int xmap_sim3_counters_wait(int64_t *h_out) {
+    XM_ARG(h_out);
+    const int64_t *h = nullptr;
+    int rcode = host_wait_take(HW_PAIRS, &h);
+    if (rcode) return rcode;
+    for (int c = 0; c < 6; c++) h_out[c] = h[c];
+    return XMAP_OK;
+}
+}
diff --git a/x-map_amd/csrc/util.hip b/x-map_amd/csrc/util.hip
--- a/x-map_amd/csrc/util.hip
+++ b/x-map_amd/csrc/util.hip
@@ -86,9 +86,74 @@
     return hipSuccess;
 }
 
+HostWait *host_wait() {
+    static thread_local HostWait *cur[64] = {nullptr};
+    int dev = 0;
+    if (hipGetDevice(&dev) != hipSuccess || dev < 0 || dev >= 64) { set_error("hipGetDevice failed"); return nullptr; }
+    if (cur[dev]) return cur[dev];
+    HostWait *p = new HostWait();
+    p->dev = dev;
+    bool ok = hipHostMalloc((void **)&p->h, sizeof(int64_t) * HW_SLOTS * HW_WORDS, hipHostMallocDefault) == hipSuccess;
+    for (int s = 0; s < HW_SLOTS && ok; s++) {
+        ok = hipEventCreateWithFlags(&p->ev[s], hipEventDisableTiming) == hipSuccess;
+        p->pending[s] = false;
+    }
+    if (!ok) { set_error("could not create the pinned read-back block"); delete p; return nullptr; }
+    cur[dev] = p;
+    return p;
+}
+int host_wait_post(hipStream_t st, int slot, const void *d_src, int words) {
+    XM_ARG(slot >= 0 && slot < HW_SLOTS && words >= 0 && words <= HW_WORDS);
+    HostWait *w = host_wait();
+    if (!w) return XMAP_ERR_HIP;
+    if (w->pending[slot]) {
+        XM_HIP(hipEventSynchronize(w->ev[slot]));
+        w->pending[slot] = false;
+    }
+    int64_t *h = w->h + (size_t)slot * HW_WORDS;
+    for (int x = 0; x < HW_WORDS; x++) h[x] = 0;
+    if (words) XM_HIP(hipMemcpyAsync(h, d_src, sizeof(int64_t) * (size_t)words, hipMemcpyDeviceToHost, st));
+    XM_HIP(hipEventRecord(w->ev[slot], st));
+    w->pending[slot] = true;
+    return XMAP_OK;
+}
+int host_wait_take(int slot, const int64_t **h) {
+    XM_ARG(slot >= 0 && slot < HW_SLOTS && h);
+    HostWait *w = host_wait();
+    if (!w) return XMAP_ERR_HIP;
+    if (!w->pending[slot]) {
+        set_error("read-back slot %d waited for without a post", slot);
+        return XMAP_ERR_ARG;
+    }
+    w->pending[slot] = false;
+    XM_HIP(hipEventSynchronize(w->ev[slot]));
+    *h = w->h + (size_t)slot * HW_WORDS;
+    return XMAP_OK;
+}
+
+__global__ __launch_bounds__(256) void k_fill_multi(FillList F) {
+    const int y = blockIdx.y;
+    unsigned *p = (unsigned *)F.p[y];
+    const unsigned long long n = F.words[y];
+    const unsigned v = F.val[y];
+    for (unsigned long long i = (unsigned long long)blockIdx.x * 256 + threadIdx.x; i < n; i += (unsigned long long)gridDim.x * 256) p[i] = v;
+}
+int fill_multi(hipStream_t st, const FillList &F) {
+    XM_ARG(F.n >= 0 && F.n <= FillList::MAX);
+    unsigned long long most = 0;
+    for (int y = 0; y < F.n; y++) most = F.words[y] > most ? F.words[y] : most;
+    if (F.n == 0 || most == 0) return XMAP_OK;
+    unsigned long long bx = (most + 1023) / 1024;
+    if (bx > 2048) bx = 2048;
+    k_fill_multi<<<dim3((unsigned)bx, (unsigned)F.n), dim3(256), 0, st>>>(F);
+    XM_LAUNCH_CHECK();
+    return XMAP_OK;
+}
+
 constexpr int SCAN_THREADS = 256;
 constexpr int SCAN_ITEMS = 8;
 constexpr int SCAN_TILE = SCAN_THREADS * SCAN_ITEMS;
+constexpr int SCAN2_MAX_TILES = 2048;
 
 __device__ __forceinline__ long long block_exclusive_scan(long long v, long long *total, long long *smem) {
     int lane = threadIdx.x & 63, w = threadIdx.x >> 6;
@@ -112,20 +177,34 @@
 }
 
 template <typename TIn>
-__global__ __launch_bounds__(SCAN_THREADS) void k_tile_sums(const TIn *in, long long n, long long *tile_sum) {
+struct ScanIn {
+    const TIn *in0, *in1;
+    int plus;
+    __device__ __forceinline__ long long load(int y, long long i) const {
+        if (y) return (long long)in1[i];
+        long long v = (long long)in0[i];
+        if (plus) v += (long long)in1[i];
+        return v;
+    }
+};
+
+template <typename TIn>
+__global__ __launch_bounds__(SCAN_THREADS) void k_tile_sums(ScanIn<TIn> S, long long n, long long n_tiles, long long *tile_sum) {
     __shared__ long long smem[4];
+    const int y = blockIdx.y;
     long long base = (long long)blockIdx.x * SCAN_TILE + (long long)threadIdx.x * SCAN_ITEMS;
     long long s = 0;
 #pragma unroll
     for (int k = 0; k < SCAN_ITEMS; k++)
-        if (base + k < n) s += (long long)in[base + k];
+        if (base + k < n) s += S.load(y, base + k);
     long long tot;
     block_exclusive_scan(s, &tot, smem);
-    if (threadIdx.x == 0) tile_sum[blockIdx.x] = tot;
-}
-
-__global__ __launch_bounds__(SCAN_THREADS) void k_scan_tile_sums(long long *tile_sum, long long n_tiles, long long *grand) {
+    if (threadIdx.x == 0) tile_sum[(long long)y * n_tiles + blockIdx.x] = tot;
+}
+
+__global__ __launch_bounds__(SCAN_THREADS) void k_scan_tile_sums(long long *tile_sum, long long n_tiles, long long *grand0, long long *grand1) {
     __shared__ long long smem[4];
+    tile_sum += (long long)blockIdx.y * n_tiles;
     long long carry = 0;
     for (long long b = 0; b < n_tiles; b += SCAN_THREADS) {
         long long i = b + threadIdx.x;
@@ -135,50 +214,74 @@
         if (i < n_tiles) tile_sum[i] = carry + ex;
         carry += tot;
     }
-    if (threadIdx.x == 0) *grand = carry;
-}
-
-template <typename TIn>
-__global__ __launch_bounds__(SCAN_THREADS) void k_tile_scan(const TIn *in, long long n, const long long *tile_off,
-                                                            long long *out) {
+    if (threadIdx.x == 0) *(blockIdx.y ? grand1 : grand0) = carry;
+}
+
+template <typename TIn, bool SELF>
+__global__ __launch_bounds__(SCAN_THREADS) void k_tile_scan(ScanIn<TIn> S, long long n, long long n_tiles, const long long *tile_sum,
+                                                            long long *out0, long long *out1) {
     __shared__ long long smem[4];
+    const int y = blockIdx.y;
+    tile_sum += (long long)y * n_tiles;
+    long long *out = y ? out1 : out0;
+    long long off;
+    if (SELF) {
+        long long part = 0;
+        for (long long t = threadIdx.x; t < (long long)blockIdx.x; t += SCAN_THREADS) part += tile_sum[t];
+        block_exclusive_scan(part, &off, smem);
+    } else {
+        off = tile_sum[blockIdx.x];
+    }
     long long base = (long long)blockIdx.x * SCAN_TILE + (long long)threadIdx.x * SCAN_ITEMS;
     long long v[SCAN_ITEMS];
     long long s = 0;
 #pragma unroll
     for (int k = 0; k < SCAN_ITEMS; k++) {
-        v[k] = (base + k < n) ? (long long)in[base + k] : 0;
+        v[k] = (base + k < n) ? S.load(y, base + k) : 0;
         s += v[k];
     }
     long long tot;
-    long long ex = block_exclusive_scan(s, &tot, smem) + tile_off[blockIdx.x];
+    long long ex = block_exclusive_scan(s, &tot, smem) + off;
 #pragma unroll
     for (int k = 0; k < SCAN_ITEMS; k++) {
         if (base + k < n) out[base + k] = ex;
         ex += v[k];
     }
+    if (SELF && blockIdx.x == gridDim.x - 1 && threadIdx.x == 0) out[n] = off + tot;
 }
 
 template <typename TIn>
-static int exclusive_scan(hipStream_t st, const TIn *in, int64_t *out, int64_t n, int64_t *h_total) {
-    XM_ARG(n >= 0);
+static int exclusive_scan(hipStream_t st, int n_arrays, const TIn *in0, const TIn *in1, int plus, int64_t *out0, int64_t *out1, int64_t n,
+                          int64_t *h_total) {
+    XM_ARG(n >= 0 && (n_arrays == 1 || n_arrays == 2));
     XM_SCOPE(st);
-    int64_t n_tiles = (n + SCAN_TILE - 1) / SCAN_TILE;
-    long long *tile = nullptr;
-    XM_HIP(xm_malloc_async((void **)&tile, sizeof(long long) * (size_t)(n_tiles + 1), st));
-    if (n_tiles > 0) {
-        k_tile_sums<TIn><<<dim3((unsigned)n_tiles), dim3(SCAN_THREADS), 0, st>>>(in, n, tile);
+    const int64_t n_tiles = (n + SCAN_TILE - 1) / SCAN_TILE;
+    XM_ARG(n_tiles < 0x7fffffffLL);
+    const ScanIn<TIn> S{in0, in1, plus};
+    if (n_tiles == 0) {
+        XM_HIP(hipMemsetAsync(out0 + n, 0, sizeof(int64_t), st));
+        if (n_arrays == 2) XM_HIP(hipMemsetAsync(out1 + n, 0, sizeof(int64_t), st));
+    } else {
+        long long *tile = nullptr;
+        XM_HIP(xm_malloc_async((void **)&tile, sizeof(long long) * (size_t)n_tiles * (size_t)n_arrays, st));
+        const dim3 grid((unsigned)n_tiles, (unsigned)n_arrays);
+        k_tile_sums<TIn><<<grid, dim3(SCAN_THREADS), 0, st>>>(S, n, n_tiles, tile);
         XM_LAUNCH_CHECK();
-    }
-    k_scan_tile_sums<<<dim3(1), dim3(SCAN_THREADS), 0, st>>>(tile, n_tiles, (long long *)(out + n));
-    XM_LAUNCH_CHECK();
-    if (n_tiles > 0) {
-        k_tile_scan<TIn><<<dim3((unsigned)n_tiles), dim3(SCAN_THREADS), 0, st>>>(in, n, tile, (long long *)out);
-        XM_LAUNCH_CHECK();
-    }
-    XM_HIP(xm_free_async(tile, st));
+        if (n_tiles <= SCAN2_MAX_TILES) {
+            k_tile_scan<TIn, true><<<grid, dim3(SCAN_THREADS), 0, st>>>(S, n, n_tiles, tile, (long long *)out0, (long long *)out1);
+            XM_LAUNCH_CHECK();
+        } else {
+            k_scan_tile_sums<<<dim3(1, (unsigned)n_arrays), dim3(SCAN_THREADS), 0, st>>>(tile, n_tiles, (long long *)(out0 + n),
+                                                                                          (long long *)(out1 ? out1 + n : nullptr));
+            XM_LAUNCH_CHECK();
+            k_tile_scan<TIn, false><<<grid, dim3(SCAN_THREADS), 0, st>>>(S, n, n_tiles, tile, (long long *)out0, (long long *)out1);
+            XM_LAUNCH_CHECK();
+        }
+        XM_HIP(xm_free_async(tile, st));
+    }
     if (h_total) {
-        XM_HIP(hipMemcpyAsync(h_total, out + n, sizeof(int64_t), hipMemcpyDeviceToHost, st));
+        XM_HIP(hipMemcpyAsync(h_total, out0 + n, sizeof(int64_t), hipMemcpyDeviceToHost, st));
+        if (n_arrays == 2) XM_HIP(hipMemcpyAsync(h_total + 1, out1 + n, sizeof(int64_t), hipMemcpyDeviceToHost, st));
         XM_HIP(hipStreamSynchronize(st));
     }
     return XMAP_OK;
@@ -187,7 +290,7 @@
 
 extern "C" {
 const char *xmap_last_error(void) { return xmap::g_err; }
-int xmap_version(void) { return 113; }
+int xmap_version(void) { return 114; }
 
 int xmap_trim(void) {
     XM_HIP(hipDeviceSynchronize());
@@ -226,9 +329,17 @@
 }
 
 int xmap_exclusive_scan_i64(void *stream, const int64_t *in, int64_t *out, int64_t n, int64_t *h_total) {
-    return xmap::exclusive_scan<long long>((hipStream_t)stream, (const long long *)in, out, n, h_total);
+    XM_ARG(out && (in || n == 0));
+    return xmap::exclusive_scan<long long>((hipStream_t)stream, 1, (const long long *)in, nullptr, 0, out, nullptr, n, h_total);
 }
 int xmap_exclusive_scan_i32_to_i64(void *stream, const int32_t *in, int64_t *out, int64_t n, int64_t *h_total) {
-    return xmap::exclusive_scan<int>((hipStream_t)stream, in, out, n, h_total);
-}
-}
+    XM_ARG(out && (in || n == 0));
+    return xmap::exclusive_scan<int>((hipStream_t)stream, 1, in, nullptr, 0, out, nullptr, n, h_total);
+}
+int xmap_exclusive_scan2_i32_to_i64(void *stream, const int32_t *in_a, const int32_t *in_b, int32_t a_plus_b, int64_t *out_a,
+                                    int64_t *out_b, int64_t n, int64_t *h_totals) {
+    XM_ARG(out_a && out_b && ((in_a && in_b) || n == 0));
+    return xmap::exclusive_scan<int>((hipStream_t)stream, 2, in_a, in_b, a_plus_b ? 1 : 0, out_a, out_b, n, h_totals);
+}
+int xmap_scan_self_tiles(void) { return xmap::SCAN2_MAX_TILES; }
+}
diff --git a/x-map_amd/xmap/engine/device.py b/x-map_amd/xmap/engine/device.py
--- a/x-map_amd/xmap/engine/device.py
+++ b/x-map_amd/xmap/engine/device.py
@@ -17,6 +17,7 @@
 
 SLOT_TARGET = 768
 CH_MIN = 2048
+STEPWISE = os.environ.get("XMAP_STAGE_A_STEPWISE") == "1"
 
 
 class DeviceRatings(object):
@@ -138,6 +139,10 @@
 
     def _empty(self, shape, dtype):
         return torch.empty(shape, dtype=dtype, device=self.dev)
+
+    def _step(self):
+        if STEPWISE:
+            torch.cuda.current_stream(self.dev).synchronize()
 
     def _out(self, shape, dtype, written):
         return self._empty(shape, dtype) if written else self._zeros(shape, dtype)
@@ -394,7 +399,7 @@
                                       vp(L.C), vp(L.uc_ptr), vp(L.uc_item), vp(L.uc_c)))
         L.slot_target = slot_target
 
-    def _tri_plan3(self, L, slot_target):
+    def _tri_plan3(self, L, slot_target, under_wait=None):
         R = self.R
         st = _stream(self.dev)
         I = R.n_items
@@ -407,10 +412,18 @@
         L.uc_c = self._empty(cap_heavy, torch.int32)
         h = (C.c_int64 * 10)()
         with self.timed("tri_plan"):
-            check(lib.xmap_sim3_plan(st, C.byref(R.c), i32(slot_target), vp(L.pre), vp(L.hid), vp(L.ctl), vp(L.Q), vp(L.C),
-                                     vp(L.small), vp(L.Wp), vp(L.Qcat), vp(L.uq_ptr), vp(L.uc_ptr),
-                                     i32(1 if getattr(L, "dups", False) else 0), vp(L.uq_item), vp(L.uq_q), vp(L.uc_item),
-                                     vp(L.uc_c), i64(cap_light), i64(cap_heavy), h))
+            check(lib.xmap_sim3_plan_begin(st, C.byref(R.c), i32(slot_target), vp(L.pre), vp(L.hid), vp(L.ctl), vp(L.Q), vp(L.C),
+                                           vp(L.small), vp(L.Wp), vp(L.Qcat), vp(L.uq_ptr), vp(L.uc_ptr),
+                                           i32(1 if getattr(L, "dups", False) else 0), vp(L.uq_item), vp(L.uq_q), vp(L.uc_item),
+                                           vp(L.uc_c), i64(cap_light), i64(cap_heavy)))
+            self._step()
+            if under_wait is not None:
+                under_wait()
+                self._step()
+            hint = getattr(L, "pairs_hint", None)
+            if hint is not None and getattr(L, "_pairs_pre", None) is None:
+                L._pairs_pre = self._pairs_buffers(L, 1.0, **hint)
+            check(lib.xmap_sim3_plan_wait(i64(cap_light), i64(cap_heavy), h))
         L.n_light, L.n_heavy_units = int(h[0]), int(h[1])
         L.cls_ptr = (C.c_int64 * 6)(*[int(h[2 + c]) for c in range(6)])
         L.CH, L.n_heavy = int(h[8]), int(h[9])
@@ -432,22 +445,17 @@
         coo_slack = 1.0
         while True:
             lo, hi = (0, L.n_light) if unit_range is None else (int(unit_range[0]), int(unit_range[1]))
-            cap_coo = (max(int(L.half_contrib * coo_slack), 1) // 4096 + 1100) * 4096
-            coo_i = self._empty(cap_coo, torch.int32)
-            coo_j = self._empty(cap_coo, torch.int32)
-            coo_sim = self._empty(cap_coo, torch.float64)
-            coo_mutu = self._empty(cap_coo, torch.int32)
-            coo_nij = self._empty(cap_coo, torch.int32)
-            coo_ls = self._empty(cap_coo, torch.float64) if (rec or raw) else None
-            rowcnt = self._empty(max(I, 1), torch.int32)
-            mircnt = self._empty(max(I, 1), torch.int32) if split else None
+            pre = L.__dict__.pop("_pairs_pre", None)
+            if pre is None or pre["key"] != self._pairs_key(L, coo_slack, rec or raw, split, count_mir and split and not raw):
+                pre = self._pairs_buffers(L, coo_slack, rec or raw, split, count_mir and split and not raw)
+            cap_coo = pre["cap_coo"]
+            coo_i, coo_j, coo_sim, coo_mutu, coo_nij, coo_ls = pre["coo"]
+            rowcnt, mircnt, d_cnt, d_shards = pre["rowcnt"], pre["mircnt"], pre["d_cnt"], pre["d_shards"]
             nh = L.n_heavy_units if do_heavy else 0
             hp_hi = self._empty(max(nh, 1) * 1024, torch.float64)
             hp_lo = self._empty(max(nh, 1) * 1024, torch.float64)
             hp_cnt = self._empty(max(nh, 1) * 1024, torch.int32)
             hp_mut = self._empty(max(nh, 1) * 1024, torch.int32)
-            d_cnt = self._zeros(6, torch.int64)
-            d_shards = self._empty(2 * 4096, torch.int64)
 
             deal = 0 if heavy_deal is None else abi.pairs_deal(heavy_deal[1], heavy_deal[0])
             heavy, merge = (abi.PAIRS_HEAVY, abi.PAIRS_HEAVY_MERGE) if do_heavy else (0, 0)
@@ -462,6 +470,7 @@
                     vp(L.uc_item), vp(L.uc_c), i32(nh), i32(L.n_heavy), phases,
                     vp(hp_hi), vp(hp_lo), vp(hp_cnt), vp(hp_mut), i64(cap_coo), vp(coo_i), vp(coo_j), vp(coo_sim),
                     vp(coo_mutu), vp(coo_nij), vp(coo_ls), vp(rowcnt), vp(d_shards), vp(d_cnt), vp(mircnt)))
+                self._step()
             if os.environ.get("XMAP_SPLIT_PHASES") == "1":
                 with self.timed("pair_heavy"):
                     run(abi.PAIRS_RESET | heavy)
@@ -472,12 +481,17 @@
             else:
                 with self.timed("pair_tri"):
                     run(abi.PAIRS_RESET | heavy | light | merge | abi.PAIRS_MIRCOUNT | abi.PAIRS_SHARD_SUMS)
+            check(lib.xmap_sim3_counters_begin(st, vp(d_cnt)))
+            self._step()
             if count_mir and split and not raw:
                 with self.timed("mir_count"):
-                    scratch = self._empty(cap_coo, torch.int32)
                     check(lib.xmap_sim3_mircount(st, i32(I), i64(cap_coo), vp(coo_i), vp(coo_j), vp(d_shards), i64(cap_coo),
-                                                 i32(1 if rec else 0), vp(scratch), vp(mircnt)))
-            h = d_cnt.tolist()
+                                                 i32(1 if rec else 0), vp(pre["mir_scratch"]), vp(mircnt)))
+                    self._step()
+                L._mirror_pre = self._mirror_buffers(cap_coo, 4 if rec else 3)
+            hc = (C.c_int64 * 6)()
+            check(lib.xmap_sim3_counters_wait(hc))
+            h = [int(x) for x in hc]
             if h[2]:
                 if L.slot_target <= 32:
                     raise abi.XmapError(abi.ERR_OVERFLOW, "pair-table overflow")
@@ -499,6 +513,31 @@
         if split:
             return out + (mircnt, d_shards) + (() if retry else (0,))
         return out if retry else out + (0,)
+
+    def _pairs_key(self, L, coo_slack, has_ls, split, count_mir):
+        cap_coo = (max(int(L.half_contrib * coo_slack), 1) // 4096 + 1100) * 4096
+        return (cap_coo, bool(has_ls), bool(split), bool(count_mir))
+
+    def _pairs_buffers(self, L, coo_slack, has_ls, split, count_mir):
+        I = self.R.n_items
+        key = self._pairs_key(L, coo_slack, has_ls, split, count_mir)
+        cap_coo = key[0]
+        coo = (self._empty(cap_coo, torch.int32), self._empty(cap_coo, torch.int32), self._empty(cap_coo, torch.float64),
+               self._empty(cap_coo, torch.int32), self._empty(cap_coo, torch.int32),
+               self._empty(cap_coo, torch.float64) if has_ls else None)
+        return {"key": key, "cap_coo": cap_coo, "coo": coo,
+                "rowcnt": self._empty(max(I, 1), torch.int32),
+                "mircnt": self._empty(max(I, 1), torch.int32) if split else None,
+                "d_cnt": self._empty(6, torch.int64),
+                "d_shards": self._empty(2 * 4096, torch.int64),
+                "mir_scratch": self._empty(cap_coo, torch.int32) if count_mir else None}
+
+    def _mirror_buffers(self, n_rec, rw):
+        I = self.R.n_items
+        return {"n_rec": int(n_rec), "rw": rw,
+                "row_ptr": self._out(I + 1, torch.int64, I > 0), "mptr": self._empty(I + 1, torch.int64),
+                "tot": self._empty(max(I, 1), torch.int32), "fill": self._empty(max(I, 1), torch.int32),
+                "buf_a": self._empty(max(int(n_rec), 1) * rw, torch.int64), "buf_b": self._empty(max(int(n_rec), 1) * rw, torch.int64)}
 
     def tri_scatter(self, coo, rowcnt, info, n=None, L=None):
         R = self.R
@@ -531,7 +570,8 @@
     def rec_sim(self, cap, slot_target=SLOT_TARGET):
         R = self.R
         with self.timed("rec_stats"):
-            stats, L = self.layout3(slot_target, ch_min=max(64, R.n_users + 2), wide=True)
+            stats, L = self.layout3(slot_target, ch_min=max(64, R.n_users + 2), wide=True,
+                                    pairs_hint=dict(has_ls=True, split=True, count_mir=True))
         S, n_unordered = self._pairs_to_csr("adjust_cosine", cap, stats, L, rec=True)
         S.cap, S.n_unordered, S.layout = int(cap), n_unordered, L
         S.norm = self.norms[R.n_items:2 * R.n_items]
@@ -549,7 +589,7 @@
                                       vp(col), vp(sim), vp(ls)))
         return cnt[:I], col[:I], sim[:I], ls[:I]
 
-    def layout3(self, slot_target=SLOT_TARGET, ch_min=CH_MIN, wide=False, item_range=None):
+    def layout3(self, slot_target=SLOT_TARGET, ch_min=CH_MIN, wide=False, item_range=None, pairs_hint=None):
         R = self.R
         st = _stream(self.dev)
         I, U, nnz = R.n_items, R.n_users, R.nnz
@@ -578,15 +618,19 @@
         L.half_contrib = R.half_contrib
         if item_range is None:
             with self.timed("layout3"):
-                call(abi.LAYOUT_RECORDS | abi.LAYOUT_STATS | abi.LAYOUT_UB_FLAGS, 0, I)
-            self._tri_plan3(L, slot_target)
+                call(abi.LAYOUT_RECORDS | abi.LAYOUT_STATS, 0, I)
+                self._step()
+            L.pairs_hint = pairs_hint
+            self._tri_plan3(L, slot_target, under_wait=None if wide else (lambda: call(abi.LAYOUT_UB_FLAGS, 0, I)))
         else:
             with self.timed("layout3"):
                 call(abi.LAYOUT_RECORDS | abi.LAYOUT_STATS, int(item_range[0]), int(item_range[1]))
+                self._step()
 
             def finish():
                 with self.timed("layout3_flags"):
                     call(abi.LAYOUT_UB_FLAGS | abi.LAYOUT_RC_FLAGS, 0, I)
+                    self._step()
                 self._tri_plan3(L, slot_target)
             L.finish = finish
         return (u_avg, u_norm, info, None, None), L
@@ -598,7 +642,7 @@
                                      vp(shards), i64(n), i32(1 if skip_self else 0), vp(scratch), vp(mir)))
         return mir
 
-    def tri_mirror(self, coo, own, mir, info, n, shards=None, rows=None, counted=False):
+    def tri_mirror(self, coo, own, mir, info, n, shards=None, rows=None, counted=False, pre=None):
         R = self.R
         st = _stream(self.dev)
         I = R.n_items
@@ -615,12 +659,9 @@
                 mir[:lo].zero_(); mir[hi:].zero_()
                 kept = int((own[lo:hi].long().sum() + mir[lo:hi].long().sum()).item())
         rw = 4 if coo_ls is not None else 3
-        row_ptr = self._out(I + 1, torch.int64, I > 0)
-        mptr = self._empty(I + 1, torch.int64)
-        tot = self._empty(max(I, 1), torch.int32)
-        fill = self._empty(max(I, 1), torch.int32)
-        buf_a = self._empty(max(int(n), 1) * rw, torch.int64)
-        buf_b = self._empty(max(int(n), 1) * rw, torch.int64)
+        if pre is None or pre["rw"] != rw or pre["n_rec"] < int(n):
+            pre = self._mirror_buffers(n, rw)
+        row_ptr, mptr, tot, fill, buf_a, buf_b = [pre[k] for k in ("row_ptr", "mptr", "tot", "fill", "buf_a", "buf_b")]
         col = self._empty(max(kept, 1), torch.int32)
         sim = self._empty(max(kept, 1), torch.float64)
         mutu = self._empty(max(kept, 1), torch.int32)
@@ -636,6 +677,7 @@
             check(lib.xmap_sim3_mirror(st, i32(I), i64(cap), vp(coo_i), vp(coo_j), vp(coo_sim), vp(coo_mutu), vp(coo_nij), vp(shards), i64(n),
                                        vp(own), vp(mir), vp(tot), vp(row_ptr), vp(mptr), vp(fill), vp(buf_a), vp(buf_b), vp(col),
                                        vp(sim), vp(mutu), vp(nij), vp(coo_ls), vp(ls), i32(lo), i32(hi)))
+            self._step()
         if coo_ls is not None:
             kept = int(row_ptr[I].item()) if I > 0 else 0
         S = self.sim_from_device(row_ptr, col[:kept], sim[:kept], mutu[:kept], nij[:kept], info)
@@ -648,7 +690,7 @@
             return self.tri_scatter(coo, rowcnt, stats[2], n, L), n_unordered
         coo, own, n, n_unordered, mir, shards = self.tri_pairs(method, cap, stats, L, do_heavy=not rec, rec=rec, split=True,
                                                                marks=False, count_mir=True)
-        return self.tri_mirror(coo, own, mir, stats[2], n, shards, counted=True), n_unordered
+        return self.tri_mirror(coo, own, mir, stats[2], n, shards, counted=True, pre=L.__dict__.pop("_mirror_pre", None)), n_unordered
 
     def item_sim_tri(self, method, cap, slot_target=SLOT_TARGET, ch_min=CH_MIN):
         if os.environ.get("XMAP_A_V2") == "1":
@@ -656,7 +698,7 @@
                 stats = self.stats()
             L = self.tri_layout(stats, slot_target, ch_min)
         else:
-            stats, L = self.layout3(slot_target, ch_min)
+            stats, L = self.layout3(slot_target, ch_min, pairs_hint=dict(has_ls=False, split=True, count_mir=True))
         S, n_unordered = self._pairs_to_csr(method, cap, stats, L)
         S.method = abi.METHODS[method] if isinstance(method, str) else int(method)
         S.cap = int(cap)
diff --git a/x-map_amd/xmap/engine/hipabi.py b/x-map_amd/xmap/engine/hipabi.py
--- a/x-map_amd/xmap/engine/hipabi.py
+++ b/x-map_amd/xmap/engine/hipabi.py
@@ -86,6 +86,7 @@
 
 EXPORTS = [
     "xmap_last_error", "xmap_version", "xmap_trim", "xmap_debug_arena", "xmap_debug_arena_call", "xmap_exclusive_scan_i64", "xmap_exclusive_scan_i32_to_i64",
+    "xmap_exclusive_scan2_i32_to_i64", "xmap_scan_self_tiles", "xmap_sim3_plan_begin", "xmap_sim3_plan_wait", "xmap_sim3_counters_begin", "xmap_sim3_counters_wait",
     "xmap_build_csc", "xmap_user_stats", "xmap_item_stats", 
     "xmap_sim2_layout", "xmap_sim2_plan", "xmap_sim2_units",
     "xmap_sim2_pairs", "xmap_sim2_scatter", "xmap_sim3_layout", "xmap_sim3_plan", "xmap_sim3_mircount", "xmap_sim3_mirror", "xmap_item_partials", "xmap_item_merge", "xmap_sim2_pack_partials",
```

Measured after the change: 25.85 billion, median of 6. 4.1% higher.
